# JanEGerken/HEAL-SWIN

Hardware: AMD Instinct MI355X
Metric: images/sec fwd+bwd, HEAL-SWIN nside=256 seg, batch=8 at 1/2/4/8 MI355X (higher is better)
Workload: dtype bf16

## Files before the change

heal_swin_amd/_lib.py:

```python
import ctypes
import os

import numpy as np

_PKG = os.path.dirname(os.path.abspath(__file__))
LIB_PATH = os.path.join(_PKG, "lib", "libhealswin.so")

HS_F32, HS_BF16 = 0, 1
HS_F64 = 3
HS_PRED_LABELS, HS_PRED_ROWS16 = 2, 4
HS_ATTN_COSINE = 1
HS_ATTN_FORCE_VALU = 2
HS_ATTN_RESIDUAL = 4
HS_ATTN_OVERWRITE_GRADS = 8
HS_EPI_BIAS, HS_EPI_GELU, HS_EPI_DGELU, HS_EPI_RESID = 0, 1, 2, 3
HS_ACC_DEFER = 2
HS_MLP_NORM_AFTER = 16
HS_U8, HS_I32, HS_I64 = 8, 9, 10
HS_FLAT_PATCH_ROWS, HS_FLAT_PIXEL_ROWS, HS_FLAT_IMAGE = 0, 1, 2
HS_DEPTH_L1, HS_DEPTH_L2, HS_DEPTH_HUBER, HS_DEPTH_LOGVAR = 0, 1, 2, 3
HS_DT_NONE, HS_DT_LOG, HS_DT_INV = 0, 1, 2
HS_DT_ZERO_BKG, HS_DT_1000_BKG, HS_DT_AFFINE, HS_DT_INVERSE = 1, 2, 4, 8
HS_DEPTH_STATS_WORDS = 15

c_i64 = ctypes.c_int64
c_int = ctypes.c_int
c_uint = ctypes.c_uint
c_ptr = ctypes.c_void_p
c_float = ctypes.c_float


class WgradProblem(ctypes.Structure):
    _fields_ = [("dy", c_ptr), ("x", c_ptr), ("dw", c_ptr), ("dbias", c_ptr), ("n_out", c_int), ("k_in", c_int), ("accumulate", c_int),
                ("gelu_x", c_int)]


def wgrad_problems(members):
    arr = (WgradProblem * len(members))()
    for q, (dy, x, dw, db, n_out, k_in, acc, gelu_x) in zip(arr, members):
        q.dy, q.x, q.dw, q.dbias = dy.data_ptr(), x.data_ptr(), dw.data_ptr(), (None if db is None else db.data_ptr())
        q.n_out, q.k_in, q.accumulate, q.gelu_x = int(n_out), int(k_in), int(acc), int(bool(gelu_x))
    return arr

_SIGNATURES = {
    "hs_nest2ring": [c_int, c_ptr, c_ptr, c_i64],
    "hs_ring2nest": [c_int, c_ptr, c_ptr, c_i64],
    "hs_nest_win_idcs": [c_int, c_ptr],
    "hs_rel_pos_index": [c_int, c_ptr],
    "hs_build_nest_roll_shift": [c_i64, c_int, c_int, c_ptr, c_ptr, c_ptr],
    "hs_build_nest_grid_shift": [c_int, c_int, c_int, c_ptr, c_ptr, c_ptr],
    "hs_build_ring_shift": [c_int, c_int, c_int, c_int, c_ptr, c_ptr, c_ptr],
    "hs_attn_mask_from_labels": [c_ptr, c_i64, c_int, c_ptr],
    "hs_flat_zorder": [c_int, c_int, c_int, c_ptr, c_ptr],
    "hs_build_flat_shift": [c_int, c_int, c_int, c_int, c_int, c_ptr, c_ptr, c_ptr],
    "hs_flat_rel_pos_index": [c_int, c_ptr, c_ptr],
    "hs_flat_attn_mask": [c_int, c_int, c_int, c_int, c_ptr],
    "hs_flat_img_to_rows": [c_ptr, c_int, c_ptr, c_int, c_int, c_int, c_int, c_int, c_int, c_int, c_int, c_i64, c_ptr],
    "hs_flat_rows_to_img": [c_ptr, c_int, c_ptr, c_int, c_int, c_int, c_int, c_int, c_int, c_int, c_int, c_i64, c_ptr],
    "hs_flat_resize": [c_ptr, c_int, c_i64, c_int, c_int, c_int, c_int, c_ptr, c_ptr, c_ptr, c_ptr, c_ptr, c_int, c_int, c_int, c_int, c_int,
                       c_int, c_i64, c_int, c_int, c_int, c_int, c_int, c_int, c_float, c_float, c_ptr],
    "hs_rel_bias_gather": [c_ptr, c_ptr, c_ptr, c_int, c_int, c_int, c_ptr],
    "hs_rel_bias_scatter_grad_sorted_add": [c_ptr, c_ptr, c_ptr, c_ptr, c_int, c_int, c_int, c_ptr],
    "hs_cos_head_scale_fwd": [c_ptr, c_ptr, c_int, c_ptr],
    "hs_cos_head_scale_bwd": [c_ptr, c_ptr, c_ptr, c_int, c_int, c_ptr],
    "hs_rel_bias_gather_many": [c_ptr, c_ptr, c_int, c_ptr, c_ptr, c_int, c_int, c_ptr],
    "hs_rel_bias_scatter_grad_sorted_many": [c_ptr, c_ptr, c_ptr, c_ptr, c_int, c_ptr, c_ptr, c_int, c_int, c_ptr],
    "hs_cos_head_scale_many": [c_ptr, c_ptr, c_ptr, c_ptr, c_ptr, c_int, c_ptr],
    "hs_rel_bias_scatter_grad": [c_ptr, c_ptr, c_ptr, c_int, c_int, c_int, c_ptr],
    "hs_rel_bias_scatter_grad_sorted": [c_ptr, c_ptr, c_ptr, c_ptr, c_int, c_int, c_int, c_ptr],
    "hs_window_attn_fwd": [c_ptr, c_ptr, c_ptr, c_ptr, c_ptr, c_ptr, c_i64, c_ptr,
                           c_int, c_i64, c_int, c_int, c_int, c_uint, ctypes.c_float, ctypes.c_uint64, c_int, c_ptr],
    "hs_window_attn_bwd": [c_ptr, c_ptr, c_ptr, c_ptr, c_ptr, c_ptr, c_ptr, c_ptr, c_ptr, c_ptr, c_ptr, c_i64, c_ptr,
                           c_int, c_i64, c_int, c_int, c_int, c_uint, ctypes.c_float, ctypes.c_uint64, c_int, c_ptr],
    "hs_gather_rows": [c_ptr, c_ptr, c_ptr, c_i64, c_int, c_i64, c_i64, c_ptr],
    "hs_pix2ang_nest": [c_int, c_i64, c_i64, c_ptr, c_ptr],
    "hs_ln_head_supported": [c_int, c_int, c_int],
    "hs_expand_ln_head_supported": [c_int, c_int, c_int, c_int],
    "hs_expand_ln_head_fwd": [c_ptr, c_ptr, c_ptr, c_ptr, c_ptr, c_ptr, c_ptr, c_ptr, c_ptr, c_i64, c_int, c_int, c_int, c_ptr],
    "hs_expand_ln_head_ce_fwd": [c_ptr, c_ptr, c_ptr, c_ptr, c_ptr, c_ptr, c_ptr, c_int, c_ptr, c_ptr, c_ptr, c_ptr, c_ptr, c_i64, c_int, c_int,
                                 c_int, c_ptr],
    "hs_expand_ln_head_ce_step_fwd": [c_ptr, c_ptr, c_ptr, c_ptr, c_ptr, c_ptr, c_ptr, c_int, c_ptr, c_ptr, c_ptr, c_ptr, c_ptr, c_ptr, c_ptr,
                                      c_ptr, c_i64, c_int, c_int, c_int, c_ptr],
    "hs_ln_head_ce_bwd": [c_ptr, c_ptr, c_ptr, c_ptr, c_ptr, c_ptr, c_int, c_ptr, c_ptr, c_ptr, c_ptr, c_ptr, c_ptr, c_i64, c_int, c_int, c_ptr],
    "hs_expand_ln_head_depth_fwd": [c_ptr, c_ptr, c_ptr, c_ptr, c_ptr, c_ptr, c_int, c_float, c_int, c_ptr, c_ptr, c_ptr, c_ptr, c_ptr, c_i64,
                                    c_int, c_int, c_int, c_ptr],
    "hs_expand_ln_head_depth_step_fwd": [c_ptr, c_ptr, c_ptr, c_ptr, c_ptr, c_ptr, c_int, c_float, c_int, c_ptr, c_ptr, c_ptr, c_ptr, c_ptr,
                                         c_int, c_int, c_float, c_float, c_int, ctypes.c_double, c_ptr, c_int, c_ptr, c_ptr, c_ptr, c_ptr,
                                         c_i64, c_int, c_int, c_int, c_ptr],
    "hs_ln_head_depth_bwd": [c_ptr, c_ptr, c_ptr, c_ptr, c_int, c_float, c_ptr, c_int, c_ptr, c_ptr, c_ptr, c_ptr, c_ptr, c_ptr, c_i64, c_int,
                             c_int, c_ptr],
    "hs_ln_head_fwd": [c_ptr, c_ptr, c_ptr, c_ptr, c_ptr, c_ptr, c_i64, c_int, c_int, c_int, c_ptr],
    "hs_ln_head_bwd": [c_ptr, c_ptr, c_ptr, c_ptr, c_ptr, c_ptr, c_ptr, c_ptr, c_i64, c_int, c_int, c_int, c_ptr],
    "hs_sample_bilinear_u8": [c_ptr, c_int, c_int, c_int, c_int, c_ptr, c_ptr, c_i64, c_ptr, c_ptr],
    "hs_sample_mask_u8": [c_ptr, c_int, c_int, c_int, c_ptr, c_ptr, c_i64, c_int, c_ptr, c_ptr],
    "hs_hp_interp_weights_nest": [c_int, c_ptr, c_ptr, c_i64, c_ptr, c_ptr],
    "hs_backproject_labels": [c_ptr, c_int, c_i64, c_i64, c_int, c_i64, c_i64, c_i64, c_ptr, c_i64, c_int, c_ptr, c_ptr],
    "hs_backproject_image": [c_ptr, c_i64, c_i64, c_ptr, c_ptr, c_i64, c_ptr, c_ptr],
    "hs_seg_confusion": [c_ptr, c_int, c_i64, c_i64, c_int, c_i64, c_i64, c_i64, c_ptr, c_i64, c_ptr, c_int, c_ptr, c_ptr, c_ptr],
    "hs_depth_points": [c_ptr, c_int, c_i64, c_i64, c_i64, c_i64, c_i64, c_i64, c_ptr, c_i64, c_ptr, c_int, c_ptr, c_ptr, c_ptr, c_ptr,
                        c_ptr],
    "hs_chamfer_nn": [c_ptr, c_ptr, c_i64, c_i64, c_ptr, c_ptr, c_i64, c_i64, c_i64, c_int, c_ptr, c_ptr, c_ptr, c_ptr, c_ptr, c_ptr,
                      c_ptr],
    "hs_depth_metrics": [c_ptr, c_int, c_i64, c_i64, c_i64, c_i64, c_i64, c_i64, c_i64, c_ptr, c_int, c_i64, c_i64, c_i64, c_int,
                         ctypes.c_double, c_ptr, c_int, c_ptr, c_ptr, c_ptr],
    "hs_backproject_depth": [c_ptr, c_int, c_i64, c_i64, c_i64, c_i64, c_ptr, c_ptr, c_i64, c_ptr, c_ptr],
    "hs_flat_depth_to_hp": [c_ptr, c_int, c_i64, c_i64, c_i64, c_i64, c_ptr, c_ptr, c_ptr, c_i64, c_ptr, c_ptr],
    "hs_depth_metrics_gather": [c_ptr, c_int, c_i64, c_i64, c_i64, c_i64, c_i64, c_ptr, c_ptr, c_ptr, c_i64, c_ptr, c_int, c_i64, c_i64,
                                c_int, ctypes.c_double, c_ptr, c_int, c_ptr, c_ptr, c_ptr],
    "hs_sample_bilinear_u8_f32": [c_ptr, c_int, c_int, c_int, c_int, c_ptr, c_ptr, c_i64, c_ptr, c_ptr],
    "hs_sample_nearest_f32": [c_ptr, c_int, c_int, c_int, c_ptr, c_ptr, c_i64, c_float, c_ptr, c_ptr],
    "hs_depth_target": [c_ptr, c_i64, c_i64, c_ptr, c_i64, c_i64, c_i64, c_i64, c_int, c_int, c_float, c_float, c_ptr],
    "hs_depth_stats_update": [c_ptr, c_i64, c_int, c_int, c_ptr, c_ptr, c_ptr],
    "hs_depth_stats_merge": [c_ptr, c_int, c_ptr, c_ptr],
    "hs_gelu_fwd": [c_ptr, c_ptr, c_i64, ctypes.c_float, ctypes.c_uint64, c_int, c_ptr],
    "hs_gelu_bwd": [c_ptr, c_ptr, c_ptr, c_i64, ctypes.c_float, ctypes.c_uint64, c_int, c_ptr],
    "hs_residual_drop": [c_ptr, c_ptr, c_ptr, c_ptr, c_i64, c_i64, ctypes.c_float, ctypes.c_uint64, c_int, c_ptr],
    "hs_linear_wgrad": [c_ptr, c_ptr, c_ptr, c_ptr, c_ptr, c_i64, c_int, c_int, c_int, c_int, c_ptr],
    "hs_reduce_flush": [c_ptr],
    "hs_set_seed_epoch": [c_ptr],
    "hs_linear_wgrad_gelu": [c_ptr, c_ptr, c_ptr, c_ptr, c_ptr, c_i64, c_int, c_int, c_int, c_int, c_ptr],
    "hs_linear_wgrad_gelu_supported": [c_i64, c_int, c_int, c_int],
    "hs_linear_wgrad_group_variant": [c_i64, c_int, c_int, c_int],
    "hs_linear_wgrad_group": [c_ptr, c_int, c_ptr, c_i64, c_int, c_ptr],
    "hs_mlp_fused_supported": [c_int, c_int, c_int],
    "hs_mlp_fused_fwd": [c_ptr, c_ptr, c_ptr, c_ptr, c_ptr, c_ptr, c_ptr, c_ptr, c_ptr, c_ptr, c_ptr, c_ptr, c_ptr, c_i64, c_int, c_int, c_uint,
                         c_int, c_ptr],
    "hs_mlp_fused_bwd": [c_ptr, c_ptr, c_ptr, c_ptr, c_ptr, c_ptr, c_ptr, c_i64, c_int, c_int, c_int, c_ptr],
    "hs_mlp_fused_drop_fwd": [c_ptr, c_ptr, c_ptr, c_ptr, c_ptr, c_ptr, c_ptr, c_ptr, c_ptr, c_ptr, c_ptr, c_ptr, c_ptr, c_ptr, c_i64, c_float,
                              ctypes.c_uint64, ctypes.c_uint64, c_i64, c_int, c_int, c_uint, c_int, c_ptr],
    "hs_mlp_fused_drop_bwd": [c_ptr, c_ptr, c_ptr, c_ptr, c_ptr, c_ptr, c_ptr, c_float, ctypes.c_uint64, c_i64, c_int, c_int, c_int, c_ptr],
    "hs_adam_step": [c_ptr, c_ptr, c_ptr, c_ptr, c_ptr, c_i64, c_float, c_ptr, c_float, c_float, c_float, c_float, c_int, c_ptr, c_ptr],
    "hs_adam_advance": [c_ptr, c_ptr],
    "hs_grad_stats": [c_ptr, c_i64, c_ptr, c_int, c_ptr, c_ptr],
    "hs_grad_guard_finalize": [c_ptr, c_i64, c_ptr, c_int, c_int, c_float, c_ptr, c_ptr, c_ptr, c_ptr],
    "hs_adam_step_guarded": [c_ptr, c_ptr, c_ptr, c_ptr, c_ptr, c_i64, c_float, c_ptr, c_float, c_float, c_float, c_float, c_int, c_ptr, c_float,
                             c_ptr, c_int, c_ptr],
    "hs_adam_advance_guarded": [c_ptr, c_ptr, c_int, c_ptr, c_ptr],
    "hs_grad_scale": [c_ptr, c_i64, c_float, c_ptr, c_ptr],
    "hs_split_bf16x3": [c_ptr, c_ptr, c_i64, c_int, c_int, c_ptr],
    "hs_gelu_split3": [c_ptr, c_ptr, c_ptr, c_i64, c_int, ctypes.c_float, ctypes.c_uint64, c_ptr],
    "hs_linear_wgrad_ld": [c_ptr, c_i64, c_i64, c_ptr, c_i64, c_i64, c_ptr, c_ptr, c_ptr, c_i64, c_int, c_int, c_int, c_ptr],
    "hs_layernorm_fwd": [c_ptr, c_ptr, c_ptr, c_ptr, c_ptr, c_ptr, c_ptr, c_i64, c_int, c_int, c_ptr],
    "hs_add_layernorm_fwd": [c_ptr, c_ptr, c_ptr, c_ptr, c_ptr, c_ptr, c_ptr, c_ptr, c_i64, c_int, c_int, c_ptr],
    "hs_add_layernorm_bwd": [c_ptr, c_ptr, c_ptr, c_ptr, c_ptr, c_ptr, c_ptr, c_ptr, c_ptr, c_ptr, c_int, c_i64, c_int, c_int, c_ptr],
    "hs_layernorm_drop_fwd": [c_ptr, c_ptr, c_ptr, c_ptr, c_ptr, c_ptr, c_ptr, c_ptr, c_i64, ctypes.c_float, ctypes.c_uint64,
                              c_i64, c_int, c_int, c_ptr],
    "hs_layernorm_drop_bwd": [c_ptr, c_ptr, c_ptr, c_ptr, c_ptr, c_ptr, c_ptr, c_ptr, c_ptr, c_int, c_ptr, c_i64, ctypes.c_float,
                              ctypes.c_uint64, c_i64, c_int, c_int, c_ptr],
    "hs_add_layernorm_drop_fwd": [c_ptr, c_ptr, c_ptr, c_ptr, c_ptr, c_ptr, c_ptr, c_ptr, c_ptr, c_i64, ctypes.c_float,
                                  ctypes.c_uint64, c_i64, c_int, c_int, c_ptr],
    "hs_layernorm_fwd_ex": [c_ptr, c_ptr, c_ptr, c_ptr, c_ptr, c_ptr, c_ptr, c_ptr, c_ptr, c_ptr, c_ptr, c_ptr, c_i64, ctypes.c_float,
                            ctypes.c_uint64, c_i64, c_int, c_int, c_ptr],
    "hs_add_layernorm_drop_bwd": [c_ptr, c_ptr, c_ptr, c_ptr, c_ptr, c_ptr, c_ptr, c_ptr, c_ptr, c_ptr, c_ptr, c_int, c_ptr, c_i64,
                                  ctypes.c_float, ctypes.c_uint64, c_i64, c_int, c_int, c_ptr],
    "hs_seg_ce_fwd": [c_ptr, c_ptr, c_ptr, c_ptr, c_i64, c_i64, c_int, c_i64, c_i64, c_i64, c_int, c_i64, c_int, c_ptr],
    "hs_seg_ce_bwd": [c_ptr, c_ptr, c_ptr, c_ptr, c_ptr, c_i64, c_i64, c_int, c_i64, c_i64, c_i64, c_i64, c_i64, c_i64, c_int, c_i64,
                      c_int, c_ptr],
    "hs_depth_loss_fwd": [c_ptr, c_ptr, c_ptr, c_i64, c_i64, c_int, c_i64, c_i64, c_i64, c_int, c_float, c_int, c_ptr],
    "hs_depth_loss_bwd": [c_ptr, c_ptr, c_ptr, c_ptr, c_i64, c_i64, c_int, c_i64, c_i64, c_i64, c_i64, c_i64, c_i64, c_int, c_float, c_int, c_ptr],
    "hs_gemm_nt": [c_ptr, c_i64, c_ptr, c_i64, c_int, c_ptr, c_i64, c_ptr, c_i64, c_int, c_ptr, c_ptr, c_ptr, c_i64, c_int, c_int,
                   ctypes.c_float, ctypes.c_uint64, c_int, c_ptr],
    "hs_gemm_nt_set_tile": [c_int],
    "hs_set_reserved_cus": [c_int],
    "hs_transpose_many_16": [c_ptr, c_int, c_int, c_ptr],
    "hs_debug_occupy_cus": [c_int, c_int, c_int, ctypes.c_double, c_ptr],
    "hs_debug_buffer_soffset_probe": [c_ptr, c_int, c_int, c_ptr, c_ptr],
    "hs_window_attn_module_supported": [c_int, c_int, c_int, c_int],
    "hs_window_attn_module_fwd": [c_ptr, c_ptr, c_ptr, c_ptr, c_ptr, c_ptr, c_ptr, c_ptr, c_ptr, c_ptr, c_ptr, c_i64, c_ptr, c_int, c_i64,
                                  c_int, c_int, c_int, c_uint, c_int, c_ptr],
    "hs_window_attn_module_fwd_train": [c_ptr] * 17 + [c_i64] + [c_ptr] * 6 + [c_int, c_i64, c_int, c_int, c_int, c_uint, c_int, c_ptr],
    "hs_window_attn_module_bwd_chain": [c_ptr] * 14 + [c_i64] + [c_ptr] * 11 + [c_int, c_int, c_i64, c_int, c_int, c_int, c_uint, c_int, c_ptr],
    "hs_layernorm_bwd": [c_ptr, c_ptr, c_ptr, c_ptr, c_ptr, c_ptr, c_ptr, c_ptr, c_ptr, c_int, c_i64, c_int, c_int, c_ptr],
    "hs_patch_merge_fwd": [c_ptr, c_ptr, c_ptr, c_ptr, c_ptr, c_ptr, c_ptr, c_ptr, c_i64, c_int, c_int, c_int, c_ptr],
    "hs_patch_merge_bwd": [c_ptr, c_ptr, c_ptr, c_ptr, c_ptr, c_ptr, c_ptr, c_ptr, c_ptr, c_ptr, c_ptr, c_ptr, c_ptr, c_int, c_i64,
                           c_int, c_int, c_int, c_ptr],
    "hs_patch_expand_fwd": [c_ptr, c_ptr, c_ptr, c_ptr, c_ptr, c_ptr, c_ptr, c_ptr, c_i64, c_int, c_int, c_int, c_int, c_ptr],
    "hs_patch_expand_bwd": [c_ptr, c_ptr, c_ptr, c_ptr, c_ptr, c_ptr, c_ptr, c_ptr, c_ptr, c_ptr, c_ptr, c_ptr, c_ptr, c_int, c_i64,
                            c_int, c_int, c_int, c_int, c_ptr],
}
_OTHER = {
    "hs_version": ([], ctypes.c_char_p),
    "hs_last_error": ([], ctypes.c_char_p),
    "hs_status_string": ([c_int], ctypes.c_char_p),
    "hs_device_count": ([], c_int),
    "hs_get_reserved_cus": ([], c_int),
    "hs_grad_guard_piece": ([], c_int),
    "hs_get_seed_epoch": ([], c_ptr),
    "hs_reduce_pending": ([c_ptr], c_int),
    "hs_layernorm_bwd_workspace": ([c_i64, c_int], c_i64),
    "hs_seg_ce_partials": ([c_i64, c_i64], c_i64),
    "hs_depth_loss_partials": ([c_i64, c_i64], c_i64),
    "hs_depth_points_workspace": ([c_i64, c_i64], c_i64),
    "hs_depth_metrics_partials": ([c_i64], c_i64),
    "hs_depth_stats_partials": ([c_i64], c_i64),
    "hs_flat_resize_lds_bytes": ([c_int, c_int, c_int, c_int, c_int, c_int], c_i64),
    "hs_ln_head_partials": ([c_i64], c_i64),
    "hs_expand_ln_head_blocks": ([c_i64], c_i64),
    "hs_linear_wgrad_workspace": ([c_i64, c_int, c_int], c_i64),
    "hs_linear_wgrad_group_workspace": ([c_ptr, c_int, c_i64, c_int], c_i64),
    "hs_window_attn_bwd_workspace": ([c_int, c_i64, c_int, c_int, c_int, c_int], c_i64),
    "hs_patch_merge_bwd_workspace": ([c_i64, c_int, c_int], c_i64),
    "hs_window_attn_module_bwd_chain_workspace": ([c_int, c_i64, c_int, c_int, c_int], c_i64),
    "hs_patch_expand_bwd_workspace": ([c_i64, c_int, c_int, c_int], c_i64),
}
EXPORTED_SYMBOLS = sorted(list(_SIGNATURES) + list(_OTHER))


def _load():
    if not os.path.exists(LIB_PATH):
        raise RuntimeError(
            f"libhealswin.so not found at {LIB_PATH}: build it first (python heal_swin_amd/build.py, or "
            "__graft_entry__.build()).  heal_swin_amd has no CPU or PyTorch fallback."
        )
    lib = ctypes.CDLL(LIB_PATH)
    for name, argtypes in _SIGNATURES.items():
        fn = getattr(lib, name)
        fn.argtypes = argtypes
        fn.restype = c_int
    for name, (argtypes, restype) in _OTHER.items():
        fn = getattr(lib, name)
        fn.argtypes = argtypes
        fn.restype = restype
    return lib


lib = _load()


def check(status, what):
    if status != 0:
        msg = lib.hs_last_error().decode()
        kind = lib.hs_status_string(status).decode()
        if status == 1:
            raise AssertionError(f"{what}: {msg}")
        raise RuntimeError(f"{what} failed ({kind}): {msg}")


def version():
    return lib.hs_version().decode()


def device_count():
    return int(lib.hs_device_count())


def np_ptr(a):
    return None if a is None else a.ctypes.data_as(c_ptr)


def ptr(t):
    return None if t is None else ctypes.c_void_p(t.data_ptr())


def stream_ptr(device):
    import torch

    return ctypes.c_void_p(torch.cuda.current_stream(device).cuda_stream)


def dtype_code(dtype):
    import torch

    if dtype == torch.float32:
        return HS_F32
    if dtype == torch.bfloat16:
        return HS_BF16
    raise TypeError(f"heal_swin_amd kernels support float32 and bfloat16 activations, got {dtype}")


def nest2ring(nside, ipix):
    a = np.ascontiguousarray(ipix, dtype=np.int64)
    out = np.empty_like(a)
    check(lib.hs_nest2ring(int(nside), np_ptr(a), np_ptr(out), a.size), "hs_nest2ring")
    return out


def ring2nest(nside, ipix):
    a = np.ascontiguousarray(ipix, dtype=np.int64)
    out = np.empty_like(a)
    check(lib.hs_ring2nest(int(nside), np_ptr(a), np_ptr(out), a.size), "hs_ring2nest")
    return out


def nest_win_idcs(window_size):
    side = int(round(window_size ** 0.5))
    out = np.empty((max(side, 1), max(side, 1)), dtype=np.int64)
    check(lib.hs_nest_win_idcs(int(window_size), np_ptr(out)), "hs_nest_win_idcs")
    return out


def rel_pos_index(window_size):
    out = np.empty((window_size, window_size), dtype=np.int64)
    check(lib.hs_rel_pos_index(int(window_size), np_ptr(out)), "hs_rel_pos_index")
    return out


def _shift_out(n):
    return np.empty(n, np.int32), np.empty(n, np.int32), np.empty(n, np.uint8)


def build_nest_roll_shift(n_pix, window_size, shift_size):
    idx, inv, lab = _shift_out(n_pix)
    check(lib.hs_build_nest_roll_shift(int(n_pix), int(window_size), int(shift_size), np_ptr(idx), np_ptr(inv), np_ptr(lab)),
          "hs_build_nest_roll_shift")
    return idx, inv, lab


def build_nest_grid_shift(nside, base_pix, window_size):
    idx, inv, lab = _shift_out(max(base_pix, 0) * nside * nside)
    check(lib.hs_build_nest_grid_shift(int(nside), int(base_pix), int(window_size), np_ptr(idx), np_ptr(inv), np_ptr(lab)),
          "hs_build_nest_grid_shift")
    return idx, inv, lab


def build_ring_shift(nside, base_pix, window_size, shift_size):
    idx, inv, lab = _shift_out(max(base_pix, 0) * nside * nside)
    check(lib.hs_build_ring_shift(int(nside), int(base_pix), int(window_size), int(shift_size), np_ptr(idx), np_ptr(inv),
                                  np_ptr(lab)), "hs_build_ring_shift")
    return idx, inv, lab


def attn_mask_from_labels(labels, window_size):
    lab = np.ascontiguousarray(labels, dtype=np.uint8)
    out = np.empty((lab.size // window_size, window_size, window_size), dtype=np.float32)
    check(lib.hs_attn_mask_from_labels(np_ptr(lab), lab.size, int(window_size), np_ptr(out)), "hs_attn_mask_from_labels")
    return out


def flat_zorder(Ht, Wt, T):
    z = np.empty(Ht * Wt, np.int32)
    rm = np.empty(Ht * Wt, np.int32)
    check(lib.hs_flat_zorder(int(Ht), int(Wt), int(T), np_ptr(z), np_ptr(rm)), "hs_flat_zorder")
    return z, rm


def build_flat_shift(Ht, Wt, T, window, shift):
    idx, inv, lab = _shift_out(max(Ht * Wt, 0))
    check(lib.hs_build_flat_shift(int(Ht), int(Wt), int(T), int(window), int(shift), np_ptr(idx), np_ptr(inv), np_ptr(lab)),
          "hs_build_flat_shift")
    return idx, inv, lab


# ... 13 lines not shown
```

heal_swin_amd/csrc/gemm_nt.hip:

```cpp
#include <cstdlib>
#include <type_traits>

#include "hs_gelu.h"

namespace hs {
HS_DEFINE_SEED_EPOCH_SETTER(set_seed_epoch_gemm_nt)
namespace {

typedef unsigned int u32x2 __attribute__((__vector_size__(8)));
typedef unsigned int u32x4v __attribute__((__vector_size__(16)));

#ifndef HS_GEMM_EPI_RING
#define HS_GEMM_EPI_RING 1
#endif
#ifndef HS_GEMM_STORE_AUX
#define HS_GEMM_STORE_AUX 2
#endif
#ifndef HS_GEMM_IN_AUX
#define HS_GEMM_IN_AUX 2
#endif
#ifndef HS_GEMM_EXP
#define HS_GEMM_EXP 0
#endif
#ifndef HS_GEMM_STAGGER_CYCLES
#define HS_GEMM_STAGGER_CYCLES 40000
#endif
enum { EPI_BIAS = 0, EPI_GELU = 1, EPI_DGELU = 2, EPI_RESID = 3 };
constexpr int64_t kMaxRecords = 0x7FFFFE00;

struct GemmParams {
    const uint16_t *a, *b;
    int64_t lda, ldb;
    int k;
    const uint16_t *a2, *b2;
    int64_t lda2, ldb2;
    int k2;
    const float* bias;
    uint16_t* c;
    uint16_t* aux;
    int64_t m;
    int n;
    int tiles_n, tiles, per_xcd, blocks_per_xcd;
    float drop_p;
    uint64_t seed;
#ifdef HS_GEMM_TRACE
    uint64_t* trace;
#endif
};
#ifdef HS_GEMM_TRACE
constexpr int kTraceCap = 240;
#endif

constexpr int epi_younger_ops(int tm, int i) {
    const int stores = i < 2 ? i : 1;
    const int last_d = i + 1 < tm - 1 ? i + 1 : tm - 1;
    return 4 * (stores + (last_d - i));
}

template <int OFF>
__device__ __forceinline__ u32x4 lds_read_b128(uint32_t addr) {
    u32x4 v;
    asm volatile("ds_read_b128 %0, %1 offset:%2" : "=v"(v) : "v"(addr), "n"(OFF));
    return v;
}

template <int BM, int BN, int WM, int WN, int NSTAGE, bool ALIAS, int EPI, bool DROP, bool FAST>
__global__ void __launch_bounds__(WM * WN * 64, 2) gemm_nt_kernel(GemmParams p) {
#if defined(__HIP_DEVICE_COMPILE__)
    constexpr int NW = WM * WN;
    constexpr int TM = BM / WM / 32, TN = BN / WN / 32;
    constexpr int AB = BM * 128, BB = BN * 128, STAGE = AB + BB;
    constexpr int IW = FAST ? NW / 2 : NW;
    constexpr int AI = AB / 1024 / IW, BI = BB / 1024 / IW;
    static_assert(AI >= 1 && BI >= 1 && TM >= 1 && TN >= 1, "tile too small for the wave grid");
    static_assert(!ALIAS || NW * 4096 <= STAGE, "patches do not fit a stage buffer");
    constexpr bool HAS_IN = EPI == EPI_DGELU || EPI == EPI_RESID;
    constexpr bool RING = HS_GEMM_EPI_RING && HAS_IN && ALIAS && TM == 4 && TN == 2 && STAGE >= NW * 8192;
    constexpr bool LBIAS = ALIAS && EPI != EPI_DGELU;
    constexpr int NSLOT = NSTAGE + 1;
    static_assert(BN * 4 <= 1024, "a bias slot holds one 1-KB DMA piece");
    constexpr int BIAS_OFF = NSTAGE * STAGE + (ALIAS ? 0 : NW * 4096), BIAS_LDS = LBIAS ? NSLOT * 1024 : 0;
#ifdef HS_GEMM_TRACE
    constexpr int TRACE_LDS = BIAS_OFF + BIAS_LDS + NW * kTraceCap * 8 <= 163840 ? NW * kTraceCap * 8 : 0;
#else
    constexpr int TRACE_LDS = 0;
#endif
    static_assert(BIAS_OFF + BIAS_LDS + TRACE_LDS <= 163840, "LDS of one workgroup exceeds 160 KB");
    __shared__ __attribute__((aligned(16))) unsigned char smem[BIAS_OFF + BIAS_LDS + TRACE_LDS];

    const int tid = threadIdx.x, lane = tid & 63, half = lane >> 5, l31 = lane & 31;
    const int wave = __builtin_amdgcn_readfirstlane(tid >> 6);
    const int wm = wave / WN, wn = wave % WN;

    const int xcd = blockIdx.x & 7, lb = blockIdx.x >> 3;
    const int id_end = min((xcd + 1) * p.per_xcd, p.tiles);
    const int id0 = xcd * p.per_xcd + lb;
    if (id0 >= id_end) return;
    const int nk1 = (p.k + 63) >> 6, nk2 = (p.k2 + 63) >> 6, nk = nk1 + nk2;
#if HS_GEMM_EXP & 24
    {
        const int phases = (HS_GEMM_EXP & 16) ? 4 : 2;
        const long long wait = (long long)(lb % phases) * (HS_GEMM_STAGGER_CYCLES / phases);
        const long long t0 = clock64();
        while (clock64() - t0 < wait) __builtin_amdgcn_s_sleep(8);
    }
#endif

    constexpr bool SC = FAST;
    static_assert(!FAST || (AI % 4 == 0 && BI % 4 == 0), "FAST: whole groups of four pieces per issuing wave");
    constexpr int AJ = SC ? 4 : AI, BJ = SC ? 4 : BI;
    int a_row[AJ], a_col[AJ], b_row[BJ], b_col[BJ];
#pragma unroll
    for (int j = 0; j < AJ; ++j) {
        const int q = (wave * AI + j) * 64 + lane, R = q >> 4, lc = (q & 15) ^ (R & 15);
        a_row[j] = 2 * R + (lc >> 3);
        a_col[j] = (lc & 7) << 4;
    }
#pragma unroll
    for (int j = 0; j < BJ; ++j) {
        const int q = (wave * BI + j) * 64 + lane, R = q >> 4, lc = (q & 15) ^ (R & 15);
        b_row[j] = 2 * R + (lc >> 3);
        b_col[j] = (lc & 7) << 4;
    }

    __amdgpu_buffer_rsrc_t ra, rb;
    int a_off[AJ], b_off[BJ];
    int kseg = 0;
    int a_ld32 = 0, b_ld32 = 0;
    int slot_i = 0;
    __amdgpu_buffer_rsrc_t rbias = __builtin_amdgcn_make_buffer_rsrc((void*)p.bias, 0, p.bias ? p.n * 4 : 0, 0x00020000);
    auto retarget = [&](int id, bool s2, bool enter) {
        const int tm = id / p.tiles_n, tn = id - tm * p.tiles_n;
        const int64_t m0 = (int64_t)tm * BM;
        const int n0 = tn * BN;
        if constexpr (LBIAS) {
            if (enter) {
                if (wave == 0)
                    __builtin_amdgcn_raw_ptr_buffer_load_lds(rbias, (lds_void*)(smem + BIAS_OFF + slot_i * 1024), 16,
                                                             lane * 4 < BN ? (uint32_t)(lane * 16) : kOob, n0 * 4, 0, 0);
                slot_i = slot_i + 1 == NSLOT ? 0 : slot_i + 1;
            }
        }
        const uint16_t* ap = s2 ? p.a2 : p.a;
        const uint16_t* bp = s2 ? p.b2 : p.b;
        const int64_t lda = s2 ? p.lda2 : p.lda, ldb = s2 ? p.ldb2 : p.ldb;
        kseg = (s2 ? p.k2 : p.k) * 2;
        int64_t abytes = (p.m - m0 - 1) * lda * 2 + kseg, bbytes = (int64_t)(p.n - n0 - 1) * ldb * 2 + kseg;
        abytes = abytes > kMaxRecords ? kMaxRecords : abytes;
        bbytes = bbytes > kMaxRecords ? kMaxRecords : bbytes;
        ra = __builtin_amdgcn_make_buffer_rsrc((void*)(ap + m0 * lda), 0, (int)abytes, 0x00020000);
        rb = __builtin_amdgcn_make_buffer_rsrc((void*)(bp + (int64_t)n0 * ldb), 0, (int)bbytes, 0x00020000);
#pragma unroll
        for (int j = 0; j < AJ; ++j) a_off[j] = a_row[j] * ((int)lda * 2) + a_col[j];
#pragma unroll
        for (int j = 0; j < BJ; ++j) b_off[j] = b_row[j] * ((int)ldb * 2) + b_col[j];
        a_ld32 = (int)lda * 64;
        b_ld32 = (int)ldb * 64;
    };
    auto issue_pieces = [&](int kb, int buf, auto first_c, auto count_c) {
        constexpr int first = decltype(first_c)::value, count = decltype(count_c)::value;
        if (IW < NW && wave >= IW) return;
        unsigned char* base = smem + buf * STAGE;
#pragma unroll
        for (int q = first; q < first + count; ++q) {
            if constexpr (SC) {
            if (q < AI) {
                __builtin_amdgcn_raw_ptr_buffer_load_lds(ra, (lds_void*)(base + (wave * AI + q) * 1024), 16, (uint32_t)a_off[q % AJ],
                                                         kb + (q >> 2) * a_ld32, 0, 0);
            } else {
                const int j = q - AI;
                __builtin_amdgcn_raw_ptr_buffer_load_lds(rb, (lds_void*)(base + AB + (wave * BI + j) * 1024), 16, (uint32_t)b_off[j % BJ],
                                                         kb + (j >> 2) * b_ld32, 0, 0);
            }
            } else {

            if (q < AI) {
                const uint32_t voff = kb + a_col[q] < kseg ? (uint32_t)(a_off[q] + kb) : kOob;
                __builtin_amdgcn_raw_ptr_buffer_load_lds(ra, (lds_void*)(base + (wave * AI + q) * 1024), 16, voff, 0, 0, 0);
            } else {
                const int j = q - AI;
                const uint32_t voff = kb + b_col[j] < kseg ? (uint32_t)(b_off[j] + kb) : kOob;
                __builtin_amdgcn_raw_ptr_buffer_load_lds(rb, (lds_void*)(base + AB + (wave * BI + j) * 1024), 16, voff, 0, 0, 0);
            }
            }
        }
    };

    const uint32_t lds0 = (uint32_t)(uintptr_t)(__attribute__((address_space(3))) unsigned char*)smem;
#ifdef HS_GEMM_TRACE
    const bool tr_on = TRACE_LDS > 0 && p.trace && (blockIdx.x == 0 || blockIdx.x == 9);
    int tr_n = 0;
    const uint32_t tr_base = lds0 + BIAS_OFF + BIAS_LDS + wave * kTraceCap * 8;
    auto TR = [&](int code) {
        if (tr_on && tr_n < kTraceCap) {
            const uint64_t t = (clock64() << 8) | (uint64_t)code;
            if (lane == 0) asm volatile("ds_write_b64 %0, %1" ::"v"(tr_base + tr_n * 8), "v"(t) : "memory");
            ++tr_n;
        }
    };
#else
    auto TR = [&](int) {};
#endif
    uint32_t a_frag[TM], b_frag[TN];
#pragma unroll
    for (int i = 0; i < TM; ++i) {
        const int r = wm * (BM / WM) + i * 32 + l31, R = r >> 1;
        a_frag[i] = lds0 + R * 256 + (((((r & 1) << 3) + half) ^ (R & 15)) << 4);
    }
#pragma unroll
    for (int j = 0; j < TN; ++j) {
        const int r = wn * (BN / WN) + j * 32 + l31, R = r >> 1;
        b_frag[j] = lds0 + AB + R * 256 + (((((r & 1) << 3) + half) ^ (R & 15)) << 4);
    }

    f32x16 acc[TN][TM];
#pragma unroll
    for (int j = 0; j < TN; ++j)
#pragma unroll
        for (int i = 0; i < TM; ++i)
#pragma unroll
            for (int r = 0; r < 16; ++r) acc[j][i][r] = 0.f;
#if HS_GEMM_EXP & 2
    int64_t exp_total = p.m * (int64_t)p.n * 2;
    exp_total = exp_total > kMaxRecords ? kMaxRecords : exp_total;
    const __amdgpu_buffer_rsrc_t rexp = __builtin_amdgcn_make_buffer_rsrc((void*)p.aux, 0, (int)(p.aux ? exp_total : 0), 0x00020000);
    const uint32_t exp_share = (uint32_t)((exp_total / gridDim.x) & ~(int64_t)1023);
    uint32_t exp_pos = 0;
    const uint32_t exp_base = blockIdx.x * exp_share;
#endif

    auto compute = [&](int buf, bool prefetch, int kb_next, int buf_next) {
        const uint32_t bo = buf * STAGE;
        constexpr int NSET = (TM == 4 && TN == 2) ? 2 : 3;
        u32x4 fa[NSET][TM], fb[NSET][TN];
        auto read_frags = [&](auto ks_c) {
            constexpr int ks = decltype(ks_c)::value, set = ks % NSET;
#pragma unroll
            for (int j = 0; j < TN; ++j) fb[set][j] = lds_read_b128<0>((b_frag[j] ^ (ks << 5)) + bo);
#pragma unroll
            for (int i = 0; i < TM; ++i) fa[set][i] = lds_read_b128<0>((a_frag[i] ^ (ks << 5)) + bo);
        };
        constexpr int PIECES = AI + BI;
        constexpr int PER = TM + TN;
        auto wait_frags = [&](auto ks_c, auto left_c) {
            constexpr int ks = decltype(ks_c)::value, left = decltype(left_c)::value, set = ks % NSET;
            (void)fa;
            (void)fb;
            if constexpr (TM == 2 && TN == 2)
                asm volatile("s_waitcnt lgkmcnt(%4)" : "+v"(fa[set][0]), "+v"(fa[set][1]), "+v"(fb[set][0]), "+v"(fb[set][1]) : "n"(left));
            else if constexpr (TM == 4 && TN == 2)
// ... 124 lines not shown
                    } else {
                        u32x4 rws[4];
#pragma unroll
                        for (int t = 0; t < 4; ++t)
                            rws[t] = __builtin_bit_cast(u32x4, __builtin_amdgcn_raw_buffer_load_b128(rx, rl_voff, row_soff(i, t), 0));
                        asm volatile("ds_write_b128 %0, %1" ::"v"(row_addr), "v"(rws[0]) : "memory");
                        asm volatile("ds_write_b128 %0, %1 offset:1024" ::"v"(row_addr), "v"(rws[1]) : "memory");
                        asm volatile("ds_write_b128 %0, %1 offset:2048" ::"v"(row_addr), "v"(rws[2]) : "memory");
                        asm volatile("ds_write_b128 %0, %1 offset:3072" ::"v"(row_addr), "v"(rws[3]) : "memory");
                    }
#pragma unroll
                    for (int j = 0; j < TJ; ++j)
#pragma unroll
                        for (int g = 0; g < 4; ++g)
                            asm volatile("ds_read_b64 %0, %1" : "=v"(xin[j][g]) : "v"(own_addr + (((4 * j + g) ^ (l31 & 7)) << 4)));
                    asm volatile("s_waitcnt lgkmcnt(0)"
                                 : "+v"(xin[0][0]), "+v"(xin[0][1]), "+v"(xin[0][2]), "+v"(xin[0][3]), "+v"(xin[TJ - 1][0]),
                                   "+v"(xin[TJ - 1][1]), "+v"(xin[TJ - 1][2]), "+v"(xin[TJ - 1][3]));
                } else {
#pragma unroll
                    for (int j = 0; j < TJ; ++j)
#pragma unroll
                        for (int g = 0; g < 4; ++g) {
                            const int n = ncol0 + j * 32 + 4 * half + 8 * g;
                            xin[j][g] = __builtin_amdgcn_raw_buffer_load_b64(rx, n < p.n ? (uint32_t)(ml * n2 + n * 2) : kOob, 0, 0);
                        }
                }
            }
            u32x2 o1[TJ][4], o2[TJ][4];
            {
#pragma unroll
                for (int j = 0; j < TJ; ++j) {
                    if constexpr (LBIAS) lds_bias(j, bias4[j]);
#pragma unroll
                    for (int g = 0; g < 4; ++g) {
                        const int n = ncol0 + j * 32 + 4 * half + 8 * g;
                        f32x16& a16 = acc[TJ * jh + j][i];
                        f32x2 v[2] = {f32x2{a16[4 * g], a16[4 * g + 1]} + f32x2{bias4[j][g].x, bias4[j][g].y},
                                      f32x2{a16[4 * g + 2], a16[4 * g + 3]} + f32x2{bias4[j][g].z, bias4[j][g].w}};
                        uint32_t ck = 0;
                        if (DROP) ck = rng.chunk_key((uint64_t)((m0 + ml) * p.n + n) >> 3);
                        auto drop2 = [&](int t) {
                            const uint32_t hh = ElemRng::pair_bits(ck, t == 0 ? (half ? ElemRng::kM2 : ElemRng::kM0) : (half ? ElemRng::kM3 : ElemRng::kM1));
                            return f32x2{rng.keep_lo(hh), rng.keep_hi(hh)};
                        };
                        if (EPI == EPI_GELU) {
                            o1[j][g] = u32x2{pack_bf16x2(v[0].x, v[0].y), pack_bf16x2(v[1].x, v[1].y)};
                            a16[4 * g] = v[0].x; a16[4 * g + 1] = v[0].y; a16[4 * g + 2] = v[1].x; a16[4 * g + 3] = v[1].y;
                            continue;
                        } else {
                            if (EPI == EPI_DGELU || EPI == EPI_RESID) {
#pragma unroll
                                for (int t = 0; t < 2; ++t) {
                                    const f32x2 x = {__uint_as_float(xin[j][g][t] << 16), __uint_as_float(xin[j][g][t] & 0xffff0000u)};
                                    if (EPI == EPI_DGELU) {
                                        v[t] *= gelu_grad2(x);
                                        if (DROP) v[t] *= drop2(t);
                                    } else {
                                        v[t] += x;
                                    }
                                }
                            }
                            o1[j][g] = u32x2{pack_bf16x2(v[0].x, v[0].y), pack_bf16x2(v[1].x, v[1].y)};
                        }
#pragma unroll
                        for (int r = 0; r < 4; ++r) a16[4 * g + r] = 0.f;
                    }
                }
            }
            auto make_o2 = [&]() {
#pragma unroll
                for (int j = 0; j < TJ; ++j)
#pragma unroll
                    for (int g0 = 0; g0 < 4; g0 += 2) {
                        f32x16& a16 = acc[TJ * jh + j][i];
                        f32x2 v[4] = {f32x2{a16[4 * g0], a16[4 * g0 + 1]}, f32x2{a16[4 * g0 + 2], a16[4 * g0 + 3]},
                                      f32x2{a16[4 * g0 + 4], a16[4 * g0 + 5]}, f32x2{a16[4 * g0 + 6], a16[4 * g0 + 7]}};
#if !(HS_GEMM_EXP & 4)
#pragma unroll
                        for (int t = 0; t < 4; ++t) v[t] = gelu2(v[t]);
#endif
#pragma unroll
                        for (int gg = 0; gg < 2; ++gg) {
                            const int g = g0 + gg;
                            if (DROP) {
                                const int n = ncol0 + j * 32 + 4 * half + 8 * g;
                                const uint32_t ck = rng.chunk_key((uint64_t)((m0 + ml) * p.n + n) >> 3);
#pragma unroll
                                for (int t = 0; t < 2; ++t) {
                                    const uint32_t hh = ElemRng::pair_bits(ck, t == 0 ? (half ? ElemRng::kM2 : ElemRng::kM0) : (half ? ElemRng::kM3 : ElemRng::kM1));
                                    v[2 * gg + t] *= f32x2{rng.keep_lo(hh), rng.keep_hi(hh)};
                                }
                            }
                            o2[j][g] = u32x2{pack_bf16x2(v[2 * gg].x, v[2 * gg].y), pack_bf16x2(v[2 * gg + 1].x, v[2 * gg + 1].y)};
#pragma unroll
                            for (int r = 0; r < 4; ++r) a16[4 * g + r] = 0.f;
                        }
                    }
            };
            TR(20);
            auto emit = [&](const __amdgpu_buffer_rsrc_t& rs, const u32x2 (&o)[TJ][4]) {
                if (wide) {
#pragma unroll
                    for (int j = 0; j < TJ; ++j)
#pragma unroll
                        for (int g = 0; g < 4; ++g)
                            asm volatile("ds_write_b64 %0, %1" ::"v"(own_out + (((4 * j + g) ^ (l31 & 7)) << 4)), "v"(o[j][g]) : "memory");
                    u32x4 rws[4];
                    asm volatile("ds_read_b128 %0, %1" : "=v"(rws[0]) : "v"(row_addr));
                    asm volatile("ds_read2_b64 %0, %1 offset0:129 offset1:128" : "=v"(rws[1]) : "v"(row_addr));
                    asm volatile("ds_read_b128 %0, %1 offset:2048" : "=v"(rws[2]) : "v"(row_addr));
                    asm volatile("ds_read2_b64 %0, %1 offset0:129 offset1:128" : "=v"(rws[3]) : "v"(row_addr + 2048));
                    asm volatile("s_waitcnt lgkmcnt(0)" : "+v"(rws[0]), "+v"(rws[1]), "+v"(rws[2]), "+v"(rws[3]));
                    TR(22);
#pragma unroll
                    for (int t = 0; t < 4; ++t)
                        __builtin_amdgcn_raw_buffer_store_b128(__builtin_bit_cast(u32x4v, rws[t]), rs, rl_voff, row_soff(i, t), HS_GEMM_STORE_AUX);
                    asm volatile("s_nop 0" ::"v"(rws[0]), "v"(rws[1]), "v"(rws[2]), "v"(rws[3]));
                } else {
#pragma unroll
                    for (int j = 0; j < TJ; ++j)
#pragma unroll
                        for (int g = 0; g < 4; ++g) {
                            const int n = ncol0 + j * 32 + 4 * half + 8 * g;
                            __builtin_amdgcn_raw_buffer_store_b64(o[j][g], rs, n < p.n ? (uint32_t)(ml * n2 + n * 2) : kOob, 0, HS_GEMM_STORE_AUX);
                        }
                }
            };
            if (EPI == EPI_GELU) {
                if (NW == 8 && wave >= NW / 2) {
                    make_o2();
                    emit(rx, o2);
                    TR(21);
                    __builtin_amdgcn_sched_barrier(0);
                    if (p.c) emit(rc, o1);
                } else {
                    if (p.c) emit(rc, o1);
                    TR(21);
                    __builtin_amdgcn_sched_barrier(0);
                    make_o2();
                    emit(rx, o2);
                }
            } else {
                emit(rc, o1);
            }
            if constexpr (RING) {
                if (i + 2 < TM) request_in(i + 2);
            }
            TR(12 + i);
        }
        }
    };

    const int stride = p.blocks_per_xcd;
    int id_i = id0, ks_i = 0;
    int id_c = id0, ks_c = 0;
    int slot_c = 0;
    auto advance_issue = [&]() {
        ++ks_i;
        if (ks_i == nk) {
            ks_i = 0;
            id_i += stride;
            if (id_i < id_end) retarget(id_i, nk1 == 0, true);
        } else if (ks_i == nk1) {
            retarget(id_i, true, false);
        }
    };
    auto kb_of = [&](int ks) { return (ks >= nk1 ? ks - nk1 : ks) * 128; };
    retarget(id_i, false, true);
    constexpr int AHEAD = NSTAGE - 1, PIECES_ALL = AI + BI;
    int issued = 0;
#pragma unroll
    for (int q = 0; q < AHEAD; ++q) {
        if (id_i < id_end) {
            issue_pieces(kb_of(ks_i), q, std::integral_constant<int, 0>{}, std::integral_constant<int, PIECES_ALL>{});
            advance_issue();
            ++issued;
        }
    }
    int buf = 0, buf_free = AHEAD;
#if HS_GEMM_EXP & 32
    if (NW == 8 && wave >= NW / 2) __builtin_amdgcn_s_setprio(1);
#endif
#if HS_GEMM_EXP & 64
    if (NW == 8 && wave < NW / 2) __builtin_amdgcn_s_setprio(1);
#endif
    bool drained = false;
    constexpr int kEpiOps = TM * (TN / 2 > 0 ? TN / 2 : 1) * 4;
    static_assert((AHEAD - 1) * PIECES_ALL + kEpiOps <= 63, "vmcnt immediate");
    TR(0);
    while (true) {
        TR(3);
        if (IW < NW && wave >= IW) {
        } else if (AHEAD > 1 && issued == AHEAD && !drained)
            asm volatile("s_waitcnt vmcnt(%0)" ::"n"((AHEAD - 1) * PIECES_ALL) : "memory");
        else if (drained && issued == AHEAD)
            asm volatile("s_waitcnt vmcnt(%0)" ::"n"((AHEAD - 1) * PIECES_ALL + kEpiOps) : "memory");
        else if (drained && issued == 1)
            asm volatile("s_waitcnt vmcnt(%0)" ::"n"(kEpiOps) : "memory");
        else
            asm volatile("s_waitcnt vmcnt(0)" ::: "memory");
        drained = false;
        TR(1);
        __builtin_amdgcn_s_barrier();
        TR(2);
        const bool more = id_i < id_end;
        const bool last = ks_c + 1 == nk;
        compute(buf, more, kb_of(ks_i), buf_free);
        --issued;
        if (more) {
            advance_issue();
            ++issued;
        }
        const int buf_done = buf;
        buf = buf + 1 == NSTAGE ? 0 : buf + 1;
        buf_free = buf_free + 1 == NSTAGE ? 0 : buf_free + 1;
        if (last) {
            epilogue(id_c, buf_done, slot_c);
            slot_c = slot_c + 1 == NSLOT ? 0 : slot_c + 1;
            drained = true;
            ks_c = 0;
            id_c += stride;
            if (id_c >= id_end) break;
        } else {
            ++ks_c;
        }
    }
#ifdef HS_GEMM_TRACE
    if (tr_on) {
        asm volatile("s_waitcnt vmcnt(0) lgkmcnt(0)" ::: "memory");
        uint64_t* out = p.trace + ((blockIdx.x == 0 ? 0 : 1) * NW + wave) * kTraceCap;
        for (int i = lane; i < kTraceCap; i += 64) {
            u32x2 v = {0u, 0u};
            if (i < tr_n) {
                asm volatile("ds_read_b64 %0, %1\n\ts_waitcnt lgkmcnt(0)" : "=v"(v) : "v"(tr_base + i * 8) : "memory");
            }
            out[i] = ((uint64_t)v[1] << 32) | v[0];
        }
    }
#endif
#endif
}

template <int BM, int BN, int WM, int WN, int NSTAGE, bool ALIAS, bool FAST>
int launch_tile(GemmParams& p, int epi, int wgs_per_cu, hipStream_t s) {
    const int tiles_m = (int)((p.m + BM - 1) / BM);
    p.tiles_n = (p.n + BN - 1) / BN;
    const int64_t tiles = (int64_t)tiles_m * p.tiles_n;
    if (tiles > 0x7fffffff) return fail(HS_ERR_UNSUPPORTED, "too many output tiles");
    p.tiles = (int)tiles;
    p.per_xcd = (p.tiles + 7) / 8;
    const int resident = usable_cus_per_xcd() * wgs_per_cu;
    p.blocks_per_xcd = p.per_xcd < resident ? p.per_xcd : resident;
    const dim3 grid((unsigned)(8 * p.blocks_per_xcd)), block(WM * WN * 64);
    const bool drop = p.drop_p > 0.f;
#define HS_GEMM_LAUNCH(E, D) hipLaunchKernelGGL((gemm_nt_kernel<BM, BN, WM, WN, NSTAGE, ALIAS, E, D, FAST>), grid, block, 0, s, p)
    switch (epi) {
        case EPI_BIAS: HS_GEMM_LAUNCH(EPI_BIAS, false); break;
        case EPI_GELU:
            if (drop) HS_GEMM_LAUNCH(EPI_GELU, true);
            else HS_GEMM_LAUNCH(EPI_GELU, false);
            break;
        case EPI_DGELU:
            if (drop) HS_GEMM_LAUNCH(EPI_DGELU, true);
            else HS_GEMM_LAUNCH(EPI_DGELU, false);
            break;
        default: HS_GEMM_LAUNCH(EPI_RESID, false); break;
    }
#undef HS_GEMM_LAUNCH
    HS_LAUNCH_CHECK("gemm_nt");
    return HS_OK;
}

}

int gemm_nt_check_shape(const char* who, int64_t lda, int64_t ldb, int k, int64_t lda2, int64_t ldb2, int k2, int64_t m, int n) {
    HS_CHECK_ARG(m > 0 && n > 0 && k > 0 && k2 >= 0, "%s: empty shape", who);
    if (k % 8 || k2 % 8 || lda % 8 || ldb % 8 || (k2 && (lda2 % 8 || ldb2 % 8)) || n % 4)
        return fail(HS_ERR_UNSUPPORTED, "%s: k, k2 and the row strides must be multiples of 8, n a multiple of 4", who);
    if (lda * 2 * 256 > kMaxRecords || ldb * 2 * 256 > kMaxRecords || (int64_t)n * 2 * 256 > kMaxRecords)
        return fail(HS_ERR_UNSUPPORTED, "%s: row stride too large", who);
    if (((m + 127) / 128) * (((int64_t)n + 127) / 128) > 0x7fffffff) return fail(HS_ERR_UNSUPPORTED, "%s: too many output tiles", who);
    return HS_OK;
}

}

namespace {
int g_tile_variant = 0;
}

#ifdef HS_GEMM_TRACE
namespace {
uint64_t* g_trace = nullptr;
}
extern "C" int hs_gemm_nt_set_trace(void* buf) {
    g_trace = (uint64_t*)buf;
    return 0;
}
#endif

extern "C" {

int hs_gemm_nt_set_tile(int variant) {
    g_tile_variant = variant;
    return HS_OK;
}

int hs_gemm_nt(const void* a, int64_t lda, const void* b, int64_t ldb, int k, const void* a2, int64_t lda2, const void* b2,
               int64_t ldb2, int k2, const float* bias, void* c, void* aux, int64_t m, int n, int epilogue, float drop_p,
               uint64_t seed, int dtype, void* stream) {
    using namespace hs;
    HS_CHECK_ARG(dtype == HS_BF16, "hs_gemm_nt: bf16 activations only (fp32 runs use the library GEMM)");
    HS_CHECK_ARG(a && b && m > 0 && n > 0 && k > 0, "hs_gemm_nt: null operand or empty shape");
    HS_CHECK_ARG(epilogue >= EPI_BIAS && epilogue <= EPI_RESID, "hs_gemm_nt: unknown epilogue %d", epilogue);
    HS_CHECK_ARG(k2 == 0 || (a2 && b2 && k2 > 0), "hs_gemm_nt: second segment needs a2, b2, k2 > 0");
    HS_CHECK_ARG(c || (epilogue == EPI_GELU && aux), "hs_gemm_nt: no output");
    HS_CHECK_ARG(epilogue == EPI_BIAS || aux, "hs_gemm_nt: this epilogue needs aux");
    HS_CHECK_ARG(drop_p >= 0.f && drop_p <= 1.f, "hs_gemm_nt: drop_p must be in [0, 1]");
    HS_CHECK_ALIGNED("hs_gemm_nt", 16, a, b, a2, b2, bias, c, aux);
    if (int st = gemm_nt_check_shape("hs_gemm_nt", lda, ldb, k, lda2, ldb2, k2, m, n)) return st;
    GemmParams p{};
    p.a = (const uint16_t*)a; p.b = (const uint16_t*)b; p.lda = lda; p.ldb = ldb; p.k = k;
    p.a2 = (const uint16_t*)a2; p.b2 = (const uint16_t*)b2; p.lda2 = lda2; p.ldb2 = ldb2; p.k2 = k2;
    p.bias = bias; p.c = (uint16_t*)c; p.aux = (uint16_t*)aux; p.m = m; p.n = n;
    p.drop_p = drop_p; p.seed = seed;
#ifdef HS_GEMM_TRACE
    p.trace = g_trace;
#endif
    int variant = g_tile_variant;
    if (!variant) {
        const int64_t tiles2 = ((m + 255) / 256) * ((n + 127) / 128), tiles3 = ((m + 255) / 256) * ((n + 255) / 256);
        if (tiles2 < 256)
            variant = 1;
        else if ((epilogue == EPI_GELU || epilogue == EPI_DGELU) ? n >= 512 : (n >= 1024 && k + k2 >= 512))
            variant = 3;
        else if (n >= 256 && tiles3 >= 768 && k % 64 == 0 && k2 % 64 == 0)
            variant = 3;
        else
            variant = 2;
    }
    if (variant == 3 && (epilogue == EPI_DGELU || epilogue == EPI_RESID) && n % 8) variant = 2;
    hipStream_t st = (hipStream_t)stream;
    const bool fast = k % 64 == 0 && k2 % 64 == 0;
    switch (variant) {
        case 2: return fast ? launch_tile<256, 128, 4, 2, 3, true, true>(p, epilogue, 1, st) : launch_tile<256, 128, 4, 2, 3, true, false>(p, epilogue, 1, st);
        case 3: return fast ? launch_tile<256, 256, 2, 4, 2, true, true>(p, epilogue, 1, st) : launch_tile<256, 256, 2, 4, 2, true, false>(p, epilogue, 1, st);
        default: return launch_tile<128, 128, 2, 2, 2, false, false>(p, epilogue, 2, st);
    }
}

}
```

heal_swin_amd/models_torch/swin_hp_transformer.py:

```python
import math
from contextlib import contextmanager
from dataclasses import dataclass, field
from typing import List, Literal, Optional

import numpy as np
import torch
import torch.nn as nn
import torch.nn.functional as F
import torch.utils.checkpoint as checkpoint

from .. import _lib, ops
from ..data_spec import DataSpec
from . import hp_shifting

EMIT_REFERENCE_BUFFERS = True


class HSLayerNorm(nn.LayerNorm):

    def forward(self, x, residual=None, row_scale=None, drop_p=0.0):
        assert self.elementwise_affine and len(self.normalized_shape) == 1 and abs(self.eps - 1e-5) < 1e-12
        return ops.layer_norm(x, self.weight, self.bias, residual, row_scale=row_scale, drop_p=drop_p)


def _make_norm(norm_layer, dim):
    return HSLayerNorm(dim) if norm_layer is nn.LayerNorm else norm_layer(dim)


class HSLinear(nn.Linear):

    def forward(self, x):
        return ops.linear(x, self.weight, self.bias)

    def forward_passthrough(self, x):
        return ops.linear_passthrough(x, self.weight, self.bias)

    def forward_residual(self, x, residual):
        return ops.linear_residual(x, self.weight, self.bias, residual)


class DropPath(nn.Module):

    def __init__(self, drop_prob=0.0):
        super().__init__()
        self.drop_prob = float(drop_prob)

    def sample_scale(self, batch, device):
        if self.drop_prob == 0.0 or not self.training:
            return None
        keep = 1.0 - self.drop_prob
        return torch.empty(batch, dtype=torch.float32, device=device).bernoulli_(keep).div_(keep)

    def forward(self, x):
        rs = self.sample_scale(x.shape[0], x.device)
        if rs is None:
            return x
        return x * rs.to(x.dtype).view((x.shape[0],) + (1,) * (x.dim() - 1))


class Mlp(nn.Module):

    def __init__(self, in_features, hidden_features=None, out_features=None, act_layer=nn.GELU, drop=0.0):
        super().__init__()
        self.fc1 = HSLinear(in_features, hidden_features or in_features)
        self.act = act_layer()
        self.fc2 = HSLinear(hidden_features or in_features, out_features or in_features)
        self.drop = nn.Dropout(drop)

    def forward(self, x, apply_out_drop=True, residual_alias=False, residual=None):
        exact_gelu = isinstance(self.act, nn.GELU) and getattr(self.act, "approximate", "none") == "none"
        if exact_gelu and x.dtype in (torch.bfloat16, torch.float32) and x.is_cuda:
            out = ops.mlp(x, self.fc1.weight, self.fc1.bias, self.fc2.weight, self.fc2.bias,
                          drop_p=self.drop.p if self.training else 0.0, passthrough=residual_alias, residual=residual)
            y, x_res = out if residual_alias else (out, None)
        elif residual is not None:
            return self.fc2(self.drop(self.act(self.fc1(x)))) + residual
        else:
            x_res = None
            if residual_alias:
                h, x_res = self.fc1.forward_passthrough(x)
            else:
                h = self.fc1(x)
            y = self.fc2(self.drop(self.act(h)))
        y = self.drop(y) if apply_out_drop else y
        return (y, x_res) if residual_alias else y


def _labels_from_dense_mask(mask):
    m = mask.detach().cpu()
    nW, Ws, _ = m.shape
    same = m == 0
    labels = same.to(torch.uint8).argmax(dim=2).to(torch.uint8)
    rebuilt = (labels[:, :, None] != labels[:, None, :]).to(m.dtype) * (-100)
    if not torch.equal(rebuilt.to(torch.float32), m.to(torch.float32)):
        raise NotImplementedError("WindowAttention mask is not a {0,-100} region mask; dense masks are not supported")
    return labels.reshape(-1).contiguous()


class WindowAttention(nn.Module):

    def __init__(self, dim, window_size, num_heads, rel_pos_bias=None, qkv_bias=True, qk_scale=None,
                 attn_drop=0.0, proj_drop=0.0, use_cos_attn=False):
        super().__init__()
        self.dim, self.window_size, self.num_heads = dim, window_size, num_heads
        self.use_cos_attn = use_cos_attn
        self.scale = qk_scale or (dim // num_heads) ** -0.5
        self.rel_pos_bias = rel_pos_bias
        if use_cos_attn:
            self.logit_scale = nn.Parameter(torch.log(10 * torch.ones((num_heads, 1, 1))), requires_grad=True)
        if rel_pos_bias == "flat":
            side = int(round(window_size ** 0.5))
            self.relative_position_bias_table = nn.Parameter(torch.zeros(((2 * side - 1) ** 2, num_heads)))
            rel = _lib.rel_pos_index(window_size)
            self.register_buffer("relative_position_index", torch.from_numpy(rel))
            self.register_buffer("_rel_idx32", torch.from_numpy(rel.astype(np.int32).reshape(-1)), persistent=False)
        self._scale_cache = None
        self.qkv = HSLinear(dim, dim * 3, bias=qkv_bias)
        self.attn_drop = nn.Dropout(attn_drop)
        self.proj = HSLinear(dim, dim)
        self.proj_drop = nn.Dropout(proj_drop)

    def extra_repr(self):
        return f"dim={self.dim}, window_size={self.window_size}, num_heads={self.num_heads}"

    def head_scale(self):
        if self.use_cos_attn:
            now = self.__dict__.get("_scale_now")
            if now is not None:
                return now
            if self.logit_scale.is_cuda and self.logit_scale.dtype == torch.float32:
                return ops.cos_head_scale(self.logit_scale)
            return torch.exp(torch.clamp(self.logit_scale, max=math.log(1.0 / 0.01))).reshape(-1)
        dev = self.qkv.weight.device
        if self._scale_cache is None or self._scale_cache.device != dev:
            self._scale_cache = torch.full((self.num_heads,), float(self.scale), dtype=torch.float32, device=dev)
        return self._scale_cache

    def bias(self):
        if self.rel_pos_bias is None:
            return None
        now = self.__dict__.get("_bias_now")
        if now is not None:
            return now
        return ops.RelPosBiasFn.apply(self.relative_position_bias_table, self._rel_idx32, self.window_size)

    def attend(self, x, window_size, idx, roll, labels, apply_proj_drop=True, residual_alias=False, residual=None):
        drop = self.attn_drop.p if self.training else 0.0
        if self.rel_pos_bias is not None and window_size != self.window_size:
            raise AssertionError("relative position bias needs input_resolution >= window_size")
        x_res = None
        if self.fusable(x, window_size):
            y = self.fused_module(x, window_size, idx, roll, labels)
            return (y, x) if residual_alias else y
        if residual is None and self.trainable_fused(x, window_size):
            return ops.window_attn_module_train(x, None, None, self.qkv.weight, self.qkv.bias, self.proj.weight, self.proj.bias,
                                                self.bias(), self.head_scale(), idx, roll, labels, self.num_heads, window_size,
                                                self.use_cos_attn, residual_alias=residual_alias)
        if residual_alias:
            qkv, x_res = self.qkv.forward_passthrough(x)
        else:
            qkv = self.qkv(x)
        o = ops.window_attn_core(qkv, self.bias(), self.head_scale(), idx, roll, labels, self.num_heads, window_size,
                                 self.use_cos_attn, attn_drop=drop)
        if residual is not None:
            return self.proj.forward_residual(o, residual)
        y = self.proj(o)
        y = self.proj_drop(y) if apply_proj_drop else y
        return (y, x_res) if residual_alias else y

    def fusable(self, x, window_size):
        return (ops.window_attn_module_ok(x, self.num_heads, window_size) and
                not (self.training and (self.attn_drop.p > 0 or self.proj_drop.p > 0)) and
                (self.rel_pos_bias is None or window_size == self.window_size))

    def fused_module(self, x, window_size, idx, roll, labels, norm=None, residual=False):
        return ops.window_attn_module(x, self.qkv.weight, self.qkv.bias, self.proj.weight, self.proj.bias, self.bias(),
                                      self.head_scale(), idx, roll, labels, self.num_heads, window_size, self.use_cos_attn,
                                      ln_weight=None if norm is None else norm.weight, ln_bias=None if norm is None else norm.bias,
                                      residual=residual)

    def trainable_fused(self, x, window_size):
        return (ops.window_attn_module_train_ok(x, self.num_heads, window_size) and
                not (self.training and (self.attn_drop.p > 0 or self.proj_drop.p > 0)) and
                (self.rel_pos_bias is None or window_size == self.window_size))

    def fused_module_train(self, x, window_size, idx, roll, labels, norm, norm2=None):
        return ops.window_attn_module_train(x, norm.weight, norm.bias, self.qkv.weight, self.qkv.bias, self.proj.weight,
                                            self.proj.bias, self.bias(), self.head_scale(), idx, roll, labels, self.num_heads,
                                            window_size, self.use_cos_attn,
                                            norm2=None if norm2 is None else (norm2.weight, norm2.bias))

    def forward(self, x, mask=None):
        B_, Ws, C = x.shape
        if mask is None:
            return self.attend(x.reshape(1, B_ * Ws, C), Ws, None, 0, None).reshape(B_, Ws, C)
        nW = mask.shape[0]
        labels = _labels_from_dense_mask(mask).to(x.device)
        return self.attend(x.reshape(B_ // nW, nW * Ws, C), Ws, None, 0, labels).reshape(B_, Ws, C)


class SwinTransformerBlock(nn.Module):

    def __init__(self, dim, input_resolution, base_pix, num_heads, window_size=4, shift_size=0, shift_strategy="nest_roll",
                 rel_pos_bias=None, mlp_ratio=4.0, qkv_bias=True, qk_scale=None, drop=0.0, attn_drop=0.0, drop_path=0.0,
                 act_layer=nn.GELU, norm_layer=nn.LayerNorm, use_v2_norm_placement=False, use_cos_attn=False):
        super().__init__()
        self.dim, self.input_resolution, self.num_heads = dim, input_resolution, num_heads
        self.window_size, self.shift_size, self.mlp_ratio = window_size, shift_size, mlp_ratio
        self.use_v2_norm_placement = use_v2_norm_placement
        self.n_tokens = input_resolution
        if input_resolution <= window_size:
            self.shift_size, self.window_size = 0, input_resolution

        self._build_branches(dim, WindowAttention(dim, window_size=window_size, num_heads=num_heads, rel_pos_bias=rel_pos_bias,
                                                  qkv_bias=qkv_bias, qk_scale=qk_scale, attn_drop=attn_drop, proj_drop=drop,
                                                  use_cos_attn=use_cos_attn),
                             mlp_ratio, drop, drop_path, act_layer, norm_layer)

        nside = math.sqrt(input_resolution // base_pix)
        assert nside % 1 == 0, "nside has to be an integer in every layer"
        nside = int(nside)
        if self.shift_size > 0:
            if shift_strategy == "nest_roll":
                shifter = hp_shifting.NestRollShift(self.shift_size, self.input_resolution, self.window_size)
            elif shift_strategy == "nest_grid_shift":
                shifter = hp_shifting.NestGridShift(nside, base_pix, self.window_size)
            elif shift_strategy == "ring_shift":
                shifter = hp_shifting.RingShift(nside, base_pix, self.window_size, self.shift_size)
            else:
                raise KeyError(shift_strategy)
        else:
            shifter = hp_shifting.NoShift()
        self._set_shifter(shifter)

    def _build_branches(self, dim, attn, mlp_ratio, drop, drop_path, act_layer, norm_layer):
        self.norm1 = _make_norm(norm_layer, dim)
        self.attn = attn
        self.drop_path = DropPath(drop_path) if drop_path > 0.0 else nn.Identity()
        self.norm2 = _make_norm(norm_layer, dim)
        self.mlp = Mlp(in_features=dim, hidden_features=int(dim * mlp_ratio), act_layer=act_layer, drop=drop)

    def _set_shifter(self, shifter):
        self.shifter = shifter
        self._is_roll = isinstance(self.shifter, hp_shifting.NestRollShift)
        self._shifted = self.shift_size > 0

        self.register_buffer("attn_mask", None)
        self._register_state_dict_hook(SwinTransformerBlock._emit_attn_mask)
        self._register_load_state_dict_pre_hook(self._accept_attn_mask, with_module=False)

    @staticmethod
    def _emit_attn_mask(module, state_dict, prefix, local_metadata):
        if EMIT_REFERENCE_BUFFERS and module._shifted:
            mask = module.shifter.get_mask()
            if mask is not None:
                state_dict[prefix + "attn_mask"] = mask

    def _accept_attn_mask(self, state_dict, prefix, local_metadata, strict, missing_keys, unexpected_keys, error_msgs):
        state_dict.pop(prefix + "attn_mask", None)

    def extra_repr(self):
        return (f"dim={self.dim}, input_resolution={self.input_resolution}, num_heads={self.num_heads}, "
                f"window_size={self.window_size}, shift_size={self.shift_size}, mlp_ratio={self.mlp_ratio}")

    def _attention_branch(self, x, apply_proj_drop=True, residual_alias=False, residual=None):
        if not self._shifted:
            return self.attn.attend(x, self.window_size, None, 0, None, apply_proj_drop, residual_alias, residual)
        idx, _, labels = self.shifter.tables(x.device)
        if self._is_roll:
            return self.attn.attend(x, self.window_size, None, self.shift_size % x.shape[1], labels, apply_proj_drop, residual_alias,
                                    residual)
        return self.attn.attend(x, self.window_size, idx, 0, labels, apply_proj_drop, residual_alias, residual)

    def _stochastic(self):
        return self.training and ((isinstance(self.drop_path, DropPath) and self.drop_path.drop_prob > 0) or
                                  self.attn.proj_drop.p > 0 or self.mlp.drop.p > 0)

    def _hs_norms(self):
        return isinstance(self.norm1, HSLayerNorm) and isinstance(self.norm2, HSLayerNorm)

    def _path_scale(self, x):
        return self.drop_path.sample_scale(x.shape[0], x.device) if isinstance(self.drop_path, DropPath) else None

    def _fused_mlp(self, x1, post_norm=False):
        m = self.mlp
        if not (isinstance(self.norm2, HSLayerNorm) and isinstance(m.fc1, HSLinear) and isinstance(m.fc2, HSLinear) and
                isinstance(m.act, nn.GELU) and getattr(m.act, "approximate", "none") == "none" and
                ops.fused_mlp_ok(x1, m.fc1.weight.shape[0]) and m.fc2.weight.shape[0] == self.dim):
            return None
        rs = self._path_scale(x1) if self.training else None
        dp = m.drop.p if self.training else 0.0
        if rs is None and not dp:
            return ops.fused_mlp_block(x1, self.norm2.weight, self.norm2.bias, m.fc1.weight, m.fc1.bias, m.fc2.weight, m.fc2.bias,
                                       post_norm=post_norm)
        if ops.fused_mlp_stochastic_ok(x1, post_norm):
            return ops.fused_mlp_block(x1, self.norm2.weight, self.norm2.bias, m.fc1.weight, m.fc1.bias, m.fc2.weight, m.fc2.bias,
                                       post_norm=True, row_scale=rs, drop_p=dp)
        return None

    def can_defer(self):
        return not self.use_v2_norm_placement and self._hs_norms()

    def _shift_args(self, x):
        if not self._shifted:
            return None, 0, None
        idx, _, labels = self.shifter.tables(x.device)
        if self._is_roll:
            return None, self.shift_size % x.shape[1], labels
        return idx, 0, labels

    def forward_deferred(self, x, pending, x_lo=None, comp=None):
        train = self.training
        comp = (ops.COMP_RESIDUAL if comp is None else comp) and x.dtype == torch.bfloat16
        if self.attn.fusable(x, self.window_size) and not (train and isinstance(self.drop_path, DropPath) and self.drop_path.drop_prob > 0):
            xs = self.resolve_pending(x, pending)
            idx, roll, labels = self._shift_args(xs)
            x1 = self.attn.fused_module(xs, self.window_size, idx, roll, labels, norm=self.norm1, residual=True)
            x2 = self._fused_mlp(x1)
            if x2 is not None:
                return x2, None, None
            m = self.mlp(self.norm2(x1), apply_out_drop=False)
            return x1, (m, None, 0.0), None
        if ops.RESID_EPILOGUE and x.dtype == torch.bfloat16 and not comp and x_lo is None and not self._stochastic():
            C = self.dim
            proj_own = ops.own_gemm_ok(_lib.HS_EPI_BIAS, C, C, x.dtype, m=x.numel() // C)
            fc2_own = ops.own_gemm_ok(_lib.HS_EPI_BIAS, C, self.mlp.fc1.weight.shape[0], x.dtype, m=x.numel() // C)
            if pending is None and self.attn.trainable_fused(x, self.window_size):
                idx, roll, labels = self._shift_args(x)
                if ops.FUSED_NORM2:
                    n2, x1 = self.attn.fused_module_train(x, self.window_size, idx, roll, labels, self.norm1, norm2=self.norm2)
                else:
                    x1 = self.attn.fused_module_train(x, self.window_size, idx, roll, labels, self.norm1)
                    x2 = self._fused_mlp(x1)
                    if x2 is not None:
                        return x2, None, None
                    n2, x1 = ops.layer_norm_passthrough(x1, self.norm2.weight, self.norm2.bias)
                if fc2_own:
                    return self.mlp(n2, apply_out_drop=False, residual=x1), None, None
                return x1, (self.mlp(n2, apply_out_drop=False), None, 0.0), None
            if proj_own or fc2_own:
                if pending is None:
                    n1, xs = ops.layer_norm_passthrough(x, self.norm1.weight, self.norm1.bias)
                else:
                    t, rs, dp = pending
                    xs, n1 = ops.add_layer_norm(x, t, self.norm1.weight, self.norm1.bias, row_scale=rs, drop_p=dp)
                if proj_own:
                    x1 = self._attention_branch(n1, apply_proj_drop=False, residual=xs)
                    x2 = self._fused_mlp(x1)
                    if x2 is not None:
                        return x2, None, None
                    n2, x1 = ops.layer_norm_passthrough(x1, self.norm2.weight, self.norm2.bias)
                else:
                    x1, n2 = ops.add_layer_norm(xs, self._attention_branch(n1, apply_proj_drop=False), self.norm2.weight, self.norm2.bias)
                if fc2_own:
                    return self.mlp(n2, apply_out_drop=False, residual=x1), None, None
                return x1, (self.mlp(n2, apply_out_drop=False), None, 0.0), None
        if pending is None:
            n1, x = ops.layer_norm_passthrough(x, self.norm1.weight, self.norm1.bias)
        elif comp:
            t, rs, dp = pending
            x, n1, x_lo = ops.add_layer_norm_stream(x, x_lo, t, self.norm1.weight, self.norm1.bias, row_scale=rs, drop_p=dp)
        else:
            t, rs, dp = pending
            x, n1 = ops.add_layer_norm(x, t, self.norm1.weight, self.norm1.bias, row_scale=rs, drop_p=dp)
        a = self._attention_branch(n1, apply_proj_drop=False)
        if comp:
            x1, n2, x1_lo = ops.add_layer_norm_stream(x, x_lo, a, self.norm2.weight, self.norm2.bias, row_scale=self._path_scale(x),
                                                      drop_p=self.attn.proj_drop.p if train else 0.0)
        else:
            x1_lo = None
            x1, n2 = ops.add_layer_norm(x, a, self.norm2.weight, self.norm2.bias, row_scale=self._path_scale(x),
                                        drop_p=self.attn.proj_drop.p if train else 0.0)
        m = self.mlp(n2, apply_out_drop=False)
        return x1, (m, self._path_scale(x), self.mlp.drop.p if train else 0.0), x1_lo

    def can_stream_v2(self):
        return self.use_v2_norm_placement and self._hs_norms()

    def forward_stream_v2(self, x, x_lo=None):
        train = self.training
        a, xr = self._attention_branch(x, apply_proj_drop=False, residual_alias=True)
        x, x_lo = ops.layer_norm_stream(a, self.norm1.weight, self.norm1.bias, xr, res_lo=x_lo, row_scale=self._path_scale(x),
                                        drop_p=self.attn.proj_drop.p if train else 0.0)
        m, xr = self.mlp(x, apply_out_drop=False, residual_alias=True)
        return ops.layer_norm_stream(m, self.norm2.weight, self.norm2.bias, xr, res_lo=x_lo, row_scale=self._path_scale(x),
                                     drop_p=self.mlp.drop.p if train else 0.0)

    @staticmethod
    def resolve_pending(x, pending):
        if pending is None:
            return x
        t, rs, dp = pending
        vec = 8 if t.dtype == torch.bfloat16 else 4
        if (dp or rs is not None) and t.is_cuda and t.dtype in (torch.bfloat16, torch.float32) and (t.numel() // t.shape[0]) % vec == 0:
            return ops.residual_drop(x, t, rs, dp)
        if dp:
            t = F.dropout(t, dp, True)
        if rs is not None:
            t = t * rs.to(t.dtype).view(-1, 1, 1)
        return x + t

    def forward(self, x):
        B, N, C = x.shape
        assert N == self.n_tokens, f"expected {self.n_tokens} tokens, got {N}"
        if self.can_defer():
            return self.resolve_pending(*self.forward_deferred(x, None)[:2])
        train = self.training
        if self.use_v2_norm_placement and self._hs_norms():
            a, xr = self._attention_branch(x, apply_proj_drop=False, residual_alias=True)
            x = self.norm1(a, residual=xr, row_scale=self._path_scale(x), drop_p=self.attn.proj_drop.p if train else 0.0)
            x2 = self._fused_mlp(x, post_norm=True)
            if x2 is not None:
                return x2
            m, xr = self.mlp(x, apply_out_drop=False, residual_alias=True)
            return self.norm2(m, residual=xr, row_scale=self._path_scale(x), drop_p=self.mlp.drop.p if train else 0.0)
        if self.use_v2_norm_placement:
            x = x + self.drop_path(self.norm1(self._attention_branch(x)))
            return x + self.drop_path(self.norm2(self.mlp(x)))
        x = x + self.drop_path(self._attention_branch(self.norm1(x)))
        return x + self.drop_path(self.mlp(self.norm2(x)))


class PatchMerging(nn.Module):

    def __init__(self, dim, dim_scale=2, norm_layer=nn.LayerNorm):
        super().__init__()
        self.dim = dim
        self.reduction = HSLinear(4 * dim, dim_scale * dim, bias=False)
        self.norm = _make_norm(norm_layer, 4 * dim)

    def forward(self, x):
        B, N, C = x.shape
        assert N % 4 == 0, f"x size {N} is not divisible by 4 as necessary for patching."
        return self.reduction(self.norm(x.reshape(B, N // 4, 4 * C)))


class PatchExpand(nn.Module):

    def __init__(self, dim, dim_scale=2, norm_layer=nn.LayerNorm):
        super().__init__()
        self.dim = dim
        self.expand = HSLinear(dim, dim_scale * dim, bias=False) if dim_scale != 1 else nn.Identity()
        self.norm = _make_norm(norm_layer, dim * dim_scale // 4)

    def forward(self, x):
        x = self.expand(x)
        B, N, C = x.shape
        return self.norm(x.reshape(B, N * 4, C // 4))


class FinalPatchExpand_X4(nn.Module):

    def __init__(self, patch_size, dim, norm_layer=nn.LayerNorm):
        super().__init__()
        self.dim, self.patch_size, self.output_dim = dim, patch_size, dim
        self.expand = HSLinear(dim, patch_size * dim, bias=False)
        self.norm = _make_norm(norm_layer, dim)

    def forward(self, x):
        x = self.expand(x)
        B, N, C = x.shape
        return self.norm(x.reshape(B, N * self.patch_size, C // self.patch_size))


def _build_blocks(dim, input_resolution, depth, num_heads, window_size, base_pix, shift_size, shift_strategy, rel_pos_bias,
                  mlp_ratio, qkv_bias, qk_scale, drop, attn_drop, drop_path, norm_layer, use_v2_norm_placement, use_cos_attn):
    return nn.ModuleList([
        SwinTransformerBlock(dim=dim, input_resolution=input_resolution, base_pix=base_pix, num_heads=num_heads,
                             window_size=window_size, shift_size=shift_size if i % 2 else 0,
                             shift_strategy=shift_strategy, rel_pos_bias=rel_pos_bias, mlp_ratio=mlp_ratio, qkv_bias=qkv_bias,
                             qk_scale=qk_scale, drop=drop, attn_drop=attn_drop,
                             drop_path=drop_path[i] if isinstance(drop_path, list) else drop_path, norm_layer=norm_layer,
                             use_v2_norm_placement=use_v2_norm_placement, use_cos_attn=use_cos_attn)
        for i in range(depth)
    ])


class _Stage(nn.Module):
    def _run_blocks(self, x):
        pending = None
        x_lo = None
        for blk in self.blocks:
            if self.use_checkpoint:
                x, pending, x_lo = SwinTransformerBlock.resolve_pending(x, pending), None, None
                x = checkpoint.checkpoint(blk, x, use_reentrant=False)
            elif blk.can_defer():
                x, pending, x_lo = blk.forward_deferred(x, pending, x_lo, comp=self._comp())
            elif blk.can_stream_v2() and self._comp() and x.dtype == torch.bfloat16 and x.is_cuda:
                x, x_lo = blk.forward_stream_v2(x, x_lo)
            else:
                x, pending, x_lo = SwinTransformerBlock.resolve_pending(x, pending), None, None
                x = blk(x)
        return SwinTransformerBlock.resolve_pending(x, pending)

    comp_residual = None

    def _comp(self):
        return ops.COMP_RESIDUAL if self.comp_residual is None else bool(self.comp_residual)

    def extra_repr(self):
        return f"dim={self.dim}, input_resolution={self.input_resolution}, depth={self.depth}"


class BasicLayer(_Stage):

    def __init__(self, dim, input_resolution, depth, num_heads, window_size, base_pix, shift_size, shift_strategy, rel_pos_bias,
                 mlp_ratio=4.0, qkv_bias=True, qk_scale=None, drop=0.0, attn_drop=0.0, drop_path=0.0, norm_layer=nn.LayerNorm,
                 downsample=None, use_checkpoint=False, use_v2_norm_placement=False, use_cos_attn=False):
        super().__init__()
        self.dim, self.input_resolution, self.depth, self.use_checkpoint = dim, input_resolution, depth, use_checkpoint
        self.blocks = _build_blocks(dim, input_resolution, depth, num_heads, window_size, base_pix, shift_size, shift_strategy,
                                    rel_pos_bias, mlp_ratio, qkv_bias, qk_scale, drop, attn_drop, drop_path, norm_layer,
                                    use_v2_norm_placement, use_cos_attn)
        self.downsample = downsample(dim=dim, norm_layer=norm_layer) if downsample is not None else None

    def forward(self, x):
        x = self._run_blocks(x)
        return x if self.downsample is None else self.downsample(x)


class BasicLayer_up(_Stage):

    def __init__(self, dim, input_resolution, depth, num_heads, window_size, base_pix, shift_size, shift_strategy, rel_pos_bias,
                 mlp_ratio=4.0, qkv_bias=True, qk_scale=None, drop=0.0, attn_drop=0.0, drop_path=0.0, norm_layer=nn.LayerNorm,
                 upsample=None, use_checkpoint=False, use_v2_norm_placement=False, use_cos_attn=False):
        super().__init__()
# ... 401 lines not shown
```

heal_swin_amd/ops/attention.py:

```python
import ctypes
import os

import torch

from .. import _lib
from .._lib import check, lib, ptr, stream_ptr
from .runtime import RT, _cast_param, _f32, _require_gpu, _sink_buffer, _timed
from .norm import LayerNormFn
from .gemm import LinearFn


class RelPosBiasFn(torch.autograd.Function):

    @staticmethod
    def forward(ctx, table, rel_idx, window_size):
        _require_gpu(table, rel_idx)
        assert rel_idx.dtype == torch.int32 and rel_idx.is_contiguous()
        t = _f32(table)
        rows, nh = t.shape
        bias = torch.empty((nh, window_size, window_size), dtype=torch.float32, device=t.device)
        check(lib.hs_rel_bias_gather(ptr(t), ptr(rel_idx), ptr(bias), rows, nh, window_size, stream_ptr(t.device)),
              "hs_rel_bias_gather")
        ctx.save_for_backward(rel_idx)
        ctx.shape = (rows, nh, window_size)
# ... 168 lines not shown

FORCE_VALU_ATTENTION = False


class WindowAttnCoreFn(torch.autograd.Function):

    @staticmethod
    def forward(ctx, qkv, bias, head_scale, idx, roll, labels, num_heads, window_size, cosine, attn_drop=0.0, seed=0, pre=None):
        _require_gpu(qkv, bias, head_scale, idx, labels)
        B, N, C3 = qkv.shape
        C = C3 // 3
        qkv = qkv.contiguous()
        dt = _lib.dtype_code(qkv.dtype)
        hs = _f32(head_scale).reshape(-1)
        assert hs.numel() == num_heads
        bias_c = _f32(bias)
        flags = (_lib.HS_ATTN_COSINE if cosine else 0) | (_lib.HS_ATTN_FORCE_VALU if FORCE_VALU_ATTENTION else 0)
        if pre is not None:
            out, lse = pre
        else:
            out = torch.empty((B, N, C), dtype=qkv.dtype, device=qkv.device)
            need_grad = any(ctx.needs_input_grad[:3])
            lse = torch.empty((B, num_heads, N), dtype=torch.float32, device=qkv.device) if need_grad else None
            with _timed("window_attn_fwd", qkv.device, 4 * B * N * C * qkv.element_size(), 4 * B * N * C * window_size):
                check(lib.hs_window_attn_fwd(ptr(qkv), ptr(out), ptr(lse), ptr(bias_c), ptr(hs), ptr(idx), int(roll), ptr(labels),
                                             B, N, C, num_heads, window_size, flags, float(attn_drop), int(seed), dt,
                                             stream_ptr(qkv.device)),
                      "hs_window_attn_fwd")
        ctx.save_for_backward(qkv, out, lse, bias_c, hs, idx, labels)
        ctx.args = (B, N, C, num_heads, window_size, flags, dt, int(roll))
        ctx.drop = (float(attn_drop), int(seed))
        ctx.bias_dtype = None if bias is None else bias.dtype
        ctx.scale_meta = (head_scale.dtype, head_scale.shape)
        return out

    @staticmethod
    def backward(ctx, dout):
        qkv, out, lse, bias_c, hs, idx, labels = ctx.saved_tensors
        B, N, C, nh, ws, flags, dt, roll = ctx.args
        dout = dout.contiguous()
        dqkv = torch.empty_like(qkv)
        nb = bias_c.numel() if bias_c is not None else 0
        mfma_bf16 = qkv.dtype == torch.bfloat16 and ws == 64 and C == 32 * nh and not (flags & _lib.HS_ATTN_FORCE_VALU)
        if mfma_bf16:
            flags |= _lib.HS_ATTN_OVERWRITE_GRADS
            zeros = torch.empty(nb + hs.numel(), dtype=torch.float32, device=qkv.device)
        else:
            zeros = torch.zeros(nb + hs.numel(), dtype=torch.float32, device=qkv.device)
        dbias = zeros[:nb].view(bias_c.shape) if bias_c is not None else None
        dscale = zeros[nb:].view(hs.shape)
        nws = int(lib.hs_window_attn_bwd_workspace(B, N, C, nh, ws, dt))
        wsp = torch.empty(nws, dtype=torch.float32, device=qkv.device) if nws else None
        streams = 7 if mfma_bf16 else 8
        with _timed("window_attn_bwd", qkv.device, streams * B * N * C * qkv.element_size(), 10 * B * N * C * ws):
            check(lib.hs_window_attn_bwd(ptr(qkv), ptr(out), ptr(dout), ptr(lse), ptr(dqkv), ptr(dbias), ptr(dscale), ptr(wsp),
                                         ptr(bias_c), ptr(hs), ptr(idx), roll, ptr(labels),
                                         B, N, C, nh, ws, flags, ctx.drop[0], ctx.drop[1], dt, stream_ptr(qkv.device)),
                  "hs_window_attn_bwd")
        dbias_out = None if dbias is None else dbias.to(ctx.bias_dtype)
        sdt, sshape = ctx.scale_meta
        dscale_out = dscale.to(sdt).reshape(sshape) if (flags & _lib.HS_ATTN_COSINE) else None
        return dqkv, dbias_out, dscale_out, None, None, None, None, None, None, None, None, None


def window_attn_core(qkv, bias, head_scale, idx, roll, labels, num_heads, window_size, cosine, attn_drop=0.0, seed=None):
    if attn_drop > 0.0 and seed is None:
        seed = int(torch.randint(0, 2 ** 62, (1,)).item())
    return WindowAttnCoreFn.apply(qkv, bias, head_scale, idx, roll, labels, num_heads, window_size, cosine,
                                  float(attn_drop), int(seed or 0))


COMP_RESIDUAL = os.environ.get("HS_COMP_RESIDUAL", "0") == "1"
COMP_RESIDUAL_LAST_STAGE = False


FUSED_ATTN_MODULE = True


def window_attn_module_ok(x, num_heads, window_size):
    return (FUSED_ATTN_MODULE and x.is_cuda and x.dtype == torch.bfloat16 and not torch.is_grad_enabled() and
            bool(lib.hs_window_attn_module_supported(x.shape[-1], num_heads, window_size, _lib.HS_BF16)))


def window_attn_module(x, qkv_w, qkv_b, proj_w, proj_b, bias, head_scale, idx, roll, labels, num_heads, window_size, cosine,
                       ln_weight=None, ln_bias=None, residual=False):
    _require_gpu(x, qkv_w, proj_w, bias, head_scale, idx, labels)
    B, N, C = x.shape
    x = x.contiguous()
    out = torch.empty_like(x)
    wq, wp = _cast_param(qkv_w, torch.bfloat16).contiguous(), _cast_param(proj_w, torch.bfloat16).contiguous()
    hs = _f32(head_scale).reshape(-1)
    flags = (_lib.HS_ATTN_COSINE if cosine else 0) | (_lib.HS_ATTN_RESIDUAL if residual else 0)
    nbytes = (3 if residual else 2) * B * N * C * 2
    flops = B * N * (8 * C * C + 4 * window_size * C)
    with _timed("window_attn_module_fwd", x.device, nbytes, flops):
        check(lib.hs_window_attn_module_fwd(ptr(x), ptr(out), ptr(wq), ptr(_f32(qkv_b)), ptr(wp), ptr(_f32(proj_b)), ptr(_f32(ln_weight)),
                                            ptr(_f32(ln_bias)), ptr(_f32(bias)), ptr(hs), ptr(idx), int(roll), ptr(labels), B, N, C,
                                            num_heads, window_size, flags, _lib.HS_BF16, stream_ptr(x.device)),
              "hs_window_attn_module_fwd")
    return out


FUSED_ATTN_MODULE_TRAIN = os.environ.get("HS_FUSED_ATTN_TRAIN", "1") != "0"
FUSED_NORM2 = False


def window_attn_module_train_ok(x, num_heads, window_size):
    return (FUSED_ATTN_MODULE_TRAIN and x.is_cuda and x.dtype == torch.bfloat16 and torch.is_grad_enabled() and
            not FORCE_VALU_ATTENTION and bool(lib.hs_window_attn_module_supported(x.shape[-1], num_heads, window_size, _lib.HS_BF16)))


def window_attn_module_train(x, ln_weight, ln_bias, qkv_w, qkv_b, proj_w, proj_b, bias, head_scale, idx, roll, labels, num_heads,
                             window_size, cosine, residual_alias=False, norm2=None):
    _require_gpu(x, qkv_w, proj_w, bias, head_scale, idx, labels)
    B, N, C = x.shape
    x = x.contiguous()
    dev = x.device
    has_ln = ln_weight is not None
    out, o = torch.empty_like(x), torch.empty_like(x)
    xn = torch.empty_like(x) if has_ln else None
    qkv = torch.empty((B, N, 3 * C), dtype=x.dtype, device=dev)
    mean = torch.empty(B * N, dtype=torch.float32, device=dev) if has_ln else None
    rstd = torch.empty(B * N, dtype=torch.float32, device=dev) if has_ln else None
    lse = torch.empty((B, num_heads, N), dtype=torch.float32, device=dev)
    n2 = mean2 = rstd2 = None
    if norm2 is not None:
        assert has_ln and not residual_alias
        n2 = torch.empty_like(x)
        mean2 = torch.empty(B * N, dtype=torch.float32, device=dev)
        rstd2 = torch.empty(B * N, dtype=torch.float32, device=dev)
    wq, wp = _cast_param(qkv_w, torch.bfloat16).contiguous(), _cast_param(proj_w, torch.bfloat16).contiguous()
    hs = _f32(head_scale).reshape(-1)
    flags = (_lib.HS_ATTN_COSINE if cosine else 0) | (_lib.HS_ATTN_RESIDUAL if has_ln else 0)
    with _timed("window_attn_module_fwd_train", dev, ((9 if has_ln else 6) + (1 if n2 is not None else 0)) * B * N * C * 2,
                B * N * (8 * C * C + 4 * window_size * C)):
        check(lib.hs_window_attn_module_fwd_train(ptr(x), ptr(out), ptr(xn), ptr(mean), ptr(rstd), ptr(qkv), ptr(o), ptr(lse), ptr(wq),
                                                  ptr(_f32(qkv_b)), ptr(wp), ptr(_f32(proj_b)), ptr(_f32(ln_weight)), ptr(_f32(ln_bias)),
                                                  ptr(_f32(bias)), ptr(hs), ptr(idx), int(roll), ptr(labels),
                                                  ptr(None if n2 is None else _f32(norm2[0])), ptr(None if n2 is None else _f32(norm2[1])),
                                                  ptr(n2), ptr(mean2), ptr(rstd2), B, N, C, num_heads,
                                                  window_size, flags, _lib.HS_BF16, stream_ptr(dev)),
              "hs_window_attn_module_fwd_train")
    if not has_ln:
        x_res = None
        if residual_alias:
            qkv_t, x_res = LinearFn.apply(x, qkv_w, qkv_b, True, None, (qkv,))
        else:
            qkv_t = LinearFn.apply(x, qkv_w, qkv_b, False, None, (qkv,))
        o_t = WindowAttnCoreFn.apply(qkv_t, bias, head_scale, idx, roll, labels, num_heads, window_size, cosine, 0.0, 0, (o, lse))
        y = LinearFn.apply(o_t, proj_w, proj_b, False, None, (out,))
        return (y, x_res) if residual_alias else y
    assert not residual_alias
    n1, xs = LayerNormFn.apply(x, ln_weight, ln_bias, None, None, True, None, False, (xn, mean, rstd))
    qkv_t = LinearFn.apply(n1, qkv_w, qkv_b, False, None, (qkv,))
    o_t = WindowAttnCoreFn.apply(qkv_t, bias, head_scale, idx, roll, labels, num_heads, window_size, cosine, 0.0, 0, (o, lse))
    x1 = LinearFn.apply(o_t, proj_w, proj_b, False, xs, (out,))
    if n2 is None:
        return x1
    return LayerNormFn.apply(x1, norm2[0], norm2[1], None, None, True, None, False, (n2, mean2, rstd2))
```

heal_swin_amd/ops/gemm.py:

```python
import math
import os

import torch

from .. import _lib
from .._lib import check, lib, ptr, stream_ptr
from . import runtime
from .runtime import RT, _aligned, _cast_param, _defer_flag, _defer_keep, _require_gpu, _sink_buffer, _timed


OWN_GEMM = os.environ.get("HS_OWN_GEMM", "auto")


OWN_GELU_MAX_K = 4096
OWN_DGELU_MAX_K = 1024
OWN_BIAS_MAX_K = 0


class GemmTuner:
    MIN_FLOP = 1 << 33

    def __init__(self):
        self.picks = {}
        self.trials = {}

    @staticmethod
    def key(m, n, k):
        return (max(1, int(m)).bit_length(), int(n), int(k))

    def pick(self, m, n, k, device):
        key = self.key(m, n, k)
        if key in self.picks:
            return self.picks[key]
        if 2 * m * n * k < self.MIN_FLOP or not torch.cuda.is_available() or torch.cuda.is_current_stream_capturing():
            return None
        try:
            return self._trial(key, m, n, k, device)
        except Exception:
            self.picks[key] = None
            return None

    def _trial(self, key, m, n, k, device):
        with torch.no_grad():
            g = torch.Generator(device=device).manual_seed(1)
            sets = [(torch.randn((m, k), generator=g, device=device).to(torch.bfloat16),
                     (torch.randn((n, k), generator=g, device=device) * k ** -0.5).to(torch.bfloat16)) for _ in range(2)]
            bias32 = torch.zeros(n, device=device)
            bias16 = bias32.to(torch.bfloat16)
            best = {True: float("inf"), False: float("inf")}
            for rep in range(4):
                for own in (True, False):
                    a, w = sets[rep & 1]
                    e0, e1 = torch.cuda.Event(enable_timing=True), torch.cuda.Event(enable_timing=True)
                    e0.record()
                    if own:
                        gemm_nt(a, w, bias32)
                    else:
                        torch.nn.functional.linear(a, w, bias16)
                    e1.record()
                    e1.synchronize()
                    if rep:
                        best[own] = min(best[own], e0.elapsed_time(e1))
            del sets
        self.trials[key] = (round(1e3 * best[True], 1), round(1e3 * best[False], 1))
        self.picks[key] = best[True] <= best[False]
        return self.picks[key]


GEMM_TUNE = True
GEMM_TUNER = GemmTuner()


def own_gemm_ok(epi, n, k, dtype, k2=0, m=None):
    if dtype != torch.bfloat16 or OWN_GEMM == "0" or k % 8 or k2 % 8 or n % 8 or n < 16:
        return False
    if OWN_GEMM == "1" or RT.prefer_own_gemm:
        return True
    kk = k + k2
    if epi == _lib.HS_EPI_DGELU:
        return kk <= OWN_DGELU_MAX_K
    if epi == _lib.HS_EPI_GELU:
        return kk <= OWN_GELU_MAX_K
    if OWN_BIAS_MAX_K > 0:
        return kk <= OWN_BIAS_MAX_K
    if GEMM_TUNE and m is not None and k2 == 0 and torch.cuda.is_available():
        pick = GEMM_TUNER.pick(int(m), n, kk, torch.device("cuda", torch.cuda.current_device()))
        if pick is not None:
            return pick
    return kk <= 128 or n <= 128 or (n <= 256 and kk <= 256)


RESID_DGRAD_OWN = True


def own_gemm_legal(n, k, dtype):
    return dtype == torch.bfloat16 and OWN_GEMM != "0" and k % 8 == 0 and n % 8 == 0 and n >= 16


RESID_EPILOGUE = True


def gemm_nt(a2d, w, bias=None, epi=0, aux=None, a2=None, w2=None, want_c=True, drop_p=0.0, seed=0):
    w, w2, bias = _aligned(w), _aligned(w2), _aligned(bias)
    if epi != _lib.HS_EPI_GELU:
        aux = _aligned(aux)
    m, k = a2d.shape
    n = w.shape[0]
    assert a2d.stride(1) == 1 and w.stride(1) == 1 and a2d.dtype == torch.bfloat16 and w.dtype == torch.bfloat16
    c = torch.empty((m, n), dtype=torch.bfloat16, device=a2d.device) if want_c else None
    if epi == _lib.HS_EPI_GELU:
        aux = torch.empty((m, n), dtype=torch.bfloat16, device=a2d.device)
    k2 = 0 if a2 is None else a2.shape[1]
    if bias is not None and bias.dtype != torch.float32:
        bias = bias.float()
    with _timed(f"hs_gemm_nt epi={epi} m={m} n={n} k={k + k2}", a2d.device, 2 * (m * (k + k2) + n * (k + k2) + m * n * (2 if (epi and want_c) else 1)), 2 * m * n * (k + k2)):
        check(lib.hs_gemm_nt(ptr(a2d), a2d.stride(0), ptr(w), w.stride(0), k, ptr(a2), 0 if a2 is None else a2.stride(0), ptr(w2),
                             0 if w2 is None else w2.stride(0), k2, ptr(bias), ptr(c), ptr(aux), m, n, epi, float(drop_p), int(seed),
                             _lib.HS_BF16, stream_ptr(a2d.device)), "hs_gemm_nt")
    return c, aux


def _lib_tag(kind, m, n, k):
    return f"lib {kind} m={m} n={n} k={k}"


FP32_GEMM = os.environ.get("HS_FP32_GEMM", "bf16x3")
_BF16X3_MIN = 160
_SPLIT_MEMO = []
_MM_OUT_DTYPE = [None]


def _bf16x3_ok(x, n=None, k=None):
    ok = FP32_GEMM == "bf16x3" and x.dtype == torch.float32 and x.is_cuda and x.shape[-1] % 8 == 0
    ok = ok and (n is None or n * k >= _BF16X3_MIN * (n + k))
    if ok and _MM_OUT_DTYPE[0] is None:
        _probe_mm_out_dtype(x.device)
    return ok and _MM_OUT_DTYPE[0] is not False


def _probe_mm_out_dtype(device):
    try:
        a = torch.zeros((8, 8), dtype=torch.bfloat16, device=device)
        torch.mm(a, a, out_dtype=torch.float32)
        _MM_OUT_DTYPE[0] = True
    except Exception:
        _MM_OUT_DTYPE[0] = False
        import warnings
        warnings.warn("heal_swin_amd: torch.mm(..., out_dtype=) is unavailable in this PyTorch build; fp32 Linear products run as "
                      "exact fp32 GEMMs (HS_FP32_GEMM=strict behaviour) instead of bf16x3")


def split3(x2d, mode):
    x2d = x2d.contiguous()
    key = (x2d.data_ptr(), tuple(x2d.shape), x2d._version, mode)
    for kk, _, t in _SPLIT_MEMO:
        if kk == key:
            return t
    rows, k = x2d.shape
    out = torch.empty((rows, 3 * k), dtype=torch.bfloat16, device=x2d.device)
    check(lib.hs_split_bf16x3(ptr(x2d), ptr(out), rows, k, mode, stream_ptr(x2d.device)), "hs_split_bf16x3")
    if mode == 0:
        _SPLIT_MEMO.append((key, x2d, out))
        del _SPLIT_MEMO[:-2]
    return out


class _Split:

    def __init__(self, t3, k):
        self.t3, self.shape, self.dtype, self.device = t3, (t3.shape[0], k), torch.float32, t3.device

    def is_contiguous(self):
        return True

    def record_stream(self, stream):
        self.t3.record_stream(stream)

    def dim(self):
        return 2


def _split_of(x2d):
    if isinstance(x2d, _Split):
        return x2d.t3
    if x2d is None or x2d.dtype != torch.float32:
        return None
    key = (x2d.data_ptr(), tuple(x2d.shape), x2d._version, 0)
    for kk, _, t in _SPLIT_MEMO:
        if kk == key:
            return t
    return None


_WSPLIT = {}
_WSPLIT_CAPACITY = 1024


def _weight_split(w2d, transposed):
    key = (w2d.untyped_storage().data_ptr(), w2d.storage_offset(), tuple(w2d.shape), tuple(w2d.stride()), bool(transposed))
    hit = _WSPLIT.get(key)
    if hit is not None and hit[0] == w2d._version and hit[1] == RT.weight_epoch:
        return hit[3]
    src = w2d.t().contiguous() if transposed else w2d.contiguous()
    rows, k = src.shape
    out = torch.empty((rows, 3 * k), dtype=torch.bfloat16, device=src.device)
    check(lib.hs_split_bf16x3(ptr(src), ptr(out), rows, k, 1, stream_ptr(src.device)), "hs_split_bf16x3")
    if len(_WSPLIT) >= _WSPLIT_CAPACITY:
        for old in list(_WSPLIT)[:_WSPLIT_CAPACITY // 2]:
            del _WSPLIT[old]
    _WSPLIT[key] = (w2d._version, RT.weight_epoch, w2d.detach(), out)
    return out


def _mm_f32(a3, b3t, bias=None):
    if _MM_OUT_DTYPE[0] is None:
        _probe_mm_out_dtype(a3.device)
    if not _MM_OUT_DTYPE[0]:
        raise RuntimeError("HS_FP32_GEMM=bf16x3 needs torch.mm(..., out_dtype=torch.float32); set HS_FP32_GEMM=strict")
    if bias is None:
        return torch.mm(a3, b3t, out_dtype=torch.float32)
    if _MM_OUT_DTYPE[0] is True:
        try:
            y = torch.addmm(bias, a3, b3t, out_dtype=torch.float32)
            _MM_OUT_DTYPE[0] = "addmm"
            return y
        except Exception:
            _MM_OUT_DTYPE[0] = "mm"
    if _MM_OUT_DTYPE[0] == "addmm":
        return torch.addmm(bias, a3, b3t, out_dtype=torch.float32)
    return torch.mm(a3, b3t, out_dtype=torch.float32).add_(bias)


def _lib_linear(x2, w, b):
    if isinstance(x2, _Split):
        m, k = x2.shape
        with _timed(_lib_tag("fwd bf16x3", m, w.shape[0], 3 * k), x2.device, 4 * (m * k + m * w.shape[0]), 6 * m * k * w.shape[0]):
            return _mm_f32(x2.t3, _weight_split(w.reshape(w.shape[0], k), False).t(), b)
    m, k = x2.shape[0] if x2.dim() == 2 else x2.numel() // x2.shape[-1], x2.shape[-1]
    if _bf16x3_ok(x2, w.shape[0], k) and w.dtype == torch.float32 and w.shape[0] % 8 == 0:
        with _timed(_lib_tag("fwd bf16x3", m, w.shape[0], 3 * k), x2.device, 4 * (m * k + m * w.shape[0]), 6 * m * k * w.shape[0]):
            y = _mm_f32(split3(x2.reshape(m, k), 0), _weight_split(w.reshape(w.shape[0], k), False).t(), b)
        return y.view(x2.shape[:-1] + (w.shape[0],))
    with _timed(_lib_tag("fwd", m, w.shape[0], k), x2.device, 2 * (m * k + m * w.shape[0]), 2 * m * k * w.shape[0]):
        return torch.nn.functional.linear(x2, w, b)


def _lib_matmul(dy2, w, res=None):
    m, n = dy2.shape
    if isinstance(dy2, _Split):
        with _timed(_lib_tag("dgrad bf16x3", m, w.shape[1], 3 * n), dy2.device, 4 * (m * n + m * w.shape[1]), 6 * m * n * w.shape[1]):
            return _mm_f32(dy2.t3, _weight_split(w, True).t(), res)
    if _bf16x3_ok(dy2, w.shape[1], n) and w.dtype == torch.float32 and w.shape[1] % 8 == 0:
        with _timed(_lib_tag("dgrad bf16x3", m, w.shape[1], 3 * n), dy2.device, 4 * (m * n + m * w.shape[1]), 6 * m * n * w.shape[1]):
            dx = _mm_f32(split3(dy2, 0), _weight_split(w, True).t(), res)
        return dx
    with _timed(_lib_tag("dgrad", m, w.shape[1], n), dy2.device, 2 * (m * n + m * w.shape[1]), 2 * m * n * w.shape[1]):
        return dy2 @ w if res is None else torch.addmm(res, dy2, w)


def _cast_param_t(p, dtype, cache=None):
    if cache is None:
        cache = RT.cast_cache if RT.cast_cache is not None else RT.last_cast_cache
    c = cache.get_t(p, dtype) if (cache is not None and p.dim() == 2 and cache.current(p)) else None
    if c is None:
        n_out = p.shape[0]
        c = p.detach().to(dtype).view(n_out, -1).t().contiguous()
    return c


def _wgrad_group_ok(dy2, x2, n_out, k_in, want_b, bbuf, x3):
    return bool(runtime.WGRAD_GROUP and x3 is None and x2 is not None and x2.dtype == torch.bfloat16 and dy2.dtype == torch.bfloat16 and
                (bbuf is not None or not want_b) and _defer_flag(dy2.device) and
                lib.hs_linear_wgrad_group_variant(dy2.shape[0], n_out, k_in, _lib.HS_BF16) == 1)


def _wgrad_issue(members, dev):
    rows = members[0][0].shape[0]
    arr = _lib.wgrad_problems(members)
    ws = torch.empty(int(lib.hs_linear_wgrad_group_workspace(arr, len(members), rows, _lib.HS_BF16)), dtype=torch.float32, device=dev)
    with _timed("linear_wgrad" if len(members) == 1 else "linear_wgrad group", dev, sum(2 * rows * (m[4] + m[5]) for m in members),
                sum(2 * rows * m[4] * m[5] for m in members)):
        check(lib.hs_linear_wgrad_group(arr, len(members), ptr(ws), rows, _lib.HS_BF16, stream_ptr(dev)), "hs_linear_wgrad_group")
    _defer_keep(dev, ws)


def _wgrad_grouped(member):
    dev = member[0].device
    s = torch.cuda.current_stream(dev).cuda_stream
    parked = runtime._PARKED.pop(s, None)
    if parked is not None and parked[0].shape[0] == member[0].shape[0]:
        _wgrad_issue([parked, member], dev)
        return
    if parked is not None:
        _wgrad_issue([parked], dev)
    runtime._PARKED[s] = member


def _wgrad_flush_parked(s, device=None):
    parked = runtime._PARKED.pop(s, None)
    if parked is not None:
        _wgrad_issue([parked], parked[0].device)


runtime._PARK_FLUSH[:] = [_wgrad_flush_parked]


def _param_grads(dy2, x2, weight, bias, want_w, want_b, x3=None, gelu_x=False):
    n_out = weight.shape[0]
    k_in = weight.numel() // n_out
    if not (want_w or want_b):
        return None, None
    if x2 is None:
        assert x3 is not None and dy2.dtype == torch.float32
        hip_ok = dy2.is_contiguous() and n_out % 8 == 0
        assert hip_ok
    else:
        hip_ok = (x2.is_contiguous() and dy2.is_contiguous() and n_out % 4 == 0 and
                  ((x2.dtype == torch.bfloat16 and k_in % 8 == 0) or (x2.dtype == torch.float32 and k_in % 4 == 0)))
    wbuf = _sink_buffer(weight) if (hip_ok and want_w) else None
    bbuf = _sink_buffer(bias) if (wbuf is not None and want_b) else None
    if wbuf is not None and (not want_b or bbuf is not None):
        aw = RT.async_wgrad
        wbuf = wbuf.view(n_out, k_in)
        if aw is not None:
            cur = torch.cuda.current_stream(dy2.device)
            aw.stream.wait_stream(cur)
            dy2.record_stream(aw.stream)
            (x2 if x2 is not None else x3).record_stream(aw.stream)
            with torch.cuda.stream(aw.stream):
                LinearFn._wgrad_hip(dy2, x2, n_out, k_in, want_b, wbuf, bbuf, x3, gelu_x)
        elif _wgrad_group_ok(dy2, x2, n_out, k_in, want_b, bbuf, x3):
            _wgrad_grouped((dy2, x2, wbuf, bbuf if want_b else None, n_out, k_in, 1 | _lib.HS_ACC_DEFER, gelu_x))
        else:
            LinearFn._wgrad_hip(dy2, x2, n_out, k_in, want_b, wbuf, bbuf, x3, gelu_x)
        RT.grad_sink.deposited(weight)
        if want_b:
            RT.grad_sink.deposited(bias)
        return None, None
    dw = db = None
    if hip_ok:
        dw32, db32 = LinearFn._wgrad_hip(dy2, x2, n_out, k_in, want_b, x3=x3, gelu_x=gelu_x)
        dw = dw32.to(weight.dtype).view(weight.shape) if want_w else None
        db = db32.to(bias.dtype) if want_b else None
    else:
        assert not gelu_x
        if want_w:
            dw = (dy2.t() @ x2).to(weight.dtype).view(weight.shape)
        if want_b:
            db = dy2.sum(0).to(bias.dtype)
    return dw, db


class LinearFn(torch.autograd.Function):

    @staticmethod
    def forward(ctx, x, weight, bias, passthrough=False, residual=None, pre=None):
        _require_gpu(x, weight, bias, residual)
        n_out = weight.shape[0]
        k_in = weight.numel() // n_out
        w = _cast_param(weight, x.dtype).view(n_out, k_in)
        ctx.x_shape = x.shape
        ctx.bias_param = bias
        ctx.w_cast = w if w.dtype != weight.dtype else None
        ctx.cast_cache = RT.cast_cache
        ctx.passthrough = passthrough
        ctx.has_residual = residual is not None
        ctx.x3 = None
        if pre is not None:
            y = pre[0]
        elif residual is not None:
            assert not passthrough
            if own_gemm_legal(n_out, k_in, x.dtype) and x.is_contiguous():
                res2 = residual.reshape(-1, n_out)
                res2 = res2 if res2.is_contiguous() else res2.contiguous()
                y = gemm_nt(x.reshape(-1, k_in), w, bias, _lib.HS_EPI_RESID, aux=res2)[0].view(x.shape[:-1] + (n_out,))
            else:
                y = _lib_linear(x, w, None if bias is None else _cast_param(bias, x.dtype)) + residual
                ctx.x3 = _split_of(x.reshape(-1, k_in)) if x.is_contiguous() else None
        elif own_gemm_ok(_lib.HS_EPI_BIAS, n_out, k_in, x.dtype, m=x.numel() // k_in) and x.is_contiguous():
            y = gemm_nt(x.reshape(-1, k_in), w, bias)[0].view(x.shape[:-1] + (n_out,))
        else:
            y = _lib_linear(x, w, None if bias is None else _cast_param(bias, x.dtype))
            ctx.x3 = _split_of(x.reshape(-1, k_in)) if x.is_contiguous() else None
        ctx.save_for_backward(None if ctx.x3 is not None else x, weight)
        return (y, x.view_as(x)) if passthrough else y

    @staticmethod
    def _wgrad_hip(dy2, x2, n_out, k_in, want_b, dw_out=None, db_out=None, x3=None, gelu_x=False):
        rows = dy2.shape[0]
        dev = dy2.device
        accumulate = 1 if dw_out is not None else 0
        defer = _defer_flag(dev) if (dw_out is not None and (db_out is not None or not want_b)) else 0
        dw32 = dw_out if dw_out is not None else torch.empty((n_out, k_in), dtype=torch.float32, device=dev)
        db32 = None
        if want_b:
            db32 = db_out if db_out is not None else torch.empty(n_out, dtype=torch.float32, device=dev)
        nws = int(lib.hs_linear_wgrad_workspace(rows, n_out, k_in))
        ws = torch.empty(nws, dtype=torch.float32, device=dev)
        if x3 is not None or (_bf16x3_ok(x2, n_out, k_in) and n_out % 8 == 0 and x2.dtype == dy2.dtype):
            dy3 = dy2.t3 if isinstance(dy2, _Split) else split3(dy2, 0)
            x3 = x3 if x3 is not None else split3(x2, 0)
            aw = RT.async_wgrad
            if aw is not None and torch.cuda.current_stream(dev) == aw.stream:
                dy3.record_stream(aw.stream)
                x3.record_stream(aw.stream)
            with _timed("linear_wgrad bf16x3", dev, 3 * 2 * rows * (n_out + k_in), 6 * rows * n_out * k_in):
                for i, (yo, xo, dbp) in enumerate(((0, 0, db32), (0, 2 * k_in, None), (2 * n_out, 0, db32))):
                    d = defer if i == 2 else 0
                    check(lib.hs_linear_wgrad_ld(ptr(dy3), 3 * n_out, yo, ptr(x3), 3 * k_in, xo, ptr(dw32), ptr(dbp), ptr(ws), rows,
                                                 n_out, k_in, (1 if (accumulate or i) else 0) | d, stream_ptr(dev)), "hs_linear_wgrad_ld")
                if defer:
                    _defer_keep(dev, ws)
            return dw32, db32
        with _timed("linear_wgrad", dev, x2.element_size() * rows * (n_out + k_in), 2 * rows * n_out * k_in):
            if gelu_x:
                check(lib.hs_linear_wgrad_gelu(ptr(dy2), ptr(x2), ptr(dw32), ptr(db32), ptr(ws), rows, n_out, k_in, accumulate | defer,
                                               _lib.dtype_code(x2.dtype), stream_ptr(dev)), "hs_linear_wgrad_gelu")
            else:
                check(lib.hs_linear_wgrad(ptr(dy2), ptr(x2), ptr(dw32), ptr(db32), ptr(ws), rows, n_out, k_in, accumulate | defer,
                                          _lib.dtype_code(x2.dtype), stream_ptr(dev)), "hs_linear_wgrad")
        if defer:
            _defer_keep(dev, ws)
        return dw32, db32

    @staticmethod
    def backward(ctx, dy, dx_res=None):
        x, weight = ctx.saved_tensors
        bias = ctx.bias_param
        n_out = weight.shape[0]
        k_in = weight.numel() // n_out
        if dy is None:
            return dx_res, None, None, None, None, None
        dy2 = dy.reshape(-1, n_out)
        x2 = None if x is None else x.reshape(-1, k_in)
        if not dy2.is_contiguous():
            dy2 = dy2.contiguous()
        dx = None
        if ctx.needs_input_grad[0]:
            dx = _input_grad(dy2, weight, ctx.w_cast, None if dx_res is None else dx_res.reshape(-1, k_in), ctx.cast_cache).reshape(ctx.x_shape)
        ctx.w_cast = ctx.cast_cache = None
        x3, ctx.x3 = ctx.x3, None
        dw, db = _param_grads(dy2, x2, weight, bias, ctx.needs_input_grad[1], bias is not None and ctx.needs_input_grad[2], x3)
        return dx, dw, db, None, (dy if ctx.has_residual else None), None


def _input_grad(dy2, weight, w_cast, dx_res2=None, cache=None):
    n_out = weight.shape[0]
    k_in = weight.numel() // n_out
    epi = _lib.HS_EPI_BIAS if dx_res2 is None else _lib.HS_EPI_RESID
    if own_gemm_ok(epi, k_in, n_out, dy2.dtype, m=dy2.shape[0]) or (dx_res2 is not None and RESID_DGRAD_OWN and own_gemm_legal(k_in, n_out, dy2.dtype)):
        res = None if dx_res2 is None else dx_res2.to(dy2.dtype).contiguous()
        return gemm_nt(dy2, _cast_param_t(weight, dy2.dtype, cache), None, epi, aux=res)[0]
    w = w_cast if (w_cast is not None and w_cast.dtype == dy2.dtype) else (
        weight if weight.dtype == dy2.dtype else weight.to(dy2.dtype)).view(n_out, k_in)
    if dx_res2 is not None:
        return _lib_matmul(dy2, w, dx_res2.to(dy2.dtype))
    return _lib_matmul(dy2, w)


def linear(x, weight, bias=None):
    return LinearFn.apply(x, weight, bias)


def linear_residual(x, weight, bias, residual):
    return LinearFn.apply(x, weight, bias, False, residual)


def linear_passthrough(x, weight, bias=None):
    return LinearFn.apply(x, weight, bias, True)




class PadSliceFn(torch.autograd.Function):

    @staticmethod
    def forward(ctx, x, n):
        ctx.shape, ctx.n = x.shape, n
        return x[..., :n]

    @staticmethod
    def backward(ctx, g):
        full = RT.zero_padded_grads.pop(g.data_ptr(), None)
        if (full is not None and g._base is full and full.numel() == math.prod(ctx.shape) and full.dtype == g.dtype and
                g.shape == ctx.shape[:-1] + (ctx.n,) and g.stride() == full.view(ctx.shape)[..., :ctx.n].stride()):
            return full.view(ctx.shape), None
        out = g.new_zeros(ctx.shape)
        out[..., :ctx.n] = g
        return out, None


def pad_slice(x, n):
    return PadSliceFn.apply(x, n)
```

heal_swin_amd/ops/mlp_branch.py:

```python
import os

import torch

from .. import _lib
from .._lib import check, lib, ptr, stream_ptr
from .runtime import RT, _cast_param, _defer_flag, _defer_keep, _draw_seed, _extras, _f32, _require_gpu, _timed
from .norm import _norm_param_grads, _norm_param_result
from .gemm import (_Split, _bf16x3_ok, _cast_param_t, _input_grad, _lib_linear, _lib_matmul, _param_grads, _split_of, gemm_nt, own_gemm_legal, own_gemm_ok)


class MlpFn(torch.autograd.Function):

    @staticmethod
    def forward(ctx, x, w1, b1, w2, b2, drop_p, seed, passthrough, residual=None):
        _require_gpu(x, w1, b1, w2, b2, residual)
        c_in, hid = w1.shape[1], w1.shape[0]
        x2 = x.reshape(-1, c_in)
        if not x2.is_contiguous():
            x2 = x2.contiguous()
        dt = x.dtype
        x3 = a3 = None
        w1c, w2c = _cast_param(w1, dt), _cast_param(w2, dt)
        need_grad = any(ctx.needs_input_grad[:5])
        if own_gemm_ok(_lib.HS_EPI_GELU, hid, c_in, dt):
            h, a = gemm_nt(x2, w1c, b1, _lib.HS_EPI_GELU, want_c=need_grad, drop_p=drop_p, seed=seed)
        else:
            h = _lib_linear(x2, w1c, None if b1 is None else _cast_param(b1, dt))
            x3 = _split_of(x2)
            if _bf16x3_ok(h, w2.shape[0], hid) and w2c.dtype == torch.float32 and w2.shape[0] % 8 == 0 and hid % 8 == 0:
                a3 = torch.empty((h.shape[0], 3 * hid), dtype=torch.bfloat16, device=h.device)
                check(lib.hs_gelu_split3(None, ptr(h), ptr(a3), h.shape[0], hid, float(drop_p), int(seed), stream_ptr(h.device)),
                      "hs_gelu_split3")
                a = _Split(a3, hid)
            else:
                a = torch.empty_like(h)
                check(lib.hs_gelu_fwd(ptr(h), ptr(a), h.numel(), float(drop_p), int(seed), _lib.dtype_code(dt), stream_ptr(h.device)),
                      "hs_gelu_fwd")
        ctx.has_residual = residual is not None
        if residual is not None and own_gemm_legal(w2.shape[0], hid, dt):
            res2 = residual.reshape(-1, w2.shape[0])
            y = gemm_nt(a, w2c, b2, _lib.HS_EPI_RESID, aux=res2 if res2.is_contiguous() else res2.contiguous())[0]
        elif own_gemm_ok(_lib.HS_EPI_BIAS, w2.shape[0], hid, dt):
            y = gemm_nt(a, w2c, b2)[0]
        else:
            y = _lib_linear(a, w2c, None if b2 is None else _cast_param(b2, dt))
            a3 = _split_of(a)
            if isinstance(a, _Split):
                a = None
        if residual is not None and not own_gemm_legal(w2.shape[0], hid, dt):
            y = y + residual.reshape(-1, w2.shape[0])
        assert not isinstance(a, _Split)
        ctx.save_for_backward(None if x3 is not None else x2, h, None if a3 is not None else a, w1, w2)
        ctx.biases = (b1, b2)
        ctx.casts = (w1c if w1c.dtype != w1.dtype else None, w2c if w2c.dtype != w2.dtype else None)
        ctx.cast_cache = RT.cast_cache
        ctx.meta = (float(drop_p), int(seed), x.shape)
        ctx.splits = (x3, a3)
        y = y.view(x.shape[:-1] + (w2.shape[0],))
        return (y, x.view_as(x)) if passthrough else y

    @staticmethod
    def backward(ctx, dy, dx_res=None):
        x2, h, a, w1, w2 = ctx.saved_tensors
        b1, b2 = ctx.biases
        w1c, w2c = ctx.casts
        p, seed, xshape = ctx.meta
        if dy is None:
            return dx_res, None, None, None, None, None, None, None, None
        c_out, hid, c_in = w2.shape[0], w1.shape[0], w1.shape[1]
        dy2 = dy.reshape(-1, c_out)
        if not dy2.is_contiguous():
            dy2 = dy2.contiguous()
        dt = dy2.dtype
        if own_gemm_ok(_lib.HS_EPI_DGELU, hid, c_out, dt):
            dh = gemm_nt(dy2, _cast_param_t(w2, dt, ctx.cast_cache), None, _lib.HS_EPI_DGELU, aux=h, drop_p=p, seed=seed)[0]
        else:
            da = _lib_matmul(dy2, w2c if (w2c is not None and w2c.dtype == dt) else w2.to(dt))
            if _bf16x3_ok(da, c_in, hid) and w1.dtype == torch.float32 and c_in % 8 == 0 and hid % 8 == 0:
                dh3 = torch.empty((h.shape[0], 3 * hid), dtype=torch.bfloat16, device=h.device)
                check(lib.hs_gelu_split3(ptr(da), ptr(h), ptr(dh3), h.shape[0], hid, p, seed, stream_ptr(h.device)), "hs_gelu_split3")
                dh = _Split(dh3, hid)
            else:
                dh = torch.empty_like(h)
                check(lib.hs_gelu_bwd(ptr(da), ptr(h), ptr(dh), h.numel(), p, seed, _lib.dtype_code(dt), stream_ptr(h.device)), "hs_gelu_bwd")
            del da
        dx = None
        if ctx.needs_input_grad[0]:
            dx = _input_grad(dh, w1, w1c, None if dx_res is None else dx_res.reshape(-1, c_in), ctx.cast_cache).reshape(xshape)
        ctx.casts = ctx.cast_cache = None
        (x3, a3), ctx.splits = ctx.splits, (None, None)
        dw2, db2 = _param_grads(dy2, a, w2, b2, ctx.needs_input_grad[3], b2 is not None and ctx.needs_input_grad[4], a3)
        dw1, db1 = _param_grads(dh, x2, w1, b1, ctx.needs_input_grad[1], b1 is not None and ctx.needs_input_grad[2], x3)
        return dx, dw1, db1, dw2, db2, None, None, None, (dy if ctx.has_residual else None)


def mlp(x, w1, b1, w2, b2, drop_p=0.0, seed=None, passthrough=False, residual=None):
    if drop_p > 0.0 and seed is None:
        seed = _draw_seed()
    return MlpFn.apply(x, w1, b1, w2, b2, float(drop_p), int(seed or 0), bool(passthrough), residual)


FUSED_MLP = os.environ.get("HS_FUSED_MLP", "1") != "0"
MLP_KEEP_ACT = True


def fused_mlp_ok(x, hidden):
    c = x.shape[-1]
    return bool(FUSED_MLP and x.is_cuda and x.dtype == torch.bfloat16 and (x.numel() // c) % 32 == 0 and
                lib.hs_mlp_fused_supported(int(c), int(hidden), _lib.HS_BF16))


class FusedMlpBlockFn(torch.autograd.Function):

    @staticmethod
    def forward(ctx, x, ln_w, ln_b, w1, b1, w2, b2, post_norm=False, stoch=None):
        _require_gpu(x, ln_w, ln_b, w1, b1, w2, b2)
        assert stoch is None or post_norm
        C, hid = x.shape[-1], w1.shape[0]
        x2 = x.reshape(-1, C)
        if not x2.is_contiguous():
            x2 = x2.contiguous()
        rows = x2.shape[0]
        dev = x.device
        need = any(ctx.needs_input_grad)
        w1c, w2c = _cast_param(w1, torch.bfloat16).contiguous(), _cast_param(w2, torch.bfloat16).contiguous()
        g, b = _f32(ln_w), _f32(ln_b)
        out = torch.empty_like(x2)
        n = torch.empty_like(x2) if need else None
        mean = torch.empty(rows, dtype=torch.float32, device=dev) if need else None
        rstd = torch.empty(rows, dtype=torch.float32, device=dev) if need else None
        h = torch.empty((rows, hid), dtype=x.dtype, device=dev) if need else None
        keep_act = need and (MLP_KEEP_ACT or (stoch is not None and stoch[2] > 0) or
                             not lib.hs_linear_wgrad_gelu_supported(rows, C, hid, _lib.HS_BF16))
        act = torch.empty((rows, hid), dtype=x.dtype, device=dev) if keep_act else None
        flags = _lib.HS_ATTN_RESIDUAL | (_lib.HS_MLP_NORM_AFTER if post_norm else 0)
        with _timed("mlp_fused_fwd", dev, 2 * rows * ((3 if need else 2) * C + ((2 if keep_act else 1) * hid if need else 0)), 4 * rows * C * hid):
            if stoch is None:
                check(lib.hs_mlp_fused_fwd(ptr(x2), ptr(g), ptr(b), ptr(w1c), ptr(_f32(b1)), ptr(w2c), ptr(_f32(b2)), ptr(n), ptr(mean), ptr(rstd),
                                           ptr(h), ptr(act), ptr(out), rows, C, hid, flags, _lib.HS_BF16, stream_ptr(dev)),
                      "hs_mlp_fused_fwd")
            else:
                rs, rps, dp, seed_h, seed_o = stoch
                check(lib.hs_mlp_fused_drop_fwd(ptr(x2), ptr(g), ptr(b), ptr(w1c), ptr(_f32(b1)), ptr(w2c), ptr(_f32(b2)), ptr(n), ptr(mean),
                                                ptr(rstd), ptr(h), ptr(act), ptr(out), ptr(rs), rps, dp, seed_h, seed_o, rows, C, hid, flags,
                                                _lib.HS_BF16, stream_ptr(dev)), "hs_mlp_fused_drop_fwd")
        ctx.stoch = stoch
        ctx.save_for_backward(x2, n, mean, rstd, h, act, g, w1, w2)
        ctx.params = (ln_w, ln_b, b1, b2)
        ctx.cast_cache = RT.cast_cache
        ctx.x_shape = x.shape
        ctx.post_norm = bool(post_norm)
        return out.view(x.shape)

    @staticmethod
    def backward(ctx, dout):
        x2, n, mean, rstd, h, act, g, w1, w2 = ctx.saved_tensors
        ln_w, ln_b, b1, b2 = ctx.params
        rows, C = x2.shape
        hid = w1.shape[0]
        dev = x2.device
        dy2 = dout.reshape(rows, C)
        if not dy2.is_contiguous():
            dy2 = dy2.contiguous()
        w2t = _cast_param_t(w2, torch.bfloat16, ctx.cast_cache)
        w1t = _cast_param_t(w1, torch.bfloat16, ctx.cast_cache)
        ctx.cast_cache = None
        dgamma, dbeta, direct = _norm_param_grads(ln_w, ln_b, C, dev, ctx.needs_input_grad[1] and ctx.needs_input_grad[2])
        ws = torch.empty(int(lib.hs_layernorm_bwd_workspace(rows, C)), dtype=torch.float32, device=dev)
        acc = (1 | _defer_flag(dev)) if direct else 0
        dh = torch.empty_like(h)
        if ctx.post_norm:
            dm = torch.empty_like(x2)
            stoch = ctx.stoch
            if stoch is None:
                check(lib.hs_layernorm_bwd(ptr(dy2), ptr(n), ptr(g), ptr(mean), ptr(rstd), ptr(dm), ptr(dgamma), ptr(dbeta), ptr(ws), acc, rows, C,
                                           _lib.HS_BF16, stream_ptr(dev)), "hs_layernorm_bwd")
            else:
                rs, rps, dp, seed_h, seed_o = stoch
                check(lib.hs_layernorm_drop_bwd(ptr(dy2), ptr(n), ptr(g), ptr(mean), ptr(rstd), ptr(dm), ptr(dgamma), ptr(dbeta), ptr(ws), acc,
                                                ptr(rs), rps, dp, seed_o, rows, C, _lib.HS_BF16, stream_ptr(dev)), "hs_layernorm_drop_bwd")
            dx = torch.empty_like(x2)
            with _timed("mlp_fused_bwd", dev, 2 * rows * (3 * C + 2 * hid), 4 * rows * C * hid):
                if stoch is None:
                    check(lib.hs_mlp_fused_bwd(ptr(dm), ptr(h), ptr(w2t), ptr(w1t), ptr(dy2), ptr(dh), ptr(dx), rows, C, hid, _lib.HS_BF16,
                                               stream_ptr(dev)), "hs_mlp_fused_bwd")
                else:
                    check(lib.hs_mlp_fused_drop_bwd(ptr(dm), ptr(h), ptr(w2t), ptr(w1t), ptr(dy2), ptr(dh), ptr(dx), dp, seed_h, rows, C, hid,
                                                    _lib.HS_BF16, stream_ptr(dev)), "hs_mlp_fused_drop_bwd")
            dw2, db2 = _param_grads(dm, h if act is None else act, w2, b2, ctx.needs_input_grad[5], b2 is not None and ctx.needs_input_grad[6],
                                    gelu_x=act is None)
            dw1, db1 = _param_grads(dh, x2, w1, b1, ctx.needs_input_grad[3], b1 is not None and ctx.needs_input_grad[4])
        else:
            dn = torch.empty_like(x2)
            with _timed("mlp_fused_bwd", dev, 2 * rows * (2 * C + 2 * hid), 4 * rows * C * hid):
                check(lib.hs_mlp_fused_bwd(ptr(dy2), ptr(h), ptr(w2t), ptr(w1t), None, ptr(dh), ptr(dn), rows, C, hid, _lib.HS_BF16,
                                           stream_ptr(dev)), "hs_mlp_fused_bwd")
            dw2, db2 = _param_grads(dy2, h if act is None else act, w2, b2, ctx.needs_input_grad[5], b2 is not None and ctx.needs_input_grad[6],
                                    gelu_x=act is None)
            dw1, db1 = _param_grads(dh, n, w1, b1, ctx.needs_input_grad[3], b1 is not None and ctx.needs_input_grad[4])
            dx = torch.empty_like(x2)
            check(lib.hs_add_layernorm_bwd(ptr(dn), ptr(dy2), ptr(x2), ptr(g), ptr(mean), ptr(rstd), ptr(dx), ptr(dgamma), ptr(dbeta), ptr(ws),
                                           acc, rows, C, _lib.HS_BF16, stream_ptr(dev)), "hs_add_layernorm_bwd")
        if acc & _lib.HS_ACC_DEFER:
            _defer_keep(dev, ws)
        dlw, dlb = _norm_param_result(ln_w, ln_b, dgamma, dbeta, direct)
        return dx.view(ctx.x_shape), dlw, dlb, dw1, db1, dw2, db2, None, None


def fused_mlp_block(x, ln_w, ln_b, w1, b1, w2, b2, post_norm=False, row_scale=None, drop_p=0.0, seeds=None):
    stoch = None
    if row_scale is not None or drop_p:
        ex = _extras(x, row_scale, drop_p, 0)
        seed_h, seed_o = seeds if seeds is not None else ((_draw_seed(), _draw_seed()) if drop_p else (0, 0))
        stoch = (ex[0], ex[1], ex[2], int(seed_h), int(seed_o))
    return FusedMlpBlockFn.apply(x, ln_w, ln_b, w1, b1, w2, b2, bool(post_norm), stoch)


def fused_mlp_stochastic_ok(x, post_norm):
    return bool(post_norm) and (x.numel() // x.shape[-1] // x.shape[0]) % 32 == 0
```

heal_swin_amd/ops/norm.py:

```python

import torch

from .. import _lib
from .._lib import check, lib, ptr, stream_ptr
from .runtime import RT, _aligned, _defer_flag, _defer_keep, _draw_seed, _extras, _f32, _require_gpu, _sink_buffer


def _norm_param_grads(weight, bias, width, device, want):
    wbuf = _sink_buffer(weight) if want else None
    bbuf = _sink_buffer(bias) if wbuf is not None else None
    if wbuf is not None and bbuf is not None:
        return wbuf.view(-1), bbuf.view(-1), True
    return (torch.empty(width, dtype=torch.float32, device=device), torch.empty(width, dtype=torch.float32, device=device), False)


def _norm_param_result(weight, bias, dgamma, dbeta, direct):
    if not direct:
        return dgamma.to(weight.dtype), dbeta.to(bias.dtype)
    RT.grad_sink.deposited(weight)
    RT.grad_sink.deposited(bias)
    return None, None


def _norm_backward(weight, bias, want, rows, width, device, call):
    dgamma, dbeta, direct = _norm_param_grads(weight, bias, width, device, want)
    ws = torch.empty(int(lib.hs_layernorm_bwd_workspace(rows, width)), dtype=torch.float32, device=device)
    acc = (1 | _defer_flag(device)) if direct else 0
    call(ptr(dgamma), ptr(dbeta), ptr(ws), acc)
    if acc & _lib.HS_ACC_DEFER:
        _defer_keep(device, ws)
    return _norm_param_result(weight, bias, dgamma, dbeta, direct)


class LayerNormFn(torch.autograd.Function):

    @staticmethod
    def forward(ctx, x, weight, bias, residual, extras, passthrough=False, res_lo=None, want_lo=False, pre=None):
        _require_gpu(x, weight, bias, residual)
        ctx.set_materialize_grads(False)
        x = _aligned(x.contiguous())
        width = x.shape[-1]
        rows = x.numel() // width
        dt = _lib.dtype_code(x.dtype)
        g, b = _f32(weight), _f32(bias)
        res = None if residual is None else _aligned(residual.contiguous())
        if res is not None:
            assert res.shape == x.shape and res.dtype == x.dtype
        y_lo = None
        if pre is None:
            y = torch.empty_like(x)
            need_grad = any(ctx.needs_input_grad[:3])
            mean = torch.empty(rows, dtype=torch.float32, device=x.device) if need_grad else None
            rstd = torch.empty(rows, dtype=torch.float32, device=x.device) if need_grad else None
        if pre is not None:
            assert res is None and extras is None and not want_lo and res_lo is None
            y, mean, rstd = pre
        else:
            assert not (passthrough and want_lo) and (res is not None or res_lo is None)
            y_lo = torch.empty_like(x) if want_lo else None
            rs, rps, p, seed = extras if extras is not None else (None, 1, 0.0, 0)
            check(lib.hs_layernorm_fwd_ex(ptr(x), ptr(res), None, ptr(None if res_lo is None else _aligned(res_lo.contiguous())), ptr(g), ptr(b),
                                          ptr(y), None, ptr(y_lo), ptr(mean), ptr(rstd), ptr(rs), rps, p, seed, rows, width, dt,
                                          stream_ptr(x.device)), "hs_layernorm_fwd_ex")
        ctx.save_for_backward(x, g, mean, rstd, None if extras is None else extras[0])
        ctx.meta = (rows, width, dt, residual is not None, extras)
        ctx.params = (weight, bias)
        ctx.second_is_alias = bool(passthrough)
        assert not passthrough or (extras is None and residual is None)
        if want_lo:
            ctx.mark_non_differentiable(y_lo)
            return y, y_lo
        return (y, x.view_as(x)) if passthrough else y

    @staticmethod
    def backward(ctx, dy, dx_alias=None):
        x, g, mean, rstd, rs = ctx.saved_tensors
        rows, width, dt, has_res, extras = ctx.meta
        weight, bias = ctx.params
        if not ctx.second_is_alias:
            dx_alias = None
        if dy is None:
            return dx_alias, None, None, None, None, None, None, None, None
        dy = _aligned(dy.contiguous())
        dx = torch.empty_like(x)

        def call(dgamma, dbeta, ws, acc):
            if dx_alias is not None:
                check(lib.hs_add_layernorm_bwd(ptr(dy), ptr(_aligned(dx_alias.contiguous())), ptr(x), ptr(g), ptr(mean), ptr(rstd), ptr(dx),
                                               dgamma, dbeta, ws, acc, rows, width, dt, stream_ptr(x.device)), "hs_add_layernorm_bwd")
            else:
                _, rps, p, seed = extras if extras is not None else (None, 1, 0.0, 0)
                check(lib.hs_layernorm_drop_bwd(ptr(dy), ptr(x), ptr(g), ptr(mean), ptr(rstd), ptr(dx), dgamma, dbeta, ws, acc, ptr(rs),
                                                rps, p, seed, rows, width, dt, stream_ptr(x.device)), "hs_layernorm_drop_bwd")

        dw, db = _norm_backward(weight, bias, ctx.needs_input_grad[1] and ctx.needs_input_grad[2], rows, width, x.device, call)
        return dx, dw, db, (dy if has_res else None), None, None, None, None, None


def layer_norm(x, weight, bias, residual=None, row_scale=None, drop_p=0.0, seed=None):
    return LayerNormFn.apply(x, weight, bias, residual, _extras(x, row_scale, drop_p, seed))


def layer_norm_hilo(x, weight, bias):
    return LayerNormFn.apply(x, weight, bias, None, None, False, None, True)


def layer_norm_stream(x, weight, bias, residual, res_lo=None, row_scale=None, drop_p=0.0, seed=None):
    return LayerNormFn.apply(x, weight, bias, residual, _extras(x, row_scale, drop_p, seed), False, res_lo, True)


def layer_norm_passthrough(x, weight, bias):
    return LayerNormFn.apply(x, weight, bias, None, None, True)


class AddLayerNormFn(torch.autograd.Function):

    @staticmethod
    def forward(ctx, a, b, weight, bias, extras, a_lo=None, want_lo=False):
        _require_gpu(a, b, weight, bias)
        a, b = _aligned(a.contiguous()), _aligned(b.contiguous())
        assert a.shape == b.shape and a.dtype == b.dtype
        width = a.shape[-1]
        rows = a.numel() // width
        dt = _lib.dtype_code(a.dtype)
        g, be = _f32(weight), _f32(bias)
        s = torch.empty_like(a)
        y = torch.empty_like(a)
        mean = torch.empty(rows, dtype=torch.float32, device=a.device)
        rstd = torch.empty(rows, dtype=torch.float32, device=a.device)
        s_lo = torch.empty_like(a) if want_lo else None
        rs, rps, p, seed = extras if extras is not None else (None, 1, 0.0, 0)
        check(lib.hs_layernorm_fwd_ex(ptr(a), None, ptr(b), ptr(None if a_lo is None else _aligned(a_lo.contiguous())), ptr(g), ptr(be), ptr(y),
                                      ptr(s), ptr(s_lo), ptr(mean), ptr(rstd), ptr(rs), rps, p, seed, rows, width, dt,
                                      stream_ptr(a.device)), "hs_layernorm_fwd_ex")
        ctx.save_for_backward(s, g, mean, rstd, None if extras is None else extras[0])
        ctx.meta = (rows, width, dt, extras)
        ctx.params = (weight, bias)
        if want_lo:
            ctx.mark_non_differentiable(s_lo)
            return s, y, s_lo
        return s, y

    @staticmethod
    def backward(ctx, ds, dy, ds_lo=None):
        s, g, mean, rstd, rs = ctx.saved_tensors
        rows, width, dt, extras = ctx.meta
        weight, bias = ctx.params
        if dy is None:
            if extras is None:
                return ds, ds, None, None, None, None, None
            dy = torch.zeros_like(s)
        dy = _aligned(dy.contiguous())
        ds_c = None if ds is None else _aligned(ds.contiguous())
        da = torch.empty_like(s)
        db = da if extras is None else torch.empty_like(s)

        def call(dgamma, dbeta, ws, acc):
            if extras is None:
                check(lib.hs_add_layernorm_bwd(ptr(dy), ptr(ds_c), ptr(s), ptr(g), ptr(mean), ptr(rstd), ptr(da), dgamma, dbeta, ws, acc,
                                               rows, width, dt, stream_ptr(s.device)), "hs_add_layernorm_bwd")
            else:
                _, rps, p, seed = extras
                check(lib.hs_add_layernorm_drop_bwd(ptr(dy), ptr(ds_c), ptr(s), ptr(g), ptr(mean), ptr(rstd), ptr(da), ptr(db), dgamma, dbeta,
                                                    ws, acc, ptr(rs), rps, p, seed, rows, width, dt, stream_ptr(s.device)),
                      "hs_add_layernorm_drop_bwd")

        dw, dbias = _norm_backward(weight, bias, ctx.needs_input_grad[2] and ctx.needs_input_grad[3], rows, width, s.device, call)
        return da, db, dw, dbias, None, None, None


def add_layer_norm(a, b, weight, bias, row_scale=None, drop_p=0.0, seed=None):
    return AddLayerNormFn.apply(a, b, weight, bias, _extras(a, row_scale, drop_p, seed))


def add_layer_norm_stream(a, a_lo, b, weight, bias, row_scale=None, drop_p=0.0, seed=None):
    return AddLayerNormFn.apply(a, b, weight, bias, _extras(a, row_scale, drop_p, seed), a_lo, True)


class GeluDropoutFn(torch.autograd.Function):

    @staticmethod
    def forward(ctx, x, p, seed):
        _require_gpu(x)
        x = _aligned(x.contiguous())
        y = torch.empty_like(x)
        dt = _lib.dtype_code(x.dtype)
        check(lib.hs_gelu_fwd(ptr(x), ptr(y), x.numel(), float(p), int(seed), dt, stream_ptr(x.device)), "hs_gelu_fwd")
        ctx.save_for_backward(x)
        ctx.meta = (float(p), int(seed), dt)
        return y

    @staticmethod
    def backward(ctx, dy):
        (x,) = ctx.saved_tensors
        p, seed, dt = ctx.meta
        dy = _aligned(dy.contiguous())
        dx = torch.empty_like(x)
        check(lib.hs_gelu_bwd(ptr(dy), ptr(x), ptr(dx), x.numel(), p, seed, dt, stream_ptr(x.device)), "hs_gelu_bwd")
        return dx, None, None


class ResidualDropFn(torch.autograd.Function):

    @staticmethod
    def forward(ctx, x, t, row_scale, p, seed):
        _require_gpu(x, t, row_scale)
        x, t = _aligned(x.contiguous()), _aligned(t.contiguous())
        assert x.shape == t.shape and x.dtype == t.dtype
        rs = None if row_scale is None else row_scale.detach().to(torch.float32).contiguous()
        eps = t.numel() // t.shape[0]
        out = torch.empty_like(t)
        dt = _lib.dtype_code(t.dtype)
        check(lib.hs_residual_drop(ptr(x), ptr(t), ptr(out), ptr(rs), eps, t.numel(), float(p), int(seed), dt, stream_ptr(t.device)),
              "hs_residual_drop")
        ctx.save_for_backward(rs)
        ctx.meta = (eps, float(p), int(seed), dt)
        return out

    @staticmethod
    def backward(ctx, dy):
        (rs,) = ctx.saved_tensors
        eps, p, seed, dt = ctx.meta
        dy = _aligned(dy.contiguous())
        dtv = torch.empty_like(dy)
        check(lib.hs_residual_drop(None, ptr(dy), ptr(dtv), ptr(rs), eps, dy.numel(), p, seed, dt, stream_ptr(dy.device)),
              "hs_residual_drop (backward)")
        return dy, dtv, None, None, None


def residual_drop(x, t, row_scale=None, p=0.0, seed=None):
    if p > 0.0 and seed is None:
        seed = _draw_seed()
    return ResidualDropFn.apply(x, t, row_scale, float(p), int(seed or 0))


def gelu_dropout(x, p=0.0, seed=None):
    if p > 0.0 and seed is None:
        seed = _draw_seed()
    return GeluDropoutFn.apply(x, float(p), int(seed or 0))
```

include/healswin.h:

```cpp
#ifndef HEALSWIN_H
#define HEALSWIN_H

#include <stdint.h>

#ifdef __cplusplus
extern "C" {
#endif

typedef enum {
    HS_OK = 0,
    HS_ERR_INVALID_ARG = 1,
    HS_ERR_UNSUPPORTED = 2,
    HS_ERR_HIP = 3,
    HS_ERR_NOT_PERMUTATION = 4,
    HS_ERR_MISALIGNED = 5
} hs_status;

typedef enum { HS_F32 = 0, HS_BF16 = 1 } hs_dtype;

#define HS_ATTN_COSINE 1u
#define HS_ATTN_FORCE_VALU 2u
#define HS_ATTN_RESIDUAL 4u
#define HS_ATTN_OVERWRITE_GRADS 8u

// ... 59 lines not shown
                       const int32_t* idx, int64_t roll, const uint8_t* labels,
                       int batch, int64_t n_tokens, int channels, int num_heads, int window_size,
                       unsigned flags, float attn_drop, uint64_t seed, int dtype, void* stream);

int hs_gather_rows(const void* x, void* out, const int32_t* idx, int64_t roll,
                   int batch, int64_t n_tokens, int64_t row_bytes, void* stream);

int hs_layernorm_fwd(const void* x, const void* residual, const float* gamma, const float* beta,
                     void* y, float* mean, float* rstd,
                     int64_t rows, int width, int dtype, void* stream);
int64_t hs_layernorm_bwd_workspace(int64_t rows, int width);
int hs_layernorm_bwd(const void* dy, const void* x, const float* gamma, const float* mean, const float* rstd,
                     void* dx, float* dgamma, float* dbeta, float* workspace, int accumulate,
                     int64_t rows, int width, int dtype, void* stream);

int hs_add_layernorm_fwd(const void* a, const void* b, const float* gamma, const float* beta,
                         void* sum_out, void* y, float* mean, float* rstd,
                         int64_t rows, int width, int dtype, void* stream);
int hs_add_layernorm_bwd(const void* dy, const void* dsum, const void* sum, const float* gamma,
                         const float* mean, const float* rstd, void* dx, float* dgamma, float* dbeta, float* workspace,
                         int accumulate, int64_t rows, int width, int dtype, void* stream);

int hs_layernorm_drop_fwd(const void* x, const void* residual, const float* gamma, const float* beta, void* y,
                          float* mean, float* rstd, const float* row_scale, int64_t rows_per_sample, float drop_p,
                          uint64_t seed, int64_t rows, int width, int dtype, void* stream);
int hs_layernorm_drop_bwd(const void* dy, const void* x, const float* gamma, const float* mean, const float* rstd,
                          void* dx, float* dgamma, float* dbeta, float* workspace, int accumulate, const float* row_scale,
                          int64_t rows_per_sample, float drop_p, uint64_t seed, int64_t rows, int width, int dtype,
                          void* stream);
int hs_add_layernorm_drop_fwd(const void* a, const void* b, const float* gamma, const float* beta, void* sum_out, void* y,
                              float* mean, float* rstd, const float* row_scale, int64_t rows_per_sample, float drop_p,
                              uint64_t seed, int64_t rows, int width, int dtype, void* stream);
int hs_layernorm_fwd_ex(const void* x, const void* residual, const void* add_in, const void* lo_in, const float* gamma,
                        const float* beta, void* y, void* sum_out, void* lo_out, float* mean, float* rstd,
                        const float* row_scale, int64_t rows_per_sample, float drop_p, uint64_t seed, int64_t rows, int width,
                        int dtype, void* stream);
int hs_add_layernorm_drop_bwd(const void* dy, const void* dsum, const void* sum, const float* gamma, const float* mean,
                              const float* rstd, void* da, void* db, float* dgamma, float* dbeta, float* workspace, int accumulate,
                              const float* row_scale, int64_t rows_per_sample, float drop_p, uint64_t seed,
                              int64_t rows, int width, int dtype, void* stream);

int hs_gelu_fwd(const void* x, void* y, int64_t n, float drop_p, uint64_t seed, int dtype, void* stream);
int hs_gelu_bwd(const void* dy, const void* x, void* dx, int64_t n, float drop_p, uint64_t seed, int dtype, void* stream);

int hs_residual_drop(const void* x, const void* t, void* out, const float* row_scale, int64_t elems_per_sample, int64_t n,
                     float drop_p, uint64_t seed, int dtype, void* stream);

int64_t hs_seg_ce_partials(int64_t batch, int64_t npix);
int hs_seg_ce_fwd(const void* logits, const void* labels, const float* class_weights, float* partials,
                  int64_t batch, int64_t npix, int n_classes, int64_t stride_b, int64_t stride_k, int64_t stride_p,
                  int label_bytes, int64_t ignore_index, int dtype, void* stream);
int hs_seg_ce_bwd(const void* logits, const void* labels, const float* class_weights, const float* scale, void* dlogits,
                  int64_t batch, int64_t npix, int n_classes, int64_t stride_b, int64_t stride_k, int64_t stride_p,
                  int64_t dstride_b, int64_t dstride_k, int64_t dstride_p, int label_bytes, int64_t ignore_index,
                  int dtype, void* stream);

#define HS_DEPTH_L1 0
#define HS_DEPTH_L2 1
#define HS_DEPTH_HUBER 2
#define HS_DEPTH_LOGVAR 3
int64_t hs_depth_loss_partials(int64_t batch, int64_t npix);
int hs_depth_loss_fwd(const void* pred, const float* target, float* partials, int64_t batch, int64_t npix, int channels,
                      int64_t stride_b, int64_t stride_c, int64_t stride_p, int kind, float huber_delta, int dtype, void* stream);
int hs_depth_loss_bwd(const void* pred, const float* target, const float* scale, void* dpred, int64_t batch, int64_t npix, int channels,
                      int64_t stride_b, int64_t stride_c, int64_t stride_p, int64_t dstride_b, int64_t dstride_c, int64_t dstride_p,
                      int kind, float huber_delta, int dtype, void* stream);

int64_t hs_linear_wgrad_workspace(int64_t rows, int n_out, int k_in);
int hs_linear_wgrad(const void* dy, const void* x, float* dw, float* dbias, float* workspace,
                    int64_t rows, int n_out, int k_in, int accumulate, int dtype, void* stream);
int hs_linear_wgrad_gelu_supported(int64_t rows, int n_out, int k_in, int dtype);
int hs_linear_wgrad_gelu(const void* dy, const void* h, float* dw, float* dbias, float* workspace, int64_t rows, int n_out, int k_in,
                         int accumulate, int dtype, void* stream);
typedef struct hs_wgrad_problem {
    const void* dy;
    const void* x;
    float* dw;
    float* dbias;
    int n_out, k_in, accumulate, gelu_x;
} hs_wgrad_problem;
int hs_linear_wgrad_group_variant(int64_t rows, int n_out, int k_in, int dtype);
int64_t hs_linear_wgrad_group_workspace(const hs_wgrad_problem* problems, int count, int64_t rows, int dtype);
int hs_linear_wgrad_group(const hs_wgrad_problem* problems, int count, float* workspace, int64_t rows, int dtype, void* stream);

#define HS_ACC_DEFER 2
int hs_reduce_pending(void* stream);
int hs_reduce_flush(void* stream);

#define HS_MLP_NORM_AFTER 16u
int hs_mlp_fused_supported(int channels, int hidden, int dtype);
int hs_mlp_fused_fwd(const void* x, const float* ln_gamma, const float* ln_beta, const void* w1, const float* b1, const void* w2,
                     const float* b2, void* n_out, float* mean_out, float* rstd_out, void* h_out, void* act_out, void* out, int64_t rows,
                     int channels, int hidden, unsigned flags, int dtype, void* stream);
int hs_mlp_fused_bwd(const void* dy, const void* h, const void* w2_t, const void* w1_t, const void* dres, void* dh, void* dn, int64_t rows,
                     int channels, int hidden, int dtype, void* stream);
int hs_mlp_fused_drop_fwd(const void* x, const float* ln_gamma, const float* ln_beta, const void* w1, const float* b1, const void* w2,
                          const float* b2, void* m_out, float* mean_out, float* rstd_out, void* h_out, void* act_out, void* out,
                          const float* row_scale, int64_t rows_per_sample, float drop_p, uint64_t seed_hidden, uint64_t seed_out,
                          int64_t rows, int channels, int hidden, unsigned flags, int dtype, void* stream);
int hs_mlp_fused_drop_bwd(const void* dy, const void* h, const void* w2_t, const void* w1_t, const void* dres, void* dh, void* dn,
                          float drop_p, uint64_t seed_hidden, int64_t rows, int channels, int hidden, int dtype, void* stream);

int hs_adam_step(float* p, const float* g, float* m, float* v, void* p_bf16, int64_t n, float lr, const float* lr_dev, float beta1,
                 float beta2, float eps, float weight_decay, int decoupled, const int64_t* step, void* stream);
int hs_adam_advance(int64_t* step, void* stream);

typedef struct {
    float total_norm;
    float clip_coef;
    int32_t finite;
    int32_t reserved;
} hs_grad_guard;
int hs_grad_guard_piece(void);
int hs_grad_stats(const float* g, int64_t n, const int64_t* items, int n_items, double* partials, void* stream);
int hs_grad_guard_finalize(const double* partials, int64_t n_items, const int32_t* params, int n_params, int norm_inf, float max_norm,
                           float* param_norm, double* work, hs_grad_guard* guard, void* stream);
int hs_adam_step_guarded(float* p, const float* g, float* m, float* v, void* p_bf16, int64_t n, float lr, const float* lr_dev, float beta1,
                         float beta2, float eps, float weight_decay, int decoupled, const int64_t* step, float clip_value,
                         const hs_grad_guard* guard, int skip_nonfinite, void* stream);
int hs_adam_advance_guarded(int64_t* step, const hs_grad_guard* guard, int skip_nonfinite, int64_t* skipped, void* stream);
int hs_grad_scale(float* g, int64_t n, float clip_value, const hs_grad_guard* guard, void* stream);

int hs_window_attn_module_supported(int channels, int num_heads, int window_size, int dtype);
int hs_window_attn_module_fwd(const void* x, void* out, const void* qkv_w, const float* qkv_b, const void* proj_w,
                              const float* proj_b, const float* ln_gamma, const float* ln_beta, const float* bias,
                              const float* head_scale, const int32_t* idx, int64_t roll, const uint8_t* labels, int batch,
                              int64_t n_tokens, int channels, int num_heads, int window_size, unsigned flags, int dtype,
                              void* stream);

int hs_window_attn_module_fwd_train(const void* x, void* out, void* xn_out, float* mean_out, float* rstd_out, void* qkv_out,
                                    void* attn_out, float* lse_out, const void* qkv_w, const float* qkv_b, const void* proj_w,
                                    const float* proj_b, const float* ln_gamma, const float* ln_beta, const float* bias,
                                    const float* head_scale, const int32_t* idx, int64_t roll, const uint8_t* labels,
                                    const float* norm2_gamma, const float* norm2_beta, void* n2_out, float* mean2_out, float* rstd2_out,
                                    int batch, int64_t n_tokens, int channels, int num_heads, int window_size, unsigned flags, int dtype,
                                    void* stream);

int64_t hs_window_attn_module_bwd_chain_workspace(int batch, int64_t n_tokens, int channels, int num_heads, int window_size);
int hs_window_attn_module_bwd_chain(const void* dout, const void* x, const void* xn, const float* mean, const float* rstd, const void* qkv,
                              const void* attn_out, const float* lse, const void* qkv_w_t, const void* proj_w_t, const float* ln_gamma,
                              const float* bias, const float* head_scale, const int32_t* idx, int64_t roll, const uint8_t* labels,
                              void* dx, float* dqkv_w, float* dqkv_b, float* dproj_w, float* dproj_b, float* dln_gamma, float* dln_beta,
                              float* dbias, float* dhead_scale, float* workspace, int accumulate, int batch, int64_t n_tokens, int channels,
                              int num_heads, int window_size, unsigned flags, int dtype, void* stream);

#define HS_EPI_BIAS 0
#define HS_EPI_GELU 1
#define HS_EPI_DGELU 2
#define HS_EPI_RESID 3
int hs_gemm_nt(const void* a, int64_t lda, const void* b, int64_t ldb, int k, const void* a2, int64_t lda2, const void* b2,
               int64_t ldb2, int k2, const float* bias, void* c, void* aux, int64_t m, int n, int epilogue, float drop_p,
               uint64_t seed, int dtype, void* stream);
int hs_gemm_nt_set_tile(int variant);

int hs_pix2ang_nest(int nside, int64_t first, int64_t count, double* theta, double* phi);
int hs_sample_bilinear_u8(const void* img, int batch, int channels, int height, int width, const double* rx, const double* ry,
                          int64_t n, void* out, void* stream);
int hs_sample_mask_u8(const void* mask, int batch, int height, int width, const double* rx, const double* ry, int64_t n,
                      int background, void* out, void* stream);

#define HS_PRED_LABELS 2
#define HS_PRED_ROWS16 4
int hs_hp_interp_weights_nest(int nside, const double* theta, const double* phi, int64_t n, int64_t* pix, double* wgt);
int hs_backproject_labels(const void* pred, int pred_kind, int64_t batch, int64_t npix, int n_classes, int64_t stride_b,
                          int64_t stride_k, int64_t stride_p, const int32_t* nearest, int64_t n_out, int background, uint8_t* out,
                          void* stream);
int hs_backproject_image(const uint8_t* hp_img, int64_t planes, int64_t npix, const int32_t* idx, const double* wgt, int64_t n_out,
                         double* out, void* stream);
int hs_seg_confusion(const void* pred, int pred_kind, int64_t batch, int64_t npix, int n_classes, int64_t stride_b, int64_t stride_k,
                     int64_t stride_p, const int32_t* nearest, int64_t n_out, const uint8_t* target, int uncovered, int64_t* conf,
                     int64_t* bad, void* stream);

#define HS_F64 3
#define HS_DS_N 0
#define HS_DS_SE 1
#define HS_DS_AE 2
#define HS_DS_MEAN_SE 3
#define HS_DS_MEAN_AE 4
#define HS_DS_PRED 5
#define HS_DS_SIL_N 6
#define HS_DS_SIL_D 7
#define HS_DS_SIL_D2 8
#define HS_DS_INV_N 9
#define HS_DS_INV_SE 10
#define HS_DS_STD_N 11
#define HS_DS_STD 12
#define HS_DS_RANGE 13
#define HS_DEPTH_NSUMS 29
int64_t hs_depth_points_workspace(int64_t batch, int64_t n);
int hs_depth_points(const void* depth, int kind, int64_t batch, int64_t n, int64_t width, int64_t stride_b, int64_t stride_h,
                    int64_t stride_w, const uint8_t* foreground, int64_t fg_stride_b, const float* background, int n_background,
                    const double* dir, void* workspace, float* points, int64_t* offsets, void* stream);
int hs_chamfer_nn(const float* a, const int64_t* a_off, int64_t a_rows, int64_t a_max, const float* b, const int64_t* b_off,
                  int64_t b_rows, int64_t b_max, int64_t batch, int splits, void* workspace, float* dist_a, float* dist_b,
                  int64_t* idx_a, int64_t* idx_b, double* term, void* stream);
int64_t hs_depth_metrics_partials(int64_t total);
int hs_depth_metrics(const void* pred, int pred_kind, int64_t batch, int64_t n, int64_t width, int64_t stride_b, int64_t stride_c,
                     int64_t stride_h, int64_t stride_w, const void* target, int target_kind, int64_t t_stride_b, int64_t t_stride_h,
                     int64_t t_stride_w, int use_logvar, double total_mean, const float* ranges, int n_ranges, double* partial,
                     double* state, void* stream);
int hs_backproject_depth(const void* pred, int kind, int64_t batch, int64_t npix, int64_t stride_b, int64_t stride_p, const int32_t* idx,
                         const double* wgt, int64_t n_out, double* out, void* stream);

int hs_flat_depth_to_hp(const void* pred, int kind, int64_t batch, int64_t n_src, int64_t stride_b, int64_t stride_p, const int32_t* nearest,
                        const int32_t* idx, const float* wgt, int64_t n, float* out, void* stream);
int hs_depth_metrics_gather(const void* pred, int pred_kind, int64_t batch, int64_t n_src, int64_t stride_b, int64_t stride_c, int64_t stride_p,
                            const int32_t* nearest, const int32_t* idx, const float* wgt, int64_t n, const void* target, int target_kind,
                            int64_t t_stride_b, int64_t t_stride_p, int use_logvar, double total_mean, const float* ranges, int n_ranges,
                            double* partial, double* state, void* stream);

#define HS_DT_NONE 0
#define HS_DT_LOG 1
#define HS_DT_INV 2
#define HS_DT_ZERO_BKG 1
#define HS_DT_1000_BKG 2
#define HS_DT_AFFINE 4
#define HS_DT_INVERSE 8
#define HS_DSTAT_TOTAL 0
#define HS_DSTAT_BACKGROUND 1
#define HS_DSTAT_VALUES 2
#define HS_DSTAT_FINITE 3
#define HS_DSTAT_POSINF 4
#define HS_DSTAT_NEGINF 5
#define HS_DSTAT_NAN 6
#define HS_DSTAT_FG_VALUES 7
#define HS_DSTAT_FG_POSINF 8
#define HS_DSTAT_FG_NAN 9
#define HS_DSTAT_NCOUNTS 10
#define HS_DEPTH_STATS_WORDS 15
int hs_sample_bilinear_u8_f32(const void* img, int batch, int channels, int height, int width, const double* rx, const double* ry,
                              int64_t n, float* out, void* stream);
int hs_sample_nearest_f32(const float* src, int batch, int height, int width, const double* rx, const double* ry, int64_t n,
                          float background, float* out, void* stream);
int hs_depth_target(const float* in, int64_t in_stride_b, int64_t in_stride_p, float* out, int64_t out_stride_b, int64_t out_stride_p,
                    int64_t batch, int64_t n, int flags, int transform, float shift, float scale, void* stream);
int64_t hs_depth_stats_partials(int64_t n);
int hs_depth_stats_update(const float* depth, int64_t n, int transform, int use_masking, int64_t* partial, int64_t* state, void* stream);
int hs_depth_stats_merge(const int64_t* states, int count, int64_t* state, void* stream);

int hs_ln_head_supported(int width, int n_classes, int dtype);
int64_t hs_ln_head_partials(int64_t rows);
int hs_ln_head_fwd(const void* y, const void* wfold, const float* bvec, void* logits, float* mean, float* rstd, int64_t rows,
                   int width, int dtype, int logits_dtype, void* stream);
int hs_ln_head_bwd(const void* y, const float* mean, const float* rstd, const void* dlogits, const void* afold, void* dy,
                   void* dprime, float* partials, int64_t rows, int width, int dtype, int logits_dtype, void* stream);

int hs_split_bf16x3(const float* x, void* out, int64_t rows, int k, int mode, void* stream);
int hs_gelu_split3(const float* dy, const float* x, void* out3, int64_t rows, int k, float drop_p, uint64_t seed, void* stream);
int hs_linear_wgrad_ld(const void* dy, int64_t ldy, int64_t ycol0, const void* x, int64_t ldx, int64_t xcol0, float* dw, float* dbias,
                       float* workspace, int64_t rows, int n_out, int k_in, int accumulate, void* stream);

int hs_expand_ln_head_supported(int width, int children, int n_classes, int dtype);
int hs_expand_ln_head_fwd(const void* xn, const void* xn_lo, const void* wexp, const void* wfold, const float* bvec, void* y, float* logits,
                          float* mean, float* rstd, int64_t tokens, int width, int children, int dtype, void* stream);

int64_t hs_expand_ln_head_blocks(int64_t tokens);
int hs_expand_ln_head_ce_fwd(const void* xn, const void* xn_lo, const void* wexp, const void* wfold, const float* bvec, const uint8_t* labels,
                             const float* class_weights, int n_classes, void* y, float* logits, float* mean, float* rstd,
                             float* loss_partials, int64_t tokens, int width, int children, int dtype, void* stream);
int hs_expand_ln_head_ce_step_fwd(const void* xn, const void* xn_lo, const void* wexp, const void* wfold, const float* bvec,
                                  const uint8_t* labels, const float* class_weights, int n_classes, void* y, float* logits, float* mean,
                                  float* rstd, float* loss_partials, uint8_t* preds, int64_t* confmat, int64_t* bad, int64_t tokens,
                                  int width, int children, int dtype, void* stream);
int hs_ln_head_ce_bwd(const void* y, const float* mean, const float* rstd, const uint8_t* labels, const float* class_weights,
                      const float* scale, int n_classes, const void* wfold, const float* bvec, const void* afold, void* dy, void* dprime,
                      float* partials, int64_t rows, int width, int dtype, void* stream);

int hs_expand_ln_head_depth_fwd(const void* xn, const void* xn_lo, const void* wexp, const void* wfold, const float* bvec, const float* target,
                                int kind, float huber_delta, int n_out, void* y, float* logits, float* mean, float* rstd, float* loss_partials,
                                int64_t tokens, int width, int children, int dtype, void* stream);
int hs_expand_ln_head_depth_step_fwd(const void* xn, const void* xn_lo, const void* wexp, const void* wfold, const float* bvec,
                                     const float* target, int kind, float huber_delta, int n_out, void* y, float* logits, float* mean,
                                     float* rstd, float* loss_partials, int flags, int transform, float shift, float scale, int use_logvar,
                                     double total_mean, const float* ranges, int n_ranges, double* metric_partials, double* metric_state,
                                     float* preds, float* logvar_out, int64_t tokens, int width, int children, int dtype, void* stream);
int hs_ln_head_depth_bwd(const void* y, const float* mean, const float* rstd, const float* target, int kind, float huber_delta,
                         const float* scale, int n_out, const void* wfold, const float* bvec, const void* afold, void* dy, void* dprime,
                         float* partials, int64_t rows, int width, int dtype, void* stream);

int hs_patch_merge_fwd(const void* x, const float* gamma, const float* beta, const void* w, void* normed, float* mean, float* rstd,
                       void* out, int64_t rows, int dim, int dim_out, int dtype, void* stream);
int64_t hs_patch_merge_bwd_workspace(int64_t rows, int dim, int dim_out);
int hs_patch_merge_bwd(const void* dout, const void* x, const void* normed, const float* gamma, const float* mean, const float* rstd,
                       const void* w_t, void* dnormed, void* dx, float* dw, float* dgamma, float* dbeta, float* workspace,
                       int accumulate, int64_t rows, int dim, int dim_out, int dtype, void* stream);
int hs_patch_expand_fwd(const void* x, const void* w, const float* gamma, const float* beta, void* expanded, float* mean, float* rstd,
                        void* out, int64_t rows, int dim, int dim_exp, int children, int dtype, void* stream);
int64_t hs_patch_expand_bwd_workspace(int64_t rows, int dim, int dim_exp, int children);
int hs_patch_expand_bwd(const void* dout, const void* x, const void* expanded, const float* gamma, const float* mean, const float* rstd,
                        const void* w_t, void* dexpanded, void* dx, float* dw, float* dgamma, float* dbeta, float* workspace,
                        int accumulate, int64_t rows, int dim, int dim_exp, int children, int dtype, void* stream);

int hs_flat_zorder(int Ht, int Wt, int T, int32_t* z_of_rm, int32_t* rm_of_z);
int hs_build_flat_shift(int Ht, int Wt, int T, int w, int s, int32_t* idx, int32_t* inv, uint8_t* labels);
int hs_flat_rel_pos_index(int w, int64_t* row_major, int64_t* zorder);
int hs_flat_attn_mask(int Ht, int Wt, int w, int s, float* out);

#define HS_U8 8
#define HS_I32 9
#define HS_I64 10
#define HS_FLAT_PATCH_ROWS 0
#define HS_FLAT_PIXEL_ROWS 1
int hs_flat_img_to_rows(const void* img, int in_dtype, void* rows, int out_dtype, int batch, int nch, int H, int W, int p, int T,
                        int mode, int64_t ld, void* stream);
int hs_flat_rows_to_img(const void* rows, int in_dtype, void* img, int out_dtype, int batch, int nch, int H, int W, int p, int T,
                        int mode, int64_t ld, void* stream);
// ... 13 lines not shown
```

Baseline: 58.33.

## Fuse LayerNorm backward into the input-gradient GEMM epilogue

Measured after the change: 58.55, median of 6. About the same (+0.4%).

```diff
diff --git a/heal_swin_amd/_lib.py b/heal_swin_amd/_lib.py
--- a/heal_swin_amd/_lib.py
+++ b/heal_swin_amd/_lib.py
@@ -161,6 +161,8 @@
     "hs_gemm_nt": [c_ptr, c_i64, c_ptr, c_i64, c_int, c_ptr, c_i64, c_ptr, c_i64, c_int, c_ptr, c_ptr, c_ptr, c_i64, c_int, c_int,
                    ctypes.c_float, ctypes.c_uint64, c_int, c_ptr],
     "hs_gemm_nt_set_tile": [c_int],
+    "hs_gemm_nt_ln_bwd": [c_ptr, c_i64, c_ptr, c_i64, c_int, c_ptr, c_ptr, c_ptr, c_ptr, c_ptr, c_ptr, c_ptr, c_ptr, c_ptr, c_int, c_i64,
+                          c_int, c_int, c_ptr],
     "hs_set_reserved_cus": [c_int],
     "hs_transpose_many_16": [c_ptr, c_int, c_int, c_ptr],
     "hs_debug_occupy_cus": [c_int, c_int, c_int, ctypes.c_double, c_ptr],
@@ -188,6 +190,8 @@
     "hs_get_seed_epoch": ([], c_ptr),
     "hs_reduce_pending": ([c_ptr], c_int),
     "hs_layernorm_bwd_workspace": ([c_i64, c_int], c_i64),
+    "hs_gemm_nt_ln_bwd_workspace": ([c_int], c_i64),
+    "hs_gemm_nt_resident_grid": ([], c_int),
     "hs_seg_ce_partials": ([c_i64, c_i64], c_i64),
     "hs_depth_loss_partials": ([c_i64, c_i64], c_i64),
     "hs_depth_points_workspace": ([c_i64, c_i64], c_i64),
diff --git a/heal_swin_amd/csrc/gemm_nt.hip b/heal_swin_amd/csrc/gemm_nt.hip
--- a/heal_swin_amd/csrc/gemm_nt.hip
+++ b/heal_swin_amd/csrc/gemm_nt.hip
@@ -25,7 +25,7 @@
 #ifndef HS_GEMM_STAGGER_CYCLES
 #define HS_GEMM_STAGGER_CYCLES 40000
 #endif
-enum { EPI_BIAS = 0, EPI_GELU = 1, EPI_DGELU = 2, EPI_RESID = 3 };
+enum { EPI_BIAS = 0, EPI_GELU = 1, EPI_DGELU = 2, EPI_RESID = 3, EPI_LN_BWD = 4 };
 constexpr int64_t kMaxRecords = 0x7FFFFE00;
 
 struct GemmParams {
@@ -43,6 +43,9 @@
     int tiles_n, tiles, per_xcd, blocks_per_xcd;
     float drop_p;
     uint64_t seed;
+    const uint16_t* ln_x;
+    const float *ln_mean, *ln_rstd;
+    float* ln_part;
 #ifdef HS_GEMM_TRACE
     uint64_t* trace;
 #endif
@@ -95,7 +98,11 @@
     const int xcd = blockIdx.x & 7, lb = blockIdx.x >> 3;
     const int id_end = min((xcd + 1) * p.per_xcd, p.tiles);
     const int id0 = xcd * p.per_xcd + lb;
-    if (id0 >= id_end) return;
+    if (id0 >= id_end) {
+        if constexpr (EPI == EPI_LN_BWD)
+            for (int c = tid; c < 2 * p.n; c += NW * 64) p.ln_part[(size_t)blockIdx.x * (2 * p.n) + c] = 0.f;
+        return;
+    }
     const int nk1 = (p.k + 63) >> 6, nk2 = (p.k2 + 63) >> 6, nk = nk1 + nk2;
 #if HS_GEMM_EXP & 24
     {
@@ -526,6 +533,153 @@
         }
     };
 
+    float dg_acc = 0.f, db_acc = 0.f;
+    auto epilogue_ln = [&](int id, int buf_done, int slot_c) {
+        static_assert(EPI != EPI_LN_BWD || (ALIAS && FAST && TM == 2 && TN == 2 && BN == WN * 64), "EPI_LN_BWD: 64 x 64 wave tiles, patches in the stage buffer");
+        static_assert(EPI != EPI_LN_BWD || NW * 4096 + BM * WN * 8 <= STAGE, "EPI_LN_BWD: the row-sum records lie behind the patches");
+        const uint32_t patch_off = buf_done * STAGE;
+        __builtin_amdgcn_s_barrier();
+        const int64_t m0 = (int64_t)id * BM;
+        constexpr int n2 = BN * 2;
+        int64_t cbytes = (p.m - m0) * (int64_t)n2;
+        cbytes = cbytes > kMaxRecords ? kMaxRecords : cbytes;
+        const __amdgpu_buffer_rsrc_t rc = __builtin_amdgcn_make_buffer_rsrc((void*)(p.c + m0 * BN), 0, (int)cbytes, 0x00020000);
+        const __amdgpu_buffer_rsrc_t rxs = __builtin_amdgcn_make_buffer_rsrc((void*)(p.ln_x + m0 * BN), 0, (int)cbytes, 0x00020000);
+        const __amdgpu_buffer_rsrc_t rg = __builtin_amdgcn_make_buffer_rsrc((void*)(p.aux + m0 * BN), 0, (int)(p.aux ? cbytes : 0), 0x00020000);
+        const uint32_t rl_voff = (uint32_t)((lane >> 3) * n2 + (wn * 64 + (lane & 7) * 8) * 2);
+        auto row_soff = [&](int i, int t) -> int { return (wm * (BM / WM) + i * 32 + 8 * t) * n2; };
+        const uint32_t pbase = lds0 + patch_off;
+        const uint32_t own_addr = pbase + own_rel, row_addr = pbase + row_rel, own_out = pbase + own_out_rel;
+        const uint32_t stat_addr = pbase + NW * 4096 + (wm * (BM / WM) + l31) * 8;
+        const uint32_t gaddr = lds0 + BIAS_OFF + slot_c * 1024 + (wn * 64 + 4 * half) * 4;
+        auto lds_gamma = [&](int j, float (&gv)[4][4]) {
+            u32x4 bq[4];
+#pragma unroll
+            for (int g = 0; g < 4; ++g) asm volatile("ds_read_b128 %0, %1" : "=v"(bq[g]) : "v"(gaddr + (j * 32 + 8 * g) * 4));
+            asm volatile("s_waitcnt lgkmcnt(0)" : "+v"(bq[0]), "+v"(bq[1]), "+v"(bq[2]), "+v"(bq[3]));
+#pragma unroll
+            for (int g = 0; g < 4; ++g)
+#pragma unroll
+                for (int r = 0; r < 4; ++r) gv[g][r] = __uint_as_float(bq[g][r]);
+        };
+        auto stage_block = [&](const __amdgpu_buffer_rsrc_t& rs, int i) {
+            u32x4 rws[4];
+#pragma unroll
+            for (int t = 0; t < 4; ++t) rws[t] = __builtin_bit_cast(u32x4, __builtin_amdgcn_raw_buffer_load_b128(rs, rl_voff, row_soff(i, t), 0));
+            asm volatile("ds_write_b128 %0, %1" ::"v"(row_addr), "v"(rws[0]) : "memory");
+            asm volatile("ds_write_b128 %0, %1 offset:1024" ::"v"(row_addr), "v"(rws[1]) : "memory");
+            asm volatile("ds_write_b128 %0, %1 offset:2048" ::"v"(row_addr), "v"(rws[2]) : "memory");
+            asm volatile("ds_write_b128 %0, %1 offset:3072" ::"v"(row_addr), "v"(rws[3]) : "memory");
+        };
+        auto read_own = [&](int j, u32x2 (&v)[4]) {
+#pragma unroll
+            for (int g = 0; g < 4; ++g) asm volatile("ds_read_b64 %0, %1" : "=v"(v[g]) : "v"(own_addr + (((4 * j + g) ^ (l31 & 7)) << 4)));
+            asm volatile("s_waitcnt lgkmcnt(0)" : "+v"(v[0]), "+v"(v[1]), "+v"(v[2]), "+v"(v[3]));
+        };
+        auto bf16_at = [](const u32x2& q, int r) { return (r & 1) ? __uint_as_float(q[r >> 1] & 0xffff0000u) : __uint_as_float(q[r >> 1] << 16); };
+#pragma unroll
+        for (int i = 0; i < TM; ++i) {
+            u32x2 xin[2][4];
+            stage_block(rxs, i);
+            read_own(0, xin[0]);
+            read_own(1, xin[1]);
+            const int64_t row = m0 + wm * (BM / WM) + i * 32 + l31;
+            const float mean = row < p.m ? p.ln_mean[row] : 0.f, rstd = row < p.m ? p.ln_rstd[row] : 0.f;
+            float sa = 0.f, sb = 0.f;
+#pragma unroll
+            for (int j = 0; j < 2; ++j) {
+                float gam[4][4];
+                lds_gamma(j, gam);
+#pragma unroll
+                for (int g = 0; g < 4; ++g)
+#pragma unroll
+                    for (int r = 0; r < 4; ++r) {
+                        const float t = gam[g][r] * acc[j][i][4 * g + r];
+                        sa += t;
+                        sb += t * ((bf16_at(xin[j][g], r) - mean) * rstd);
+                    }
+            }
+            sa += __shfl_xor(sa, 32, 64);
+            sb += __shfl_xor(sb, 32, 64);
+            {
+                const u32x2 rec = {__float_as_uint(sa), __float_as_uint(sb)};
+                if (half == 0) asm volatile("ds_write_b64 %0, %1" ::"v"(stat_addr + (wn * BM + i * 32) * 8), "v"(rec) : "memory");
+            }
+            asm volatile("s_waitcnt lgkmcnt(0)" ::: "memory");
+            __builtin_amdgcn_s_barrier();
+            sa = 0.f;
+            sb = 0.f;
+#pragma unroll
+            for (int w = 0; w < WN; ++w) {
+                u32x2 rec;
+                asm volatile("ds_read_b64 %0, %1\n\ts_waitcnt lgkmcnt(0)" : "=v"(rec) : "v"(stat_addr + (w * BM + i * 32) * 8) : "memory");
+                sa += __uint_as_float(rec[0]);
+                sb += __uint_as_float(rec[1]);
+            }
+            const float c1 = sa * (1.f / BN), c2 = sb * (1.f / BN);
+            stage_block(rg, i);
+            auto col_step = [&](auto hc, float (&v)[16]) {
+                constexpr int h = decltype(hc)::value;
+                const bool up = (l31 & h) != 0;
+#pragma unroll
+                for (int k = 0; k < h; ++k) {
+                    const float keep = up ? v[k + h] : v[k], send = up ? v[k] : v[k + h];
+                    v[k] = keep + __shfl_xor(send, h, 64);
+                }
+            };
+            auto col_reduce16 = [&](float (&v)[16]) -> float {
+                col_step(std::integral_constant<int, 8>{}, v);
+                col_step(std::integral_constant<int, 4>{}, v);
+                col_step(std::integral_constant<int, 2>{}, v);
+                col_step(std::integral_constant<int, 1>{}, v);
+                return v[0];
+            };
+            float cb[2], cg[2];
+#pragma unroll
+            for (int j = 0; j < 2; ++j) {
+                float gam[4][4];
+                lds_gamma(j, gam);
+                float dbv[16], dgv[16];
+                u32x2 gin[4];
+                read_own(j, gin);
+#pragma unroll
+                for (int g = 0; g < 4; ++g) {
+                    float out[4];
+#pragma unroll
+                    for (int r = 0; r < 4; ++r) {
+                        const float dn = acc[j][i][4 * g + r];
+                        const float xh = (bf16_at(xin[j][g], r) - mean) * rstd;
+                        out[r] = rstd * (gam[g][r] * dn - c1 - xh * c2) + bf16_at(gin[g], r);
+                        dbv[4 * g + r] = dn;
+                        dgv[4 * g + r] = dn * xh;
+                        acc[j][i][4 * g + r] = 0.f;
+                    }
+                    const u32x2 o = {pack_bf16x2(out[0], out[1]), pack_bf16x2(out[2], out[3])};
+                    asm volatile("ds_write_b64 %0, %1" ::"v"(own_out + (((4 * j + g) ^ (l31 & 7)) << 4)), "v"(o) : "memory");
+                }
+                cb[j] = col_reduce16(dbv);
+                cg[j] = col_reduce16(dgv);
+                __builtin_amdgcn_sched_barrier(0);
+            }
+            {
+                const bool up = (l31 & 16) != 0;
+                db_acc += (up ? cb[1] : cb[0]) + __shfl_xor(up ? cb[0] : cb[1], 16, 64);
+                dg_acc += (up ? cg[1] : cg[0]) + __shfl_xor(up ? cg[0] : cg[1], 16, 64);
+            }
+            __builtin_amdgcn_sched_barrier(0);
+            u32x4 rws[4];
+            asm volatile("ds_read_b128 %0, %1" : "=v"(rws[0]) : "v"(row_addr));
+            asm volatile("ds_read2_b64 %0, %1 offset0:129 offset1:128" : "=v"(rws[1]) : "v"(row_addr));
+            asm volatile("ds_read_b128 %0, %1 offset:2048" : "=v"(rws[2]) : "v"(row_addr));
+            asm volatile("ds_read2_b64 %0, %1 offset0:129 offset1:128" : "=v"(rws[3]) : "v"(row_addr + 2048));
+            asm volatile("s_waitcnt lgkmcnt(0)" : "+v"(rws[0]), "+v"(rws[1]), "+v"(rws[2]), "+v"(rws[3]));
+#pragma unroll
+            for (int t = 0; t < 4; ++t)
+                __builtin_amdgcn_raw_buffer_store_b128(__builtin_bit_cast(u32x4v, rws[t]), rc, rl_voff, row_soff(i, t), HS_GEMM_STORE_AUX);
+            asm volatile("s_nop 0" ::"v"(rws[0]), "v"(rws[1]), "v"(rws[2]), "v"(rws[3]));
+        }
+    };
+
     const int stride = p.blocks_per_xcd;
     int id_i = id0, ks_i = 0;
     int id_c = id0, ks_c = 0;
@@ -562,6 +716,7 @@
     bool drained = false;
     constexpr int kEpiOps = TM * (TN / 2 > 0 ? TN / 2 : 1) * 4;
     static_assert((AHEAD - 1) * PIECES_ALL + kEpiOps <= 63, "vmcnt immediate");
+    static_assert(EPI != EPI_LN_BWD || kEpiOps == TM * 4, "the counted wait behind an epilogue assumes at least kEpiOps operations of it");
     TR(0);
     while (true) {
         TR(3);
@@ -590,7 +745,8 @@
         buf = buf + 1 == NSTAGE ? 0 : buf + 1;
         buf_free = buf_free + 1 == NSTAGE ? 0 : buf_free + 1;
         if (last) {
-            epilogue(id_c, buf_done, slot_c);
+            if constexpr (EPI == EPI_LN_BWD) epilogue_ln(id_c, buf_done, slot_c);
+            else epilogue(id_c, buf_done, slot_c);
             slot_c = slot_c + 1 == NSLOT ? 0 : slot_c + 1;
             drained = true;
             ks_c = 0;
@@ -598,6 +754,25 @@
             if (id_c >= id_end) break;
         } else {
             ++ks_c;
+        }
+    }
+    if constexpr (EPI == EPI_LN_BWD) {
+        float* red = (float*)smem;
+        __syncthreads();
+        red[(wave * 64 + lane) * 2] = dg_acc;
+        red[(wave * 64 + lane) * 2 + 1] = db_acc;
+        __syncthreads();
+        if (wm == 0) {
+            float sg = 0.f, sb = 0.f;
+#pragma unroll
+            for (int w = 0; w < WM; ++w) {
+                sg += red[((w * WN + wn) * 64 + lane) * 2];
+                sb += red[((w * WN + wn) * 64 + lane) * 2 + 1];
+            }
+            const int col = wn * 64 + (l31 >> 4) * 32 + 4 * half + ((l31 >> 2) & 3) * 8 + (l31 & 3);
+            float* part = p.ln_part + (size_t)blockIdx.x * (2 * BN);
+            part[col] = sg;
+            part[BN + col] = sb;
         }
     }
 #ifdef HS_GEMM_TRACE
@@ -616,17 +791,23 @@
 #endif
 }
 
-template <int BM, int BN, int WM, int WN, int NSTAGE, bool ALIAS, bool FAST>
-int launch_tile(GemmParams& p, int epi, int wgs_per_cu, hipStream_t s) {
-    const int tiles_m = (int)((p.m + BM - 1) / BM);
-    p.tiles_n = (p.n + BN - 1) / BN;
-    const int64_t tiles = (int64_t)tiles_m * p.tiles_n;
-    if (tiles > 0x7fffffff) return fail(HS_ERR_UNSUPPORTED, "too many output tiles");
+unsigned plan_grid(GemmParams& p, int bm, int bn, int wgs_per_cu) {
+    const int64_t tiles_m = (p.m + bm - 1) / bm;
+    p.tiles_n = (p.n + bn - 1) / bn;
+    const int64_t tiles = tiles_m * p.tiles_n;
+    if (tiles > 0x7fffffff) return 0;
     p.tiles = (int)tiles;
     p.per_xcd = (p.tiles + 7) / 8;
     const int resident = usable_cus_per_xcd() * wgs_per_cu;
     p.blocks_per_xcd = p.per_xcd < resident ? p.per_xcd : resident;
-    const dim3 grid((unsigned)(8 * p.blocks_per_xcd)), block(WM * WN * 64);
+    return (unsigned)(8 * p.blocks_per_xcd);
+}
+
+template <int BM, int BN, int WM, int WN, int NSTAGE, bool ALIAS, bool FAST>
+int launch_tile(GemmParams& p, int epi, int wgs_per_cu, hipStream_t s) {
+    const unsigned blocks = plan_grid(p, BM, BN, wgs_per_cu);
+    if (!blocks) return fail(HS_ERR_UNSUPPORTED, "too many output tiles");
+    const dim3 grid(blocks), block(WM * WN * 64);
     const bool drop = p.drop_p > 0.f;
 #define HS_GEMM_LAUNCH(E, D) hipLaunchKernelGGL((gemm_nt_kernel<BM, BN, WM, WN, NSTAGE, ALIAS, E, D, FAST>), grid, block, 0, s, p)
     switch (epi) {
@@ -643,6 +824,16 @@
     }
 #undef HS_GEMM_LAUNCH
     HS_LAUNCH_CHECK("gemm_nt");
+    return HS_OK;
+}
+
+template <int BM, int BN, int WM, int WN, int NSTAGE>
+int launch_ln_bwd(GemmParams& p, int* blocks, hipStream_t s) {
+    const unsigned g = plan_grid(p, BM, BN, 1);
+    if (!g) return fail(HS_ERR_UNSUPPORTED, "too many output tiles");
+    *blocks = (int)g;
+    hipLaunchKernelGGL((gemm_nt_kernel<BM, BN, WM, WN, NSTAGE, true, EPI_LN_BWD, false, true>), dim3(g), dim3(WM * WN * 64), 0, s, p);
+    HS_LAUNCH_CHECK("gemm_nt_ln_bwd");
     return HS_OK;
 }
 
@@ -724,4 +915,32 @@
     }
 }
 
-}
+int hs_gemm_nt_resident_grid(void) { return hs::usable_cus(); }
+
+int64_t hs_gemm_nt_ln_bwd_workspace(int n) { return (int64_t)256 * 2 * (n > 0 ? n : 0); }
+
+int hs_gemm_nt_ln_bwd(const void* dy, int64_t ldy, const void* w_t, int64_t ldw, int k, const void* x, const float* gamma, const float* mean,
+                      const float* rstd, const void* g, void* dx, float* dgamma, float* dbeta, float* workspace, int accumulate, int64_t m,
+                      int n, int dtype, void* stream) {
+    using namespace hs;
+    HS_CHECK_ARG(dtype == HS_BF16, "hs_gemm_nt_ln_bwd: bf16 only");
+    HS_CHECK_ARG(dy && w_t && x && gamma && mean && rstd && dx && dgamma && dbeta && workspace && m > 0 && k > 0,
+                 "hs_gemm_nt_ln_bwd: null operand or empty shape");
+    HS_CHECK_ARG((accumulate & ~(1 | HS_ACC_DEFER)) == 0, "hs_gemm_nt_ln_bwd: accumulate is 0, 1, or either with HS_ACC_DEFER");
+    if ((n != 128 && n != 256) || k % 64) return fail(HS_ERR_UNSUPPORTED, "hs_gemm_nt_ln_bwd: n must be 128 or 256 and k a multiple of 64");
+    HS_CHECK_ALIGNED("hs_gemm_nt_ln_bwd", 16, dy, w_t, x, gamma, g, dx, dgamma, dbeta, workspace);
+    HS_CHECK_ALIGNED("hs_gemm_nt_ln_bwd", 4, mean, rstd);
+    if (int st = gemm_nt_check_shape("hs_gemm_nt_ln_bwd", ldy, ldw, k, 0, 0, 0, m, n)) return st;
+    GemmParams p{};
+    p.a = (const uint16_t*)dy; p.b = (const uint16_t*)w_t; p.lda = ldy; p.ldb = ldw; p.k = k;
+    p.bias = gamma; p.c = (uint16_t*)dx; p.aux = (uint16_t*)g; p.m = m; p.n = n;
+    p.ln_x = (const uint16_t*)x; p.ln_mean = mean; p.ln_rstd = rstd; p.ln_part = workspace;
+    hipStream_t st = (hipStream_t)stream;
+    int blocks = 0;
+    const int rc = n == 128 ? launch_ln_bwd<256, 128, 4, 2, 3>(p, &blocks, st) : launch_ln_bwd<128, 256, 2, 4, 3>(p, &blocks, st);
+    if (rc) return rc;
+    if (accumulate & HS_ACC_DEFER) return reduce_defer(workspace, 2 * n, blocks, n, 2 * n, dgamma, dbeta, accumulate & 1, st);
+    return reduce_now(workspace, 2 * n, blocks, n, 2 * n, dgamma, dbeta, accumulate & 1, st);
+}
+
+}
diff --git a/heal_swin_amd/models_torch/swin_hp_transformer.py b/heal_swin_amd/models_torch/swin_hp_transformer.py
--- a/heal_swin_amd/models_torch/swin_hp_transformer.py
+++ b/heal_swin_amd/models_torch/swin_hp_transformer.py
@@ -29,8 +29,8 @@
 
 class HSLinear(nn.Linear):
 
-    def forward(self, x):
-        return ops.linear(x, self.weight, self.bias)
+    def forward(self, x, ln_input=False):
+        return ops.linear(x, self.weight, self.bias, ln_input=ln_input)
 
     def forward_passthrough(self, x):
         return ops.linear_passthrough(x, self.weight, self.bias)
@@ -67,11 +67,11 @@
         self.fc2 = HSLinear(hidden_features or in_features, out_features or in_features)
         self.drop = nn.Dropout(drop)
 
-    def forward(self, x, apply_out_drop=True, residual_alias=False, residual=None):
+    def forward(self, x, apply_out_drop=True, residual_alias=False, residual=None, ln_input=False):
         exact_gelu = isinstance(self.act, nn.GELU) and getattr(self.act, "approximate", "none") == "none"
         if exact_gelu and x.dtype in (torch.bfloat16, torch.float32) and x.is_cuda:
             out = ops.mlp(x, self.fc1.weight, self.fc1.bias, self.fc2.weight, self.fc2.bias,
-                          drop_p=self.drop.p if self.training else 0.0, passthrough=residual_alias, residual=residual)
+                          drop_p=self.drop.p if self.training else 0.0, passthrough=residual_alias, residual=residual, ln_input=ln_input)
             y, x_res = out if residual_alias else (out, None)
         elif residual is not None:
             return self.fc2(self.drop(self.act(self.fc1(x)))) + residual
@@ -144,7 +144,7 @@
             return now
         return ops.RelPosBiasFn.apply(self.relative_position_bias_table, self._rel_idx32, self.window_size)
 
-    def attend(self, x, window_size, idx, roll, labels, apply_proj_drop=True, residual_alias=False, residual=None):
+    def attend(self, x, window_size, idx, roll, labels, apply_proj_drop=True, residual_alias=False, residual=None, ln_input=False):
         drop = self.attn_drop.p if self.training else 0.0
         if self.rel_pos_bias is not None and window_size != self.window_size:
             raise AssertionError("relative position bias needs input_resolution >= window_size")
@@ -159,7 +159,7 @@
         if residual_alias:
             qkv, x_res = self.qkv.forward_passthrough(x)
         else:
-            qkv = self.qkv(x)
+            qkv = self.qkv(x, ln_input=ln_input)
         o = ops.window_attn_core(qkv, self.bias(), self.head_scale(), idx, roll, labels, self.num_heads, window_size,
                                  self.use_cos_attn, attn_drop=drop)
         if residual is not None:
@@ -263,14 +263,14 @@
         return (f"dim={self.dim}, input_resolution={self.input_resolution}, num_heads={self.num_heads}, "
                 f"window_size={self.window_size}, shift_size={self.shift_size}, mlp_ratio={self.mlp_ratio}")
 
-    def _attention_branch(self, x, apply_proj_drop=True, residual_alias=False, residual=None):
+    def _attention_branch(self, x, apply_proj_drop=True, residual_alias=False, residual=None, ln_input=False):
         if not self._shifted:
-            return self.attn.attend(x, self.window_size, None, 0, None, apply_proj_drop, residual_alias, residual)
+            return self.attn.attend(x, self.window_size, None, 0, None, apply_proj_drop, residual_alias, residual, ln_input)
         idx, _, labels = self.shifter.tables(x.device)
         if self._is_roll:
             return self.attn.attend(x, self.window_size, None, self.shift_size % x.shape[1], labels, apply_proj_drop, residual_alias,
-                                    residual)
-        return self.attn.attend(x, self.window_size, idx, 0, labels, apply_proj_drop, residual_alias, residual)
+                                    residual, ln_input)
+        return self.attn.attend(x, self.window_size, idx, 0, labels, apply_proj_drop, residual_alias, residual, ln_input)
 
     def _stochastic(self):
         return self.training and ((isinstance(self.drop_path, DropPath) and self.drop_path.drop_prob > 0) or
@@ -336,8 +336,8 @@
                         return x2, None, None
                     n2, x1 = ops.layer_norm_passthrough(x1, self.norm2.weight, self.norm2.bias)
                 if fc2_own:
-                    return self.mlp(n2, apply_out_drop=False, residual=x1), None, None
-                return x1, (self.mlp(n2, apply_out_drop=False), None, 0.0), None
+                    return self.mlp(n2, apply_out_drop=False, residual=x1, ln_input=True), None, None
+                return x1, (self.mlp(n2, apply_out_drop=False, ln_input=True), None, 0.0), None
             if proj_own or fc2_own:
                 if pending is None:
                     n1, xs = ops.layer_norm_passthrough(x, self.norm1.weight, self.norm1.bias)
@@ -345,16 +345,17 @@
                     t, rs, dp = pending
                     xs, n1 = ops.add_layer_norm(x, t, self.norm1.weight, self.norm1.bias, row_scale=rs, drop_p=dp)
                 if proj_own:
-                    x1 = self._attention_branch(n1, apply_proj_drop=False, residual=xs)
+                    x1 = self._attention_branch(n1, apply_proj_drop=False, residual=xs, ln_input=True)
                     x2 = self._fused_mlp(x1)
                     if x2 is not None:
                         return x2, None, None
                     n2, x1 = ops.layer_norm_passthrough(x1, self.norm2.weight, self.norm2.bias)
                 else:
-                    x1, n2 = ops.add_layer_norm(xs, self._attention_branch(n1, apply_proj_drop=False), self.norm2.weight, self.norm2.bias)
+                    x1, n2 = ops.add_layer_norm(xs, self._attention_branch(n1, apply_proj_drop=False, ln_input=True), self.norm2.weight,
+                                                self.norm2.bias)
                 if fc2_own:
-                    return self.mlp(n2, apply_out_drop=False, residual=x1), None, None
-                return x1, (self.mlp(n2, apply_out_drop=False), None, 0.0), None
+                    return self.mlp(n2, apply_out_drop=False, residual=x1, ln_input=True), None, None
+                return x1, (self.mlp(n2, apply_out_drop=False, ln_input=True), None, 0.0), None
         if pending is None:
             n1, x = ops.layer_norm_passthrough(x, self.norm1.weight, self.norm1.bias)
         elif comp:
@@ -363,7 +364,7 @@
         else:
             t, rs, dp = pending
             x, n1 = ops.add_layer_norm(x, t, self.norm1.weight, self.norm1.bias, row_scale=rs, drop_p=dp)
-        a = self._attention_branch(n1, apply_proj_drop=False)
+        a = self._attention_branch(n1, apply_proj_drop=False, ln_input=True)
         if comp:
             x1, n2, x1_lo = ops.add_layer_norm_stream(x, x_lo, a, self.norm2.weight, self.norm2.bias, row_scale=self._path_scale(x),
                                                       drop_p=self.attn.proj_drop.p if train else 0.0)
@@ -371,7 +372,7 @@
             x1_lo = None
             x1, n2 = ops.add_layer_norm(x, a, self.norm2.weight, self.norm2.bias, row_scale=self._path_scale(x),
                                         drop_p=self.attn.proj_drop.p if train else 0.0)
-        m = self.mlp(n2, apply_out_drop=False)
+        m = self.mlp(n2, apply_out_drop=False, ln_input=True)
         return x1, (m, self._path_scale(x), self.mlp.drop.p if train else 0.0), x1_lo
 
     def can_stream_v2(self):
diff --git a/heal_swin_amd/ops/attention.py b/heal_swin_amd/ops/attention.py
--- a/heal_swin_amd/ops/attention.py
+++ b/heal_swin_amd/ops/attention.py
@@ -344,7 +344,7 @@
         return (y, x_res) if residual_alias else y
     assert not residual_alias
     n1, xs = LayerNormFn.apply(x, ln_weight, ln_bias, None, None, True, None, False, (xn, mean, rstd))
-    qkv_t = LinearFn.apply(n1, qkv_w, qkv_b, False, None, (qkv,))
+    qkv_t = LinearFn.apply(n1, qkv_w, qkv_b, False, None, (qkv,), True)
     o_t = WindowAttnCoreFn.apply(qkv_t, bias, head_scale, idx, roll, labels, num_heads, window_size, cosine, 0.0, 0, (o, lse))
     x1 = LinearFn.apply(o_t, proj_w, proj_b, False, xs, (out,))
     if n2 is None:
diff --git a/heal_swin_amd/ops/gemm.py b/heal_swin_amd/ops/gemm.py
--- a/heal_swin_amd/ops/gemm.py
+++ b/heal_swin_amd/ops/gemm.py
@@ -98,6 +98,40 @@
 
 
 RESID_EPILOGUE = True
+LN_BWD_EPILOGUE = os.environ.get("HS_LN_BWD_EPILOGUE", "1") != "0"
+_LN_TILE_ROWS = {128: 256, 256: 128}
+_LN_DEFERRED = {}
+
+
+def ln_bwd_epilogue_ok(x, c_in, n_out):
+    if not (LN_BWD_EPILOGUE and x.is_cuda and x.dtype == torch.bfloat16 and c_in in _LN_TILE_ROWS and n_out % 64 == 0):
+        return False
+    return x.numel() // c_in >= int(lib.hs_gemm_nt_resident_grid()) * _LN_TILE_ROWS[c_in]
+
+
+def defer_input_grad(dy2, weight, cache):
+    ph = torch.empty((dy2.shape[0], weight.numel() // weight.shape[0]), dtype=dy2.dtype, device=dy2.device)
+    while len(_LN_DEFERRED) >= 8:
+        del _LN_DEFERRED[next(iter(_LN_DEFERRED))]
+    _LN_DEFERRED[ph.data_ptr()] = (ph, dy2, weight, cache)
+    return ph
+
+
+def take_deferred_input_grad(dy):
+    job = _LN_DEFERRED.get(dy.data_ptr()) if dy is not None else None
+    if job is None or job[0].numel() != dy.numel() or job[0].dtype != dy.dtype:
+        return None
+    del _LN_DEFERRED[dy.data_ptr()]
+    return job[1:]
+
+
+def gemm_nt_ln_bwd(dy2, weight, cache, x, gamma, mean, rstd, g, dx, dgamma, dbeta, ws, acc):
+    m, k = dy2.shape
+    w_t = _cast_param_t(weight, dy2.dtype, cache)
+    n = w_t.shape[0]
+    with _timed(f"hs_gemm_nt_ln_bwd m={m} n={n} k={k}", dy2.device, 2 * (m * k + n * k + m * n * (3 if g is not None else 2)), 2 * m * n * k):
+        check(lib.hs_gemm_nt_ln_bwd(ptr(dy2), dy2.stride(0), ptr(w_t), w_t.stride(0), k, ptr(x), ptr(gamma), ptr(mean), ptr(rstd), ptr(g), ptr(dx),
+                                    dgamma, dbeta, ws, acc, m, n, _lib.HS_BF16, stream_ptr(dy2.device)), "hs_gemm_nt_ln_bwd")
 
 
 def gemm_nt(a2d, w, bias=None, epi=0, aux=None, a2=None, w2=None, want_c=True, drop_p=0.0, seed=0):
@@ -354,7 +388,7 @@
 class LinearFn(torch.autograd.Function):
 
     @staticmethod
-    def forward(ctx, x, weight, bias, passthrough=False, residual=None, pre=None):
+    def forward(ctx, x, weight, bias, passthrough=False, residual=None, pre=None, ln_input=False):
         _require_gpu(x, weight, bias, residual)
         n_out = weight.shape[0]
         k_in = weight.numel() // n_out
@@ -365,6 +399,7 @@
         ctx.cast_cache = RT.cast_cache
         ctx.passthrough = passthrough
         ctx.has_residual = residual is not None
+        ctx.ln_defer = bool(ln_input) and not passthrough and ln_bwd_epilogue_ok(x, k_in, n_out)
         ctx.x3 = None
         if pre is not None:
             y = pre[0]
@@ -430,18 +465,20 @@
         n_out = weight.shape[0]
         k_in = weight.numel() // n_out
         if dy is None:
-            return dx_res, None, None, None, None, None
+            return dx_res, None, None, None, None, None, None
         dy2 = dy.reshape(-1, n_out)
         x2 = None if x is None else x.reshape(-1, k_in)
         if not dy2.is_contiguous():
             dy2 = dy2.contiguous()
         dx = None
-        if ctx.needs_input_grad[0]:
+        if ctx.needs_input_grad[0] and ctx.ln_defer and dx_res is None and _aligned(dy2) is dy2:
+            dx = defer_input_grad(dy2, weight, ctx.cast_cache).reshape(ctx.x_shape)
+        elif ctx.needs_input_grad[0]:
             dx = _input_grad(dy2, weight, ctx.w_cast, None if dx_res is None else dx_res.reshape(-1, k_in), ctx.cast_cache).reshape(ctx.x_shape)
         ctx.w_cast = ctx.cast_cache = None
         x3, ctx.x3 = ctx.x3, None
         dw, db = _param_grads(dy2, x2, weight, bias, ctx.needs_input_grad[1], bias is not None and ctx.needs_input_grad[2], x3)
-        return dx, dw, db, None, (dy if ctx.has_residual else None), None
+        return dx, dw, db, None, (dy if ctx.has_residual else None), None, None
 
 
 def _input_grad(dy2, weight, w_cast, dx_res2=None, cache=None):
@@ -458,8 +495,8 @@
     return _lib_matmul(dy2, w)
 
 
-def linear(x, weight, bias=None):
-    return LinearFn.apply(x, weight, bias)
+def linear(x, weight, bias=None, ln_input=False):
+    return LinearFn.apply(x, weight, bias, False, None, None, bool(ln_input))
 
 
 def linear_residual(x, weight, bias, residual):
diff --git a/heal_swin_amd/ops/mlp_branch.py b/heal_swin_amd/ops/mlp_branch.py
--- a/heal_swin_amd/ops/mlp_branch.py
+++ b/heal_swin_amd/ops/mlp_branch.py
@@ -6,15 +6,16 @@
 from .._lib import check, lib, ptr, stream_ptr
 from .runtime import RT, _cast_param, _defer_flag, _defer_keep, _draw_seed, _extras, _f32, _require_gpu, _timed
 from .norm import _norm_param_grads, _norm_param_result
-from .gemm import (_Split, _bf16x3_ok, _cast_param_t, _input_grad, _lib_linear, _lib_matmul, _param_grads, _split_of, gemm_nt, own_gemm_legal, own_gemm_ok)
+from .gemm import (_Split, _bf16x3_ok, _cast_param_t, _input_grad, defer_input_grad, ln_bwd_epilogue_ok, _lib_linear, _lib_matmul, _param_grads, _split_of, gemm_nt, own_gemm_legal, own_gemm_ok)
 
 
 class MlpFn(torch.autograd.Function):
 
     @staticmethod
-    def forward(ctx, x, w1, b1, w2, b2, drop_p, seed, passthrough, residual=None):
+    def forward(ctx, x, w1, b1, w2, b2, drop_p, seed, passthrough, residual=None, ln_input=False):
         _require_gpu(x, w1, b1, w2, b2, residual)
         c_in, hid = w1.shape[1], w1.shape[0]
+        ctx.ln_defer = bool(ln_input) and not passthrough and ln_bwd_epilogue_ok(x, c_in, hid)
         x2 = x.reshape(-1, c_in)
         if not x2.is_contiguous():
             x2 = x2.contiguous()
@@ -66,7 +67,7 @@
         w1c, w2c = ctx.casts
         p, seed, xshape = ctx.meta
         if dy is None:
-            return dx_res, None, None, None, None, None, None, None, None
+            return dx_res, None, None, None, None, None, None, None, None, None
         c_out, hid, c_in = w2.shape[0], w1.shape[0], w1.shape[1]
         dy2 = dy.reshape(-1, c_out)
         if not dy2.is_contiguous():
@@ -85,19 +86,21 @@
                 check(lib.hs_gelu_bwd(ptr(da), ptr(h), ptr(dh), h.numel(), p, seed, _lib.dtype_code(dt), stream_ptr(h.device)), "hs_gelu_bwd")
             del da
         dx = None
-        if ctx.needs_input_grad[0]:
+        if ctx.needs_input_grad[0] and ctx.ln_defer and dx_res is None and not isinstance(dh, _Split):
+            dx = defer_input_grad(dh, w1, ctx.cast_cache).reshape(xshape)
+        elif ctx.needs_input_grad[0]:
             dx = _input_grad(dh, w1, w1c, None if dx_res is None else dx_res.reshape(-1, c_in), ctx.cast_cache).reshape(xshape)
         ctx.casts = ctx.cast_cache = None
         (x3, a3), ctx.splits = ctx.splits, (None, None)
         dw2, db2 = _param_grads(dy2, a, w2, b2, ctx.needs_input_grad[3], b2 is not None and ctx.needs_input_grad[4], a3)
         dw1, db1 = _param_grads(dh, x2, w1, b1, ctx.needs_input_grad[1], b1 is not None and ctx.needs_input_grad[2], x3)
-        return dx, dw1, db1, dw2, db2, None, None, None, (dy if ctx.has_residual else None)
-
-
-def mlp(x, w1, b1, w2, b2, drop_p=0.0, seed=None, passthrough=False, residual=None):
+        return dx, dw1, db1, dw2, db2, None, None, None, (dy if ctx.has_residual else None), None
+
+
+def mlp(x, w1, b1, w2, b2, drop_p=0.0, seed=None, passthrough=False, residual=None, ln_input=False):
     if drop_p > 0.0 and seed is None:
         seed = _draw_seed()
-    return MlpFn.apply(x, w1, b1, w2, b2, float(drop_p), int(seed or 0), bool(passthrough), residual)
+    return MlpFn.apply(x, w1, b1, w2, b2, float(drop_p), int(seed or 0), bool(passthrough), residual, bool(ln_input))
 
 
 FUSED_MLP = os.environ.get("HS_FUSED_MLP", "1") != "0"
diff --git a/heal_swin_amd/ops/norm.py b/heal_swin_amd/ops/norm.py
--- a/heal_swin_amd/ops/norm.py
+++ b/heal_swin_amd/ops/norm.py
@@ -30,6 +30,17 @@
     if acc & _lib.HS_ACC_DEFER:
         _defer_keep(device, ws)
     return _norm_param_result(weight, bias, dgamma, dbeta, direct)
+
+
+def _deferred_product(dy, width, plain):
+    from . import gemm
+    job = gemm.take_deferred_input_grad(dy)
+    if job is None:
+        return dy, None
+    if plain and dy.dtype == torch.bfloat16 and width in gemm._LN_TILE_ROWS:
+        return dy, job
+    dy2, weight, cache = job
+    return gemm._input_grad(dy2, weight, None, None, cache).reshape(dy.shape), None
 
 
 class LayerNormFn(torch.autograd.Function):
@@ -81,11 +92,15 @@
             dx_alias = None
         if dy is None:
             return dx_alias, None, None, None, None, None, None, None, None
+        dy, job = _deferred_product(dy, width, extras is None and not has_res)
         dy = _aligned(dy.contiguous())
         dx = torch.empty_like(x)
 
         def call(dgamma, dbeta, ws, acc):
-            if dx_alias is not None:
+            if job is not None:
+                from .gemm import gemm_nt_ln_bwd
+                gemm_nt_ln_bwd(*job, x, g, mean, rstd, None if dx_alias is None else _aligned(dx_alias.contiguous()), dx, dgamma, dbeta, ws, acc)
+            elif dx_alias is not None:
                 check(lib.hs_add_layernorm_bwd(ptr(dy), ptr(_aligned(dx_alias.contiguous())), ptr(x), ptr(g), ptr(mean), ptr(rstd), ptr(dx),
                                                dgamma, dbeta, ws, acc, rows, width, dt, stream_ptr(x.device)), "hs_add_layernorm_bwd")
             else:
@@ -150,13 +165,17 @@
             if extras is None:
                 return ds, ds, None, None, None, None, None
             dy = torch.zeros_like(s)
+        dy, job = _deferred_product(dy, width, extras is None)
         dy = _aligned(dy.contiguous())
         ds_c = None if ds is None else _aligned(ds.contiguous())
         da = torch.empty_like(s)
         db = da if extras is None else torch.empty_like(s)
 
         def call(dgamma, dbeta, ws, acc):
-            if extras is None:
+            if job is not None:
+                from .gemm import gemm_nt_ln_bwd
+                gemm_nt_ln_bwd(*job, s, g, mean, rstd, ds_c, da, dgamma, dbeta, ws, acc)
+            elif extras is None:
                 check(lib.hs_add_layernorm_bwd(ptr(dy), ptr(ds_c), ptr(s), ptr(g), ptr(mean), ptr(rstd), ptr(da), dgamma, dbeta, ws, acc,
                                                rows, width, dt, stream_ptr(s.device)), "hs_add_layernorm_bwd")
             else:
diff --git a/include/healswin.h b/include/healswin.h
--- a/include/healswin.h
+++ b/include/healswin.h
@@ -235,6 +235,11 @@
                int64_t ldb2, int k2, const float* bias, void* c, void* aux, int64_t m, int n, int epilogue, float drop_p,
                uint64_t seed, int dtype, void* stream);
 int hs_gemm_nt_set_tile(int variant);
+int hs_gemm_nt_ln_bwd(const void* dy, int64_t ldy, const void* w_t, int64_t ldw, int k, const void* x, const float* gamma, const float* mean,
+                      const float* rstd, const void* g, void* dx, float* dgamma, float* dbeta, float* workspace, int accumulate, int64_t m,
+                      int n, int dtype, void* stream);
+int64_t hs_gemm_nt_ln_bwd_workspace(int n);
+int hs_gemm_nt_resident_grid(void);
 
 int hs_pix2ang_nest(int nside, int64_t first, int64_t count, double* theta, double* phi);
 int hs_sample_bilinear_u8(const void* img, int batch, int channels, int height, int width, const double* rx, const double* ry,
```
